# skmhrk1209/GANSynth

Hardware: AMD Instinct MI355X
Metric: G+D step images/sec at 128x1024x2 mel+IF (higher is better)
Workload: dtype bf16; 1 GPU; BASELINE.json configs[1]: fully grown PGGAN 128x1024x2 G+D iteration (D update + G update, R1 + mode-seeking), per-GPU batch 8, random-init weights; global_batch=8, parallelism=dp1, launch=hipGraph replay, forked branches, forked_branches=True

## Files before the change

### gansynth_amd/_lib.py

```python
import ctypes
import os
from ctypes import c_char_p, c_double, c_float, c_int, c_int64, c_size_t, c_void_p, POINTER

_HERE = os.path.dirname(os.path.abspath(__file__))
LIB_PATH = os.path.join(_HERE, "libgansynth_hip.so")

GS_F32, GS_BF16 = 0, 1
ACT_NONE, ACT_LRELU, ACT_TANH = 0, 1, 2
ACT_LRELU_BITS, ACT_WRITE_BITS = 5, 16
PREP_CONV_FWD, PREP_CONV_BWD_DATA, PREP_CONVT_FWD, PREP_CONVT_BWD_DATA = 0, 1, 2, 3
CONV_FWD, CONV_BWD_DATA, CONV_BWD_WEIGHT = 0, 1, 2

P, I, F, L, Z = c_void_p, c_int, c_float, c_int64, c_size_t


class GsConv(ctypes.Structure):
    _fields_ = [("n", ctypes.c_int32), ("h", ctypes.c_int32), ("w", ctypes.c_int32), ("ci", ctypes.c_int32), ("co", ctypes.c_int32),
                ("ksize", ctypes.c_int32), ("stride", ctypes.c_int32), ("transposed", ctypes.c_int32), ("dtype", ctypes.c_int32),
                ("w_prepared", ctypes.c_int32), ("alpha", c_float), ("ws", c_void_p), ("ws_bytes", c_size_t)]


C = POINTER(GsConv)

SIGNATURES = {
    "gs_last_error": (c_char_p, []),
    "gs_version": (I, []),
    "gs_init": (I, []),
    "gs_streams_create": (I, [I, POINTER(P)]),
    "gs_streams_destroy": (I, [I, POINTER(P)]),
    "gs_prof_enable": (I, [I]),
    "gs_prof_collect": (I, [POINTER(c_int), POINTER(c_double), POINTER(c_double)]),
    "gs_prof_roofline": (I, [ctypes.c_double, ctypes.c_double, P, P, P]),
    "gs_prof_records": (I, [I, P, P, P, P, P]),
    "gs_comm_available": (I, []),
    "gs_comm_unique_id": (I, [P]),
    "gs_comm_init": (I, [POINTER(P), I, I, P]),
    "gs_comm_destroy": (I, [P]),
    "gs_comm_count": (I, [P, POINTER(I)]),
    "gs_allreduce_sum_f32": (I, [P, P, ctypes.c_int64, P]),
    "gs_comm_set_marker_us": (I, [P, ctypes.c_double]),
    "gs_broadcast_f32": (I, [P, P, ctypes.c_int64, I, P]),
    "gs_conv_workspace_bytes": (Z, [C, I]),
    "gs_conv_fwd": (I, [C, P, P, P, I, P, P, F, P]),
    "gs_conv_fwd_mask": (I, [C, P, P, P, I, P, P]),
    "gs_conv_bwd_data": (I, [C, P, P, P, I, P, P]),
    "gs_conv_bwd_data_pnbwd": (I, [C, P, P, P, P, I, F, P, P]),
    "gs_conv_bwd_data_pnbwd_is_fused": (I, [C]),
    "gs_conv_fwd_pnbwdbwd": (I, [C, P, P, P, P, I, F, P, P, P]),
    "gs_conv_fwd_pnbwdbwd_is_fused": (I, [C]),
    "gs_conv_bwd_weight": (I, [C, P, P, P, P, I, P]),
    "gs_conv_wgrad_jobs_workspace_bytes": (Z, [P, I]),
    "gs_conv_wgrad_jobs": (I, [P, I, P, Z, P]),
    "gs_wgrad_cu_cap": (I, [I]),
    "gs_conv_igemm_config": (I, [I, I, I, I, I, I, I, I, POINTER(c_int)]),
    "gs_conv_igemm_table": (I, [I, POINTER(c_int)]),
    "gs_units_bias_act_to_nhwc": (I, [P, P, P, P, I, I, I, I, I, P]),
    "gs_nhwc_act_bwd_to_units": (I, [P, P, P, I, I, I, I, I, P]),
    "gs_dense_fwd_workspace_bytes": (Z, [I, I, I]),
    "gs_dense_fwd": (I, [P, P, P, I, I, I, F, I, P, Z, P]),
    "gs_dense_fwd_bias_act": (I, [P, P, P, P, I, I, I, F, I, I, P, Z, P]),
    "gs_dense_fwd_bias_act_nhwc": (I, [P, P, P, P, I, I, I, I, F, I, I, P, Z, P]),
    "gs_dense_bwd_data": (I, [P, P, P, I, I, I, F, I, P]),
    "gs_dense_bwd_weight": (I, [P, P, P, I, I, I, F, I, I, P]),
    "gs_dense_fwd_nhwc": (I, [P, P, P, I, I, I, I, F, I, P, Z, P]),
    "gs_dense_bwd_data_nhwc": (I, [P, P, P, I, I, I, I, F, I, P]),
    "gs_dense_bwd_weight_nhwc": (I, [P, P, P, I, I, I, I, F, I, I, P]),
    "gs_embedding_fwd": (I, [P, P, P, I, I, I, F, I, P]),
    "gs_embedding_onehot_fwd": (I, [P, P, P, P, I, I, I, F, I, P]),
    "gs_embedding_bwd": (I, [P, P, P, I, I, I, F, I, P]),
    "gs_bias_act_fwd": (I, [P, P, P, L, I, I, I, P]),
    "gs_act_bwd": (I, [P, P, P, L, I, I, P]),
    "gs_act_bwd_bias": (I, [P, P, P, P, L, I, I, I, I, P, Z, P]),
    "gs_tanh_bwd_bwd": (I, [P, P, P, P, L, I, P]),
    "gs_channel_sum_workspace_bytes": (Z, [L, I]),
    "gs_channel_sum": (I, [P, P, L, I, I, I, P, Z, P]),
    "gs_bias_partial_rows": (I, [I, L, I, I]),
    "gs_channel_fold_batch_workspace_bytes": (Z, [P, I]),
    "gs_channel_fold_batch": (I, [P, I, P, Z, P]),
    "gs_pixel_norm_fwd": (I, [P, P, L, I, F, I, P]),
    "gs_pixel_norm_bwd_fused": (I, [P, P, P, P, L, I, F, I, I, I, P]),
    "gs_pixel_norm_bwd_bias_workspace_bytes": (Z, [L, I, I]),
    "gs_pixel_norm_bwd_fused_bias": (I, [P, P, P, P, P, L, I, F, I, I, I, I, P, Z, P]),
    "gs_pixel_norm_bwd_bwd_fused": (I, [P, P, P, P, P, L, I, F, I, I, P]),
    "gs_upscale2d": (I, [P, P, I, I, I, I, I, I, F, I, P]),
    "gs_blocksum2d": (I, [P, P, I, I, I, I, I, I, F, I, P]),
    "gs_batch_stddev_fwd": (I, [P, P, I, I, I, F, I, P]),
    "gs_batch_stddev_bwd": (I, [P, P, P, P, I, I, I, F, I, P]),
    "gs_batch_stddev_bwd_bwd": (I, [P, P, P, P, P, I, I, I, F, I, P]),
    "gs_axpby": (I, [P, P, P, L, F, F, I, P]),
    "gs_axpby_dev": (I, [P, P, P, L, P, I, I, I, P]),
    "gs_sumsq_rows_workspace_bytes": (Z, [I]),
    "gs_sumsq_rows": (I, [P, P, I, L, I, P, Z, P]),
    "gs_row_scale": (I, [P, P, F, P, I, L, I, P]),
    "gs_weight_prep_batch": (I, [P, I, P]),
    "gs_gan_d_loss": (I, [P, P, P, P, F, I, I, P, P, P, P, I, P]),
    "gs_gan_g_loss": (I, [P, P, P, F, F, I, I, P, P, P, I, P]),
    "gs_adam_tf_step": (I, [P, P, P, P, L, F, F, F, F, F, P]),
    "gs_adam_tf_step_zero_grad": (I, [P, P, P, P, L, F, F, F, F, F, P]),
    "gs_adam_tf_step_dev": (I, [P, P, P, P, L, P, F, F, F, F, I, P]),
    "gs_pack_act_bits": (I, [P, L, I, I, P]),
    "gs_spectral_plan_create": (I, [POINTER(c_void_p), I, I, I, P, P]),
    "gs_spectral_plan_destroy": (I, [P]),
    "gs_stft_fwd": (I, [P, P, I, I, I, P, P, P]),
    "gs_mel_project": (I, [P, P, P, L, P]),
    "gs_if_unwrap": (I, [P, P, P, I, P]),
    "gs_stft_mel_if_fwd": (I, [P, P, I, I, I, P, I, P, Z, P]),
    "gs_stft_mel_if_workspace_bytes": (Z, [P, I]),
    "gs_mel_if_to_waveform": (I, [P, P, I, I, I, P, I, P, Z, P]),
    "gs_mel_if_to_waveform_workspace_bytes": (Z, [P, I]),
    "gs_weight_standardize": (I, [P, P, I, I, F, P]),
    "gs_resnet_stem_pool": (I, [P, P, P, P, P, I, I, I, I, I, P]),
    "gs_max_pool2d": (I, [P, P, I, I, I, I, I, P]),
    "gs_conv1x1_fwd": (I, [P, P, P, I, I, I, I, I, I, I, P]),
    "gs_group_norm_workspace_bytes": (Z, [I, I, I, I]),
    "gs_group_norm_stats": (I, [P, P, P, P, I, I, I, I, F, I, P, Z, P]),
    "gs_group_norm_apply": (I, [P, P, P, P, P, I, I, I, I, I, I, P]),
# ... 83 lines not shown
```

### gansynth_amd/config.py

```python
import os

KNOBS = {
    "GS_TORCH_COLLECTIVES": ("operational", "gradient all-reduce through torch.distributed's communicator instead of the library's own (gs_comm_*)"),
    "GS_NO_GRAPH_ALLREDUCE": ("operational", "no RCCL collective inside captured graphs: eager all-reduce behind each replay (bench.DP_LADDER's tamer modes)"),
    "GS_FORK_PROBE": ("operational", "auto | always | never: probe a forked hipGraph replay in a child process before the first forked capture "
                                     "(auto: only on HIP builds the workaround was not debugged on, fork_probe._forked_replay_ok)"),
    "GS_FORK_PROBED": ("operational", "(set by the probe for child processes: ok | died)"),
    "GS_FORK_PROBE_TIMEOUT_S": ("operational", "budget of that probe, seconds (600)"),
    "GS_LEVEL_STREAMS": ("operational", "throw-away streams alive while a graph is instantiated (128; capture.Capture._leveled_queues)"),
    "GS_COMM_MARKER_US": ("operational", "tests / profiles at world size 1: the one-rank all-reduce becomes a kernel that holds its stream this long "
                                         "(read once per communicator, comm.RcclComm; gs_comm_set_marker_us)"),
    "GS_CAPTURE_MODE": ("operational", "debugging: force torch.cuda.graph's capture_error_mode"),
    "GS_DEBUG_POISON_WS": ("operational", "debugging: kernel workspaces start as NaN bit patterns"),
    "GS_CHECK_FUSION": ("operational", "debugging: every fused cross-node form also runs its unfused definition and the two are compared"),
    "GS_FORK_EAGER": ("operational", "tests: the forked branches with eager launches on two streams"),
    "GS_NO_FORK_MARKS": ("operational", "debugging: branches start where they are opened, not at their marks"),
    "GS_NO_FORK": ("schedule", "no parallel branches in the runs' graphs (5.9 against 5.2 ms; also taken when GPU_MAX_HW_QUEUES != 4 or the probe fails)"),
    "GS_NO_MERGED_RUNS": ("schedule", "part A of the generator run NOT inside the discriminator run's graph (5.13 against 4.99 ms)"),
    "GS_NO_FUSED_ITERATION": ("schedule", "two graphs per iteration with eager optimizer steps between them (neutral on one GPU; data parallel both "
                                          "all-reduces are then the last node of a graph)"),
    "GS_OVERLAP_REDUCE": ("schedule", "data parallel: round 4's four-graph iteration, each all-reduce on a forked branch beside part A of the other run "
                                      "(hides both collectives; +0.7 ms at world size 1)"),
    "GS_NO_OVERLAP_REDUCE": ("schedule", "(overrides GS_OVERLAP_REDUCE)"),
    "GS_DEBUG_DP_BUCKET": ("operational", "print the range the first message of a two-step discriminator all-reduce covers"),
    "GS_DP_BUCKET_D": ("schedule", "data parallel: the discriminator's gradient all-reduced in two steps, ~98 % of it beside the end of its backward (300-us stand-ins: -0.09 ... -0.14 ms fully grown, +0.15 in a fade-in)"),
    "GS_EARLY_FLUSH_DIV": ("schedule", "a layer is 'large' from 1/DIV of the full resolution's pixels (16)"),
    "GS_EARLY_FLUSH_CUS": ("schedule", "CUs the early weight-gradient contraction is sized for (192; 160 / 224 / 256 within noise, round 6)"),
    "GS_D_TAIL_LEVELS": ("schedule", "levels of the discriminator's tail run over [real; fake] as one batch when the runs do not fork (3)"),
    "GS_NO_EARLY_FLUSH": ("ablation", "weight gradients of the full-chip levels contracted at the end of the run only"),
    "GS_NO_DEFERRED_REDUCE": ("ablation", "every weight gradient contracted where autograd produces it"),
    "GS_NO_DEFERRED_FOLDS": ("ablation", "bias-gradient partial rows folded by their producers"),
    "GS_NO_WGRAD_GROUPS": ("ablation", "no grouped weight-gradient launches"),
    "GS_NO_SPLIT_G_LOSS": ("ablation", "the generator's loss as one launch over both halves: the mode-seeking second-order pass waits for the discriminator's forward"),
    "GS_NO_SPLIT_FINAL_FLUSH": ("ablation", "the final weight-gradient contraction of a run on one stream (HBM-bound and MFMA-bound jobs one after the other)"),
    "GS_NO_FUSED_LOSSES": ("ablation", "per-sample loss algebra in torch instead of the one-launch loss heads"),
    "GS_NO_D_TAIL_BATCH": ("ablation", "real and fake pass through the discriminator's tail separately (no-fork schedule)"),
    "GS_NO_FUSED_NORM": ("ablation", "pixel norm as its own node behind every generator conv"),
    "GS_NO_NORM_EPILOGUE": ("ablation", "no pixel norm in conv epilogues"),
    "GS_NO_NORM_BWD_EPILOGUE": ("ablation", "no previous-block norm backward in data-gradient epilogues"),
    "GS_NO_NORM_BWD2_EPILOGUE": ("ablation", "no second-order norm kernel in the forward-on-cotangent conv"),
    "GS_NO_NORM_BWD_BIAS": ("ablation", "bias sums outside the norm's backward"),
    "GS_NO_MASK_BITS": ("ablation", "leaky-relu masks read as the bf16 activations themselves, not as the sign bits stored behind them"),
    "GS_NO_PREMASK": ("ablation", "activation derivative never folded into the consuming data-gradient kernel"),
    "GS_NO_PREMASK_GRAPH": ("ablation", "... not across autograd nodes"),
    "GS_NO_PREMASK_GRAPH2": ("ablation", "... not in second-order graphs"),
    "GS_NO_PARAMS_ONLY": ("ablation", "leaf activations receive gradients like tf.gradients would not ask for"),
    "GS_NO_DERIVED_SLICES": ("ablation", "the 257-channel conv's weight slices copied on every use"),
    "GS_NO_UNITS_NHWC": ("ablation", "dense -> reshape -> activation as three steps"),
    "GS_NO_DENSE_NHWC": ("ablation", "flatten copy + plain dense kernels"),
}


def _check(name):
    if name not in KNOBS:
        raise KeyError("gansynth_amd.config: %s is not a registered environment switch (add it to KNOBS with its description)" % name)


def flag(name):
    _check(name)
    return bool(os.environ.get(name))


def value(name, default=None):
    _check(name)
    return os.environ.get(name, default)
```

### gansynth_amd/csrc/conv_api.hip

```cpp
#include "conv_shared.h"
#include <utility>
#include <vector>

namespace gs {


bool igemm_supported(int ic, int oc, int dtype);
bool igemm_norm_fused(int mode, int N, int Hb, int Wb, int IC, int OC, int dtype, int want);
int igemm_config(int mode, int N, int Hb, int Wb, int IC, int OC, int dtype, int want, int* out);
int igemm_table(int index, int* out);
extern "C" int gs_pixel_norm_bwd_bwd_fused(const void* gg, const void* g, const void* x, void* out, void* out_g, int64_t p, int c, float eps, int pre_act,
                                           int dtype, void* stream);
bool wgrad_mfma_supported(int ic, int oc, int dtype);
size_t igemm_prep_bytes(int ic, int oc, int dtype);
int run_igemm(int mode, int variant, const void* x, const float* w_hwio, void* y, int N, int Hi, int Wi, int ICk,
              int OCk, int w_ci, int w_co, int Hb, int Wb, float alpha, const float* bias, int act, int dtype, int w_prepared,
              void* ws, size_t ws_bytes, hipStream_t st, const void* mask = nullptr, int mask_act = 0, void* y2 = nullptr, float pn_eps = 0.f,
              const void* addend = nullptr, int normbwd = 0);
extern "C" int gs_pixel_norm_bwd_fused(const void* g, const void* x, const void* addend, void* gx, int64_t p, int c, float eps, int pre_act, int post_act, int dtype,
                                       void* stream);
size_t wgrad_mfma_bytes(int mode, int dtype, int N, int Hb, int Wb, int IC, int OC);
bool wgrad_mfma_has_bias(int dtype);
int run_wgrad_mfma(int mode, const WgradSrcs& srcs, int nsrc, float* gw, float* gb, int N, int Hi, int Wi, int IC, int OC, int Hb,
                   int Wb, float alpha, int transpose, int accumulate, int dtype, void* ws, size_t ws_bytes, hipStream_t st,
                   GsWgradReduce* defer = nullptr);
bool wgrad_sk_supported(int mode, int dtype, int IC, int OC);
void wgrad_sk_job_geometry(int mode, int N, SkJob& q);
void wgrad_sk_plan(int mode, SkGroup& g);
size_t wgrad_sk_bytes(const SkGroup& g);
int run_wgrad_sk(int mode, const SkGroup& g, void* ws, size_t ws_bytes, hipStream_t st);

template <typename T, int OCV, int VEC>
__global__ void conv_direct_kernel(const T* __restrict__ x, const float* __restrict__ wp, T* __restrict__ y, int mode,
                                   int ks, int N, int Hi, int Wi, int IC, int OC, int Ho, int Wo, float alpha) {
    const int ngrp = OC / OCV;
    const long idx = (long)blockIdx.x * blockDim.x + threadIdx.x;
    const long total = (long)N * Ho * Wo * ngrp;
    if (idx >= total) return;
    const int g = idx % ngrp;
    long pix = idx / ngrp;
    const int ox = pix % Wo;
    pix /= Wo;
    const int oy = pix % Ho;
    const int n = pix / Ho;
    const int oc = g * OCV;
    float acc[OCV];
#pragma unroll
    for (int v = 0; v < OCV; ++v) acc[v] = 0.f;
    for (int ky = 0; ky < ks; ++ky) {
        int iy;
        if (mode == MODE_S1) iy = oy + ky - (ks >> 1);
// ... 140 lines not shown
                word |= (unsigned)__builtin_amdgcn_update_dpp(0, (int)word, 0x4E, 0xf, 0xf, false);
                if (piece == 0) bits[(px * OC + oc0) >> 5] = word;
                return;
            }
        }
        st_wide<T>(y + px * OC + oc0, o);
    };
    auto ldpix = [&](long px, float* xv) __attribute__((always_inline)) {
        if constexpr (IC == 2 && sizeof(T) == 2) {
            const unsigned u = *reinterpret_cast<const unsigned*>(x + px * 2);
            xv[0] = __uint_as_float(u << 16);
            xv[1] = __uint_as_float(u & 0xffff0000u);
        } else {
#pragma unroll
            for (int i = 0; i < IC; ++i) xv[i] = DT<T>::ld(x + px * IC + i);
        }
    };
    for (; pix + 3 * stride < P; pix += 4 * stride) {
        float xv[4][IC];
#pragma unroll
        for (int k = 0; k < 4; ++k) ldpix(pix + k * stride, xv[k]);
#pragma unroll
        for (int k = 0; k < 4; ++k) one(pix + k * stride, xv[k]);
    }
    for (; pix < P; pix += stride) {
        float xv[IC];
        ldpix(pix, xv);
        one(pix, xv);
    }
}

template <typename T, int IC>
__global__ __launch_bounds__(256) void thin_expand_pnbwd_kernel(const T* __restrict__ x, const float* __restrict__ wp, const T* __restrict__ z,
                                                                const T* __restrict__ addend, T* __restrict__ y, long P, int OC, float alpha, float eps, int act) {
    constexpr int WN = Wide<T>::N;
    const int groups = OC / WN;
    const int oc0 = (threadIdx.x % groups) * WN;
    float wr[WN][IC];
#pragma unroll
    for (int v = 0; v < WN; ++v)
#pragma unroll
        for (int i = 0; i < IC; ++i) wr[v][i] = wp[(long)(oc0 + v) * IC + i] * alpha;
    const long ppb = 256 / groups;
    const long stride = (long)gridDim.x * ppb;
    const long npass = (P + stride - 1) / stride;
    const float inv_c = 1.f / (float)OC;
    for (long k = 0; k < npass; ++k) {
        const long pix = (long)blockIdx.x * ppb + threadIdx.x / groups + k * stride;
        const long px = pix < P ? pix : P - 1;
        float xv[IC], zv[WN], av[WN], g[WN];
        if constexpr (IC == 2 && sizeof(T) == 2) {
            const unsigned u = *reinterpret_cast<const unsigned*>(x + px * 2);
            xv[0] = __uint_as_float(u << 16);
            xv[1] = __uint_as_float(u & 0xffff0000u);
        } else {
#pragma unroll
            for (int i = 0; i < IC; ++i) xv[i] = DT<T>::ld(x + px * IC + i);
        }
        ld_wide<T>(z + px * OC + oc0, zv);
        if (addend) ld_wide<T>(addend + px * OC + oc0, av);
        float ssq = 0.f, szg = 0.f;
#pragma unroll
        for (int v = 0; v < WN; ++v) {
            float a = 0.f;
#pragma unroll
            for (int i = 0; i < IC; ++i) a += xv[i] * wr[v][i];
            g[v] = a;
            ssq += zv[v] * zv[v];
            szg += zv[v] * a;
        }
        ssq = group_sum(ssq, groups);
        szg = group_sum(szg, groups);
        const float r = rsqrtf(ssq * inv_c + eps);
        const float m = szg * inv_c * r * r;
        float out[WN];
#pragma unroll
        for (int v = 0; v < WN; ++v) {
            float t = r * (g[v] - zv[v] * m);
            if (addend) t += av[v];
            out[v] = act == GS_ACT_LRELU ? (zv[v] > 0.f ? t : 0.2f * t) : t;
        }
        if (pix < P) st_wide<T>(y + pix * OC + oc0, out);
    }
}
static bool thin_expand_pnbwd_ok(int ks, int ICk, int OCk, int dtype) {
    const int wn = dtype == GS_F32 ? 4 : 8;
    if (ks != 1 || ICk < 1 || ICk > 4 || OCk % wn != 0) return false;
    const int groups = OCk / wn;
    return groups >= 1 && groups <= 64 && (groups & (groups - 1)) == 0;
}
static int run_thin_expand_pnbwd(const void* x, const float* wp, const void* z, const void* addend, void* y, long P, int ICk, int OCk, float alpha, float eps, int act,
                                 int dtype, hipStream_t st) {
    const int wn = dtype == GS_F32 ? 4 : 8;
    long nb = cdiv(P * (OCk / wn), 256);
    if (nb > 4096) nb = 4096;
    const unsigned grid = (unsigned)nb;
#define GS_TEP(TT, ICV) hipLaunchKernelGGL((thin_expand_pnbwd_kernel<TT, ICV>), dim3(grid), dim3(256), 0, st, (const TT*)x, wp, (const TT*)z, (const TT*)addend, (TT*)y, P, OCk, alpha, eps, act)
#define GS_TEP_ALL(TT) do { if (ICk == 1) GS_TEP(TT, 1); else if (ICk == 2) GS_TEP(TT, 2); else if (ICk == 3) GS_TEP(TT, 3); else GS_TEP(TT, 4); } while (0)
    GS_DISPATCH_DTYPE(dtype, GS_TEP_ALL(T));
#undef GS_TEP_ALL
#undef GS_TEP
    GS_CHECK_LAUNCH();
    return 0;
}

template <typename T, int OC, int ACT, int LC>
__global__ __launch_bounds__(256) void thin_reduce_kernel(const T* __restrict__ x, const float* __restrict__ wp, const float* __restrict__ bias,
                                                          T* __restrict__ y, long P, int IC, float alpha) {
    constexpr int WN = Wide<T>::N;
    const int L = LC ? LC : IC / WN;
    const int l = threadIdx.x % L;
    float wr[OC][WN];
#pragma unroll
    for (int v = 0; v < OC; ++v)
#pragma unroll
        for (int i = 0; i < WN; ++i) wr[v][i] = wp[v * IC + l * WN + i] * alpha;
    const long ppb = 256 / L;
    const long npass = (P + (long)gridDim.x * ppb - 1) / ((long)gridDim.x * ppb);
    float bv[OC];
#pragma unroll
    for (int v = 0; v < OC; ++v) bv[v] = bias ? bias[v] : 0.f;
    auto fold = [&](float* a) __attribute__((always_inline)) {
#pragma unroll
        for (int v = 0; v < OC; ++v) a[v] = group_sum(a[v], LC != 0 ? LC : L);
    };
    auto finish = [&](long pix, float* a) __attribute__((always_inline)) {
        fold(a);
        if (pix < P && l == 0) {
            if constexpr (OC == 2 && sizeof(T) == 2) {
                *reinterpret_cast<unsigned*>(y + pix * 2) = pack_bf16x2(thin_act<ACT>(a[0] + bv[0]), thin_act<ACT>(a[1] + bv[1]));
// ... 798 lines not shown
    JobPlan plan;
    if (plan_jobs(jobs, njobs, plan)) return 0;
    return plan.total_bytes;
}

extern "C" int gs_conv_wgrad_jobs(const GsWgradJob* jobs, int njobs, void* ws, size_t ws_bytes, void* stream) {
    GS_CHECK_ARG(njobs >= 0 && (njobs == 0 || jobs), "conv_wgrad_jobs: bad args");
    if (njobs == 0) return 0;
    JobPlan plan;
    if (int e = plan_jobs(jobs, njobs, plan)) return e;
    if (ws_bytes < plan.total_bytes) return fail(GS_ERR_WORKSPACE, "conv_wgrad_jobs: workspace %zu < %zu", ws_bytes, plan.total_bytes);
    hipStream_t st = as_stream(stream);
    for (auto& kg : plan.groups)
        if (int e = run_wgrad_sk(kg.first, kg.second, ws, plan.group_bytes, st)) return e;
    std::vector<GsWgradReduce> pend;
    for (size_t k = 0; k < plan.single.size(); ++k) {
        const GsWgradJob& jb = plan.single[k];
        GsConv c = job_conv(jb, jb.n[0]);
        c.ws = reinterpret_cast<unsigned char*>(ws) + plan.single_off[k];
        c.ws_bytes = (k + 1 < plan.single.size() ? plan.single_off[k + 1] : plan.total_bytes) - plan.single_off[k];
        GsWgradReduce d;
        memset(&d, 0, sizeof(d));
        if (int rc = wgrad_layer(c, jb.x, jb.gy, jb.n, jb.nsrc, jb.bias_mask, jb.gw, jb.gb, jb.accumulate, &d, stream)) return rc;
        if (jb.gw_ci_stride > jb.ci) {
            if (d.nslices <= 0 || d.transpose) return fail(GS_ERR_UNSUPPORTED, "conv_wgrad_jobs: a %d -> %d layer cannot add into a channel slice", jb.ci, jb.co);
            d.ic_ld = jb.gw_ci_stride;
        }
        if (d.nslices > 0) pend.push_back(d);
    }
    if (!pend.empty()) return wgrad_reduce_batch(pend.data(), (int)pend.size(), stream);
    return 0;
}

extern "C" int gs_conv_fwd_pnbwdbwd(const GsConv* c, const void* x, const float* w_hwio, const void* g, const void* z, int act, float eps, void* out_g, void* out_z,
                                    void* stream) {
    if (int e = check_conv(c)) return e;
    GS_CHECK_ARG(g && z && out_g && out_z && (act == GS_ACT_NONE || act == GS_ACT_LRELU), "conv_fwd_pnbwdbwd: g, z and both outputs are required, activation none or leaky relu (got %d)", act);
    const ConvRole r = conv_role(*c, GS_CONV_FWD);
    if (c->ksize == 3 && igemm_supported(r.ICk, r.OCk, c->dtype))
        return run_igemm(r.mode, r.variant, x, w_hwio, out_g, c->n, r.Hi, r.Wi, r.ICk, r.OCk, c->ci, c->co, r.Hb, r.Wb, c->alpha, nullptr, GS_ACT_NONE, c->dtype, c->w_prepared, c->ws,
                         c->ws_bytes, as_stream(stream), z, act, out_z, eps, g, 2);
    if (int e = gs_conv_fwd(c, x, w_hwio, nullptr, GS_ACT_NONE, out_g, nullptr, 0.f, stream)) return e;
    return gs_pixel_norm_bwd_bwd_fused(out_g, g, z, out_z, out_g, (int64_t)c->n * r.Ho * r.Wo, c->co, eps, act, c->dtype, stream);
}
extern "C" int gs_conv_fwd_pnbwdbwd_is_fused(const GsConv* c) {
    if (check_conv(c) || c->ksize != 3 || !(c->transposed || c->stride == 1)) return 0;
    const ConvRole r = conv_role(*c, GS_CONV_FWD);
    return igemm_norm_fused(r.mode, c->n, r.Hb, r.Wb, r.ICk, r.OCk, c->dtype, IGEMM_NORM_BWD2) ? 1 : 0;
}

extern "C" int gs_conv_bwd_data_pnbwd(const GsConv* c, const void* gy, const float* w_hwio, const void* z, const void* addend, int act, float eps, void* gx, void* stream) {
    if (int e = check_conv(c)) return e;
    GS_CHECK_ARG(z && gx && (act == GS_ACT_NONE || act == GS_ACT_LRELU), "conv_bwd_data_pnbwd: z is required, activation none or leaky relu (got %d)", act);
    hipStream_t st = as_stream(stream);
    const ConvRole r = conv_role(*c, GS_CONV_BWD_DATA);
    const bool epilogue_map = c->transposed || c->stride == 1;
    if (epilogue_map && c->ksize == 3 && igemm_supported(r.ICk, r.OCk, c->dtype))
        return run_igemm(r.mode, r.variant, gy, w_hwio, gx, c->n, r.Hi, r.Wi, r.ICk, r.OCk, c->ci, c->co, r.Hb, r.Wb, c->alpha, nullptr, GS_ACT_NONE, c->dtype, c->w_prepared, c->ws,
                         c->ws_bytes, st, z, act, nullptr, eps, addend, 1);
    if (c->stride == 1 && thin_expand_pnbwd_ok(c->ksize, r.ICk, r.OCk, c->dtype)) {
        const long total = (long)c->ci * c->co;
        if (c->ws_bytes < (size_t)total * 4) return fail(GS_ERR_WORKSPACE, "conv_bwd_data_pnbwd: workspace %zu < %zu", c->ws_bytes, (size_t)total * 4);
        float* wp = reinterpret_cast<float*>(c->ws);
        if (!c->w_prepared) {
            hipLaunchKernelGGL((weight_prep_kernel<float>), dim3(cdiv(total, 256)), dim3(256), 0, st, w_hwio, wp, 1, c->ci, c->co, 1);
            GS_CHECK_LAUNCH();
        }
        return run_thin_expand_pnbwd(gy, wp, z, addend, gx, (long)c->n * r.Ho * r.Wo, r.ICk, r.OCk, c->alpha, eps, act, c->dtype, st);
    }
    if (int e = gs_conv_bwd_data(c, gy, w_hwio, nullptr, 0, gx, stream)) return e;
    return gs_pixel_norm_bwd_fused(gx, z, addend, gx, (int64_t)c->n * r.Ho * r.Wo, c->ci, eps, GS_ACT_NONE, act, c->dtype, stream);
}
extern "C" int gs_conv_bwd_data_pnbwd_is_fused(const GsConv* c) {
    if (check_conv(c) || !(c->transposed || c->stride == 1)) return 0;
    const ConvRole r = conv_role(*c, GS_CONV_BWD_DATA);
    if (c->ksize == 1) return thin_expand_pnbwd_ok(1, r.ICk, r.OCk, c->dtype) ? 1 : 0;
    return igemm_norm_fused(r.mode, c->n, r.Hb, r.Wb, r.ICk, r.OCk, c->dtype, IGEMM_NORM_BWD) ? 1 : 0;
}
extern "C" int gs_conv_igemm_config(int mode, int n, int hb, int wb, int ic, int oc, int dtype, int want, int* out_cfg) {
    return igemm_config(mode, n, hb, wb, ic, oc, dtype, want, out_cfg);
}
extern "C" int gs_conv_igemm_table(int index, int* out11) { return igemm_table(index, out11); }
```

### gansynth_amd/csrc/conv_igemm.hip

```cpp
#include "conv_device.h"
#include "gs_prof.h"

extern "C" int gs_pixel_norm_fwd(const void* x, void* y, int64_t p, int c, float eps, int dtype, void* stream);
extern "C" int gs_pack_act_bits(void* z, int64_t p, int c, int dtype, void* stream);
extern "C" int gs_pixel_norm_bwd_fused(const void* g, const void* x, const void* addend, void* gx, int64_t p, int c, float eps, int pre_act, int post_act, int dtype,
                                       void* stream);
extern "C" int gs_pixel_norm_bwd_bwd_fused(const void* gg, const void* g, const void* x, void* out, void* out_g, int64_t p, int c, float eps, int pre_act,
                                           int dtype, void* stream);

namespace gs {

struct ConvP {
    const void* x;
    const void* wp;
    void* y;
    const float* bias;
    int act;
    const void* mask;
    int mask_act;
    const unsigned char* mask_bits;
    unsigned char* bits_out;
    void* y2;
    float pn_eps;
    const void* addend;
    int normbwd;
    int* norm_pending;
    int N, Hi, Wi, IC, OC, Hb, Wb, tiles_x, tiles_y, nsp, noct, nch;
    unsigned m_noct, m_tx, m_ty;
    float alpha;
#ifdef GS_IGEMM_TRACE
    unsigned long long* trace;
#endif
};
#ifdef GS_IGEMM_TRACE
#define GS_TR(slot)                                                                                              \
    do {                                                                                                         \
        if (p.trace && threadIdx.x == 0 && (slot) < 64) {                                                        \
            p.trace[blockIdx.x * 64 + (slot)] = __builtin_amdgcn_s_memtime();                                    \
            if ((slot) == 0 || (slot) == 63) p.trace[4096 * 64 + blockIdx.x * 2 + ((slot) == 63)] = __builtin_amdgcn_s_memrealtime(); \
        }                                                                                                        \
    } while (0)
#else
#define GS_TR(slot) do { } while (0)
#endif

__device__ __forceinline__ void lds_dma16_s(unsigned lds_addr, unsigned voff, i32x4 rs, unsigned soff) {
    asm volatile("s_mov_b32 m0, %0\n\ts_nop 0\n\tbuffer_load_dwordx4 %1, %2, %3 offen lds"
                 :
                 : "s"(lds_addr), "v"(voff), "s"(rs), "s"(__builtin_amdgcn_readfirstlane(soff))
                 : "memory", "m0");
}

#ifndef GS_NORM_EPI_PIPELINE
#define GS_NORM_EPI_PIPELINE 1
#endif
template <typename T, int MODE, int A, int B, int TW, int TG, bool RESIDENT, int D, int NORM, int RB = 64, bool SPEC = false, bool BITS = false>
__global__ __launch_bounds__(SPEC ? 512 : 256) void conv_igemm_kernel(const ConvP p) {
// ... 202 lines not shown
    zero_acc();
    if (computer) {
#pragma unroll
        for (int b = 0; b < B; ++b)
#pragma unroll
            for (int ox = 0; ox < 3; ++ox)
#pragma unroll
                for (int ks = 0; ks < KS; ++ks) asm volatile("" : "+v"(b_off[b][ox][ks]));
#pragma unroll
        for (int ks = 0; ks < KS; ++ks) asm volatile("" : "+v"(a_off[ks]));
#pragma unroll
        for (int ph = 0; ph < NPH; ++ph)
#pragma unroll
            for (int a = 0; a < A; ++a)
#pragma unroll
                for (int b = 0; b < B; ++b) asm volatile("" : "+v"(acc[ph][a][b]));
    }
    wait_vmcnt(0);
    block_barrier();
    GS_TR(3);
#ifdef GS_IGEMM_TRACE
    int tr_stage = 0;
#endif

    int item = first, done = 0, c_pb = 0, c_wb = 0;
    while (true) {
        int n, by, bx, oc0;
        item_coords(item, n, by, bx, oc0);
        unsigned mbw[BITS ? B * (MODE == MODE_T2 ? 4 : 1) : 1][A];
        constexpr bool NPIPE = (NORM == 2 || NORM == 3) && A * B <= 2 && GS_NORM_EPI_PIPELINE;
        typedef typename std::conditional<SZ == 4, float4, uint4>::type nvec_t;
        constexpr int NNV = SZ == 4 ? 4 : 2;
        nvec_t nz[NPIPE ? 2 : 1][A][NNV], nx[NPIPE ? 2 : 1][A][NNV];
        auto norm_fetch = [&](int i, nvec_t (&zq)[A][NNV], nvec_t (&xq)[A][NNV]) __attribute__((always_inline)) {
            constexpr int NPHB = MODE == MODE_T2 ? 4 : 1;
            const int b = i / NPHB, ph = i % NPHB;
            const int Ho = MODE == MODE_T2 ? 2 * Hb : Hb, Wo = MODE == MODE_T2 ? 2 * Wb : Wb;
            const int q = (wv * B + b) * 32 + l31;
            const int gy = by + q / TW, gx = bx + q % TW;
            const int oy = MODE == MODE_T2 ? 2 * gy + (ph >> 1) : gy;
            const int ox = MODE == MODE_T2 ? 2 * gx + (ph & 1) : gx;
            const long base = (gy < Hb && gx < Wb) ? (((long)n * Ho + oy) * Wo + ox) * OC + oc0 : 0;
#ifdef GS_ABL_NOMASKLOAD
            const long zbase = base & 1023;
#else
            const long zbase = base;
#endif
#pragma unroll
            for (int a = 0; a < A; ++a)
#pragma unroll
                for (int v = 0; v < NNV; ++v) {
                    zq[a][v] = *reinterpret_cast<const nvec_t*>(reinterpret_cast<const T*>(p.mask) + zbase + a * 32 + v * (32 / NNV) + hi * (16 / NNV));
                    if (NORM == 3 || p.addend)
                        xq[a][v] = *reinterpret_cast<const nvec_t*>(reinterpret_cast<const T*>(p.addend) + base + a * 32 + v * (32 / NNV) + hi * (16 / NNV));
                }
        };
        for (int ch = 0; ch < NCH; ++ch) {
#pragma unroll
            for (int tg = 0; tg < NTG; ++tg) {
                const int itg = (tg + D) % NTG;
                const int npiece = stage_pieces(itg);
                if (issuer) issue_setup(itg);
                if constexpr (NPIPE) {
                    if (tg == NTG - 1 && ch == NCH - 1 && computer) norm_fetch(0, nz[0], nx[0]);
                }
                if constexpr (BITS) {
                    if (tg == NTG - 1 && ch == NCH - 1 && computer && p.mask_bits) {
                        constexpr int NPHB = MODE == MODE_T2 ? 4 : 1;
                        const int Ho = MODE == MODE_T2 ? 2 * Hb : Hb, Wo = MODE == MODE_T2 ? 2 * Wb : Wb;
#pragma unroll
                        for (int b = 0; b < B; ++b) {
                            const int q = (wv * B + b) * 32 + l31;
                            const int gy = by + q / TW, gx = bx + q % TW;
#pragma unroll
                            for (int ph = 0; ph < NPHB; ++ph) {
                                const int oy = MODE == MODE_T2 ? 2 * gy + (ph >> 1) : gy;
                                const int ox = MODE == MODE_T2 ? 2 * gx + (ph & 1) : gx;
                                const long off = (gy < Hb && gx < Wb) ? (((long)n * Ho + oy) * Wo + ox) * OC + oc0 : 0;
#pragma unroll
                                for (int a = 0; a < A; ++a) mbw[b * NPHB + ph][a] = *reinterpret_cast<const unsigned*>(p.mask_bits + ((off + a * 32) >> 3));
                            }
                        }
                    }
                }
                if (SPEC && loader) {
#pragma unroll
                    for (int q = 0; q < npiece; ++q) issue_piece(q, itg);
                }
                const unsigned char* lp = lpatch + c_pb * PBUF;
                const unsigned char* lw = RESIDENT ? lwgt + ch * WBUF : lwgt + c_wb * WBUF;
                if (computer) {
                    constexpr int PF = NSTEP >= 6 ? 2 : 1;
                    frag_t af[PF + 1][A], bf[PF + 1][B];
                    auto load_frag = [&](int step, int r) __attribute__((always_inline)) {
                        const int tt = step / KS, ks = step % KS, buf = step % (PF + 1);
                        const int i = tg * TG + tt;
                        const int oyv = tap_off<MODE>(tap_ky<MODE>(i)), oxv = tap_off<MODE>(tap_kx<MODE>(i));
// ... 152 lines not shown
                    } else if constexpr (MASK_ALL) {
                        if (p.mask) {
#pragma unroll
                            for (int b = 0; b < B; ++b) {
                                const int q = (wv * B + b) * 32 + l31;
                                const int gy = by + q / TW, gx = bx + q % TW;
#pragma unroll
                                for (int ph = 0; ph < NPH; ++ph) {
                                    const int oy = MODE == MODE_T2 ? 2 * gy + (ph >> 1) : gy;
                                    const int ox = MODE == MODE_T2 ? 2 * gx + (ph & 1) : gx;
                                    mask_fetch((((long)n * Ho + oy) * Wo + ox) * OC + oc0, gy < Hb && gx < Wb, mz_all[b * NPH + ph]);
                                }
                            }
                        }
                    }
#pragma unroll
                    for (int b = 0; b < B; ++b) {
                        const int q = (wv * B + b) * 32 + l31;
                        const int gy = by + q / TW, gx = bx + q % TW;
#ifdef GS_ABL_NOSTORE
                        const bool inside = gy < -1000;
#else
                        const bool inside = gy < Hb && gx < Wb;
#endif
#pragma unroll
                        for (int ph = 0; ph < NPH; ++ph) {
                            const int oy = MODE == MODE_T2 ? 2 * gy + (ph >> 1) : gy;
                            const int ox = MODE == MODE_T2 ? 2 * gx + (ph & 1) : gx;
                            const long off = (((long)n * Ho + oy) * Wo + ox) * OC + oc0;
                            if constexpr (NORM == 2) {
                                constexpr int EV = 16 / NV;
                                const int cur = NPIPE ? ((b * NPH + ph) & 1) : 0;
                                if constexpr (NPIPE) {
                                    if (b * NPH + ph + 1 < B * NPH) norm_fetch(b * NPH + ph + 1, nz[(b * NPH + ph + 1) & 1], nx[(b * NPH + ph + 1) & 1]);
                                } else {
                                    mask_fetch(off, inside, nz[0]);
                                    if (p.addend) {
                                        const long base = inside ? off : 0;
#pragma unroll
                                        for (int a = 0; a < A; ++a)
#pragma unroll
                                            for (int v = 0; v < NV; ++v)
                                                nx[0][a][v] = *reinterpret_cast<const mvec_t*>(reinterpret_cast<const T*>(p.addend) + base + a * 32 + v * (32 / NV) + hi * (16 / NV));
                                    }
                                }
                                mvec_t (&zq)[A][NV] = nz[cur];
                                mvec_t (&aq)[A][NV] = nx[cur];
                                float gv[A][NV][EV], zv[A][NV][EV];
                                float ssq = 0.f, szg = 0.f;
#pragma unroll
                                for (int a = 0; a < A; ++a) {
                                    float o[4][4];
                                    finish(ph, a, b, o);
                                    if constexpr (SZ == 4) {
#pragma unroll
                                        for (int qd = 0; qd < 4; ++qd) {
                                            const float4 z4 = zq[a][qd];
                                            const float zz[4] = {z4.x, z4.y, z4.z, z4.w};
#pragma unroll
                                            for (int e = 0; e < 4; ++e) { gv[a][qd][e] = o[qd][e]; zv[a][qd][e] = zz[e]; }
                                        }
                                    } else {
#pragma unroll
                                        for (int qp = 0; qp < 2; ++qp) {
#pragma unroll
                                            for (int e = 0; e < 4; ++e) {
                                                const auto r = __builtin_amdgcn_permlane32_swap(__float_as_uint(o[2 * qp][e]), __float_as_uint(o[2 * qp + 1][e]), false, false);
                                                gv[a][qp][e] = __uint_as_float(r[0]);
                                                gv[a][qp][4 + e] = __uint_as_float(r[1]);
                                            }
                                            const uint4 z4 = zq[a][qp];
                                            const unsigned zw[4] = {z4.x, z4.y, z4.z, z4.w};
#pragma unroll
                                            for (int e = 0; e < 4; ++e) { zv[a][qp][2 * e] = __uint_as_float(zw[e] << 16); zv[a][qp][2 * e + 1] = __uint_as_float(zw[e] & 0xffff0000u); }
                                        }
                                    }
#pragma unroll
                                    for (int v = 0; v < NV; ++v)
#pragma unroll
                                        for (int e = 0; e < EV; ++e) { ssq += zv[a][v][e] * zv[a][v][e]; szg += zv[a][v][e] * gv[a][v][e]; }
                                }
                                ssq = swap32_sum(ssq);
                                szg = swap32_sum(szg);
                                const float inv_c = 1.f / (float)(32 * A);
                                const float r = rsqrtf(ssq * inv_c + p.pn_eps);
                                const float m = szg * inv_c * r * r;
#pragma unroll
                                for (int a = 0; a < A; ++a)
#pragma unroll
                                    for (int v = 0; v < NV; ++v) {
                                        float out[EV], ad[EV];
#pragma unroll
                                        for (int e = 0; e < EV; ++e) ad[e] = 0.f;
                                        if (p.addend) {
                                            if constexpr (SZ == 4) {
                                                const float4 a4 = aq[a][v];
                                                ad[0] = a4.x; ad[1] = a4.y; ad[2] = a4.z; ad[3] = a4.w;
                                            } else {
                                                const uint4 a4 = aq[a][v];
                                                const unsigned aw[4] = {a4.x, a4.y, a4.z, a4.w};
#pragma unroll
                                                for (int e = 0; e < 4; ++e) { ad[2 * e] = __uint_as_float(aw[e] << 16); ad[2 * e + 1] = __uint_as_float(aw[e] & 0xffff0000u); }
                                            }
                                        }
#pragma unroll
                                        for (int e = 0; e < EV; ++e) out[e] = (r * (gv[a][v][e] - zv[a][v][e] * m) + ad[e]) * mask_factor(zv[a][v][e]);
                                        if (inside) {
                                            if constexpr (SZ == 4) {
                                                st4(reinterpret_cast<float*>(y) + off + a * 32 + v * 8 + hi * 4, out);
                                            } else {
                                                uint4 w4;
                                                w4.x = pack_bf16x2(out[0], out[1]); w4.y = pack_bf16x2(out[2], out[3]);
                                                w4.z = pack_bf16x2(out[4], out[5]); w4.w = pack_bf16x2(out[6], out[7]);
                                                *reinterpret_cast<uint4*>(reinterpret_cast<bf16_t*>(y) + off + a * 32 + v * 16 + hi * 8) = w4;
                                            }
                                        }
                                    }
                            } else if constexpr (NORM == 3) {
                                constexpr int EV = 16 / NV;
                                const int cur = NPIPE ? ((b * NPH + ph) & 1) : 0;
                                if constexpr (NPIPE) {
                                    if (b * NPH + ph + 1 < B * NPH) norm_fetch(b * NPH + ph + 1, nz[(b * NPH + ph + 1) & 1], nx[(b * NPH + ph + 1) & 1]);
                                } else {
                                    mask_fetch(off, inside, nz[0]);
                                    const long base = inside ? off : 0;
#pragma unroll
                                    for (int a = 0; a < A; ++a)
#pragma unroll
                                        for (int v = 0; v < NV; ++v)
                                            nx[0][a][v] = *reinterpret_cast<const mvec_t*>(reinterpret_cast<const T*>(p.addend) + base + a * 32 + v * (32 / NV) + hi * (16 / NV));
                                }
                                mvec_t (&zq)[A][NV] = nz[cur];
                                mvec_t (&gq)[A][NV] = nx[cur];
                                float hv[A][NV][EV], zv[A][NV][EV], gv[A][NV][EV];
                                float ssq = 0.f, shg = 0.f, shz = 0.f, szg = 0.f;
#pragma unroll
                                for (int a = 0; a < A; ++a) {
                                    float o[4][4];
                                    finish(ph, a, b, o);
                                    if constexpr (SZ == 4) {
#pragma unroll
                                        for (int qd = 0; qd < 4; ++qd) {
                                            const float4 z4 = zq[a][qd], g4 = gq[a][qd];
                                            const float zz[4] = {z4.x, z4.y, z4.z, z4.w}, g_[4] = {g4.x, g4.y, g4.z, g4.w};
#pragma unroll
                                            for (int e = 0; e < 4; ++e) { hv[a][qd][e] = o[qd][e]; zv[a][qd][e] = zz[e]; gv[a][qd][e] = g_[e]; }
                                        }
                                    } else {
#pragma unroll
                                        for (int qp = 0; qp < 2; ++qp) {
#pragma unroll
                                            for (int e = 0; e < 4; ++e) {
                                                const auto r = __builtin_amdgcn_permlane32_swap(__float_as_uint(o[2 * qp][e]), __float_as_uint(o[2 * qp + 1][e]), false, false);
                                                hv[a][qp][e] = __uint_as_float(r[0]);
                                                hv[a][qp][4 + e] = __uint_as_float(r[1]);
                                            }
                                            const uint4 z4 = zq[a][qp], g4 = gq[a][qp];
                                            const unsigned zw[4] = {z4.x, z4.y, z4.z, z4.w}, gw_[4] = {g4.x, g4.y, g4.z, g4.w};
#pragma unroll
                                            for (int e = 0; e < 4; ++e) {
                                                zv[a][qp][2 * e] = __uint_as_float(zw[e] << 16); zv[a][qp][2 * e + 1] = __uint_as_float(zw[e] & 0xffff0000u);
                                                gv[a][qp][2 * e] = __uint_as_float(gw_[e] << 16); gv[a][qp][2 * e + 1] = __uint_as_float(gw_[e] & 0xffff0000u);
                                            }
                                        }
                                    }
#pragma unroll
                                    for (int v = 0; v < NV; ++v)
#pragma unroll
                                        for (int e = 0; e < EV; ++e) {
                                            const float zc = zv[a][v][e], gc = gv[a][v][e];
                                            const float hc = hv[a][v][e] * mask_factor(zc);
                                            hv[a][v][e] = hc;
                                            ssq += zc * zc; shg += hc * gc; shz += hc * zc; szg += zc * gc;
                                        }
                                }
                                ssq = swap32_sum(ssq); shg = swap32_sum(shg);
                                shz = swap32_sum(shz); szg = swap32_sum(szg);
                                const float inv_c = 1.f / (float)(32 * A);
                                const float r = rsqrtf(ssq * inv_c + p.pn_eps);
                                const float r2 = r * r, r3 = r2 * r;
                                const float ma = shg * inv_c, mb = shz * inv_c, mm = szg * inv_c;
                                const float kz = 3.f * r3 * r2 * mb * mm - r3 * ma;
#pragma unroll
                                for (int a = 0; a < A; ++a)
#pragma unroll
                                    for (int v = 0; v < NV; ++v) {
                                        float o1[EV], o2[EV];
#pragma unroll
                                        for (int e = 0; e < EV; ++e) {
                                            const float zc = zv[a][v][e], gc = gv[a][v][e], hc = hv[a][v][e];
                                            o1[e] = r * (hc - zc * r2 * mb);
                                            o2[e] = kz * zc - r3 * (mm * hc + mb * gc);
                                        }
                                        if (inside) {
                                            if constexpr (SZ == 4) {
                                                st4(reinterpret_cast<float*>(y) + off + a * 32 + v * 8 + hi * 4, o1);
                                                st4(reinterpret_cast<float*>(p.y2) + off + a * 32 + v * 8 + hi * 4, o2);
                                            } else {
                                                uint4 w4;
                                                w4.x = pack_bf16x2(o1[0], o1[1]); w4.y = pack_bf16x2(o1[2], o1[3]); w4.z = pack_bf16x2(o1[4], o1[5]); w4.w = pack_bf16x2(o1[6], o1[7]);
                                                *reinterpret_cast<uint4*>(reinterpret_cast<bf16_t*>(y) + off + a * 32 + v * 16 + hi * 8) = w4;
                                                w4.x = pack_bf16x2(o2[0], o2[1]); w4.y = pack_bf16x2(o2[2], o2[3]); w4.z = pack_bf16x2(o2[4], o2[5]); w4.w = pack_bf16x2(o2[6], o2[7]);
                                                *reinterpret_cast<uint4*>(reinterpret_cast<bf16_t*>(p.y2) + off + a * 32 + v * 16 + hi * 8) = w4;
                                            }
                                        }
                                    }
                            } else if constexpr (NORM == 1) {
                                float o[A][4][4], ssq = 0.f;
#pragma unroll
                                for (int a = 0; a < A; ++a) {
                                    finish(ph, a, b, o[a]);
#pragma unroll
                                    for (int k = 0; k < 16; ++k) ssq += o[a][k >> 2][k & 3] * o[a][k >> 2][k & 3];
                                }
// ... 63 lines not shown
    constexpr int OCT = 32 * A;
    constexpr int BK = RB / (int)sizeof(T);
    constexpr int NTG = 9 / TG;
    constexpr int PBUF = ((PH * PW * (RB / 16) + 255) / 256) * 4096;
    constexpr int WBUF = ((TG * OCT * RB + 4095) / 4096) * 4096;
    constexpr int NPB = 1 + (D + NTG - 1) / NTG, NWB = D + 1;
    p.tiles_x = cdiv(p.Wb, TW);
    p.tiles_y = cdiv(p.Hb, TH);
    p.nsp = p.N * p.tiles_x * p.tiles_y;
    p.noct = cdiv(p.OC, OCT);
    p.nch = p.IC / BK;
    {
        auto magic = [](int d) { return d <= 1 ? 0u : (unsigned)(((1ull << 32) + (unsigned)d - 1) / (unsigned)d); };
        if (p.noct >= 2048 || p.tiles_x >= 2048 || p.tiles_y >= 2048)
            return fail(GS_ERR_UNSUPPORTED, "conv igemm: %d channel tiles / %d x %d spatial tiles exceed the item decoder's range", p.noct, p.tiles_x, p.tiles_y);
        static const long max_items = getenv("GS_IGEMM_MAX_ITEMS") ? atol(getenv("GS_IGEMM_MAX_ITEMS")) : (1L << 21);
        if ((long)p.nsp * p.noct >= max_items) {
            const long per_image = (long)p.tiles_x * p.tiles_y * p.noct;
            const int chunk = (int)((max_items - 1) / per_image);
            if (chunk < 1) return fail(GS_ERR_UNSUPPORTED, "conv igemm: %ld work items per image exceed the item decoder's range", per_image);
            const size_t in_img = (size_t)p.Hi * p.Wi * p.IC * sizeof(T);
            const size_t out_img = (size_t)p.Hb * p.Wb * (MODE == MODE_T2 ? 4 : 1) * p.OC * sizeof(T);
            auto adv = [](const void* q, size_t b) -> const void* { return q ? (const char*)q + b : nullptr; };
            for (int n0 = 0; n0 < p.N; n0 += chunk) {
                ConvP q = p;
                q.N = p.N - n0 < chunk ? p.N - n0 : chunk;
                q.x = adv(p.x, n0 * in_img);
                q.y = const_cast<void*>(adv(p.y, n0 * out_img));
                q.y2 = const_cast<void*>(adv(p.y2, n0 * out_img));
                q.mask = adv(p.mask, n0 * out_img);
                q.mask_bits = reinterpret_cast<const unsigned char*>(adv(p.mask_bits, n0 * out_img / (8 * sizeof(T))));
                q.bits_out = reinterpret_cast<unsigned char*>(const_cast<void*>(adv(p.bits_out, n0 * out_img / (8 * sizeof(T)))));
                q.addend = adv(p.addend, n0 * out_img);
                int pending = 0;
                if (p.norm_pending) q.norm_pending = &pending;
                if (int e = launch_igemm<T, MODE, A, B, TW, TG, RESIDENT, D, NORM, RB, SPEC, BITS>(q, st)) return e;
                if (p.norm_pending && pending) *p.norm_pending = pending;
            }
            return 0;
        }
        p.m_noct = magic(p.noct); p.m_tx = magic(p.tiles_x); p.m_ty = magic(p.tiles_y);
    }
    const int wbufs = RESIDENT ? p.nch : NWB;
    const size_t lds = (size_t)NPB * PBUF + (size_t)wbufs * WBUF + (size_t)((p.OC + 3) / 4) * 16 + 0;
    if (p.OC % OCT != 0) return fail(GS_ERR_UNSUPPORTED, "conv igemm: %d output channels with %d-wide tiles", p.OC, OCT);
    if ((size_t)p.Hi * p.Wi * p.IC * sizeof(T) >= (1ull << 31)) return fail(GS_ERR_UNSUPPORTED, "conv igemm: one image exceeds 2 GiB");
    if (lds > 160 * 1024) return fail(GS_ERR_UNSUPPORTED, "conv igemm: %zu bytes of LDS needed", lds);
    if (NORM && p.OC != OCT) return fail(GS_ERR_UNSUPPORTED, "conv igemm: fused pixel norm needs the whole channel range in one tile");
    if ((NORM == 2 || NORM == 3) && p.OC != OCT) return fail(GS_ERR_UNSUPPORTED, "conv igemm: fused pixel-norm backward needs the whole channel range in one tile");
    if (!((NORM == 2 && p.normbwd == 1) || (NORM == 3 && p.normbwd == 2)) && p.normbwd) {
        if (p.norm_pending) *p.norm_pending = 1 + p.normbwd;
        p.normbwd = 0;
        p.mask = nullptr;
        p.addend = nullptr;
        p.y2 = nullptr;
    }
    if (NORM != 1 && NORM != 3 && p.y2) {
        if (!p.y) p.y = p.y2;
        p.y2 = nullptr;
        if (p.norm_pending) *p.norm_pending = 1;
    }
    if (p.IC % BK != 0) return fail(GS_ERR_UNSUPPORTED, "conv igemm: %d input channels with %d-channel chunks", p.IC, BK);
    auto kern = conv_igemm_kernel<T, MODE, A, B, TW, TG, RESIDENT, D, NORM, RB, SPEC, BITS>;
    static size_t max_set = 0;
    if (lds > max_set) {
        if (hipFuncSetAttribute(reinterpret_cast<const void*>(kern), hipFuncAttributeMaxDynamicSharedMemorySize, (int)lds) != hipSuccess)
            return fail(GS_ERR_HIP, "conv igemm: cannot reserve %zu bytes of dynamic LDS", lds);
        max_set = lds;
    }
    int per_cu = (int)((160 * 1024) / lds);
    if (per_cu > GS_MAX_BLOCKS_PER_CU) per_cu = GS_MAX_BLOCKS_PER_CU;
    if (per_cu < 1 || SPEC) per_cu = 1;
    const long total = (long)p.nsp * p.noct;
    long grid = (long)per_cu * num_cus();
    if (grid > total) grid = total;
    if (grid >= 8) grid &= ~7L;
    const double flops = 2.0 * 9.0 * (double)p.N * p.Hb * p.Wb * p.IC * p.OC;
    const double out_px = (double)p.N * p.Hb * p.Wb * (MODE == MODE_T2 ? 4 : 1);
    const double bytes = ((double)p.N * p.Hi * p.Wi * p.IC + out_px * p.OC * (1.0 + (p.mask ? (p.mask_bits ? 1.0 / 16.0 : 1.0) : 0.0) + (p.bits_out ? 1.0 / 16.0 : 0.0) + ((NORM == 1 && p.y) ? 1.0 : 0.0) + ((NORM == 2 && p.addend) ? 1.0 : 0.0) + (NORM == 3 ? 2.0 : 0.0)) + 9.0 * p.IC * p.OC) * sizeof(T);
    const int reps = prof_reps();
    ProfScope ps(st, flops, bytes, MODE, p.N, p.Hb, p.Wb, p.IC, p.OC, p.mask ? 1 : 0, NORM ? 1 : 0, reps);
    for (int r = 0; r < reps; ++r) hipLaunchKernelGGL(kern, dim3((unsigned)grid), dim3(SPEC ? 512 : 256), lds, st, p);
    return 0;
}

struct IgemmCfg {
    int A, B, TW, TG;
    bool RESIDENT = false;
    int D = 2, NORM = IGEMM_PLAIN, RB = 64;
    bool SPEC = false;
    bool operator==(const IgemmCfg& o) const {
        return A == o.A && B == o.B && TW == o.TW && TG == o.TG && RESIDENT == o.RESIDENT && D == o.D && NORM == o.NORM && RB == o.RB && SPEC == o.SPEC;
    }
};
struct IgemmKnobs { bool no_small_tiles, no_rb128, spec; };
static IgemmKnobs igemm_knobs() {
    static const IgemmKnobs k = {getenv("GS_NO_SMALL_TILES") != nullptr, getenv("GS_NO_RB128") != nullptr,
                                 getenv("GS_SPEC") ? (atoi(getenv("GS_SPEC")) & 1) != 0 : true};
    return k;
}

static IgemmCfg choose_igemm(int mode, int dtype, int N, int Hb, int Wb, int IC, int OC, int want, long cus, IgemmKnobs knobs) {
    constexpr int FWD = 1 << IGEMM_NORM_FWD, BWD = 1 << IGEMM_NORM_BWD, BWD2 = 1 << IGEMM_NORM_BWD2;
    auto epi = [&](int forms) { return (forms >> want) & 1 ? want : IGEMM_PLAIN; };
    const int nch = IC / (dtype == GS_F32 ? 16 : 32);
    const bool a2 = OC % 64 == 0;
    const int tw = Wb >= 32 ? 32 : 16;
    auto items64 = [&](int B_) { return (long)N * cdiv(Hb, 4 * B_) * cdiv(Wb, 32) * (OC / 64); };
    const bool small = !knobs.no_small_tiles && items64(1) <= cus;
    const bool rb128 = dtype == GS_BF16 && !knobs.no_rb128 && IC % 64 == 0;
    if (mode == MODE_S2) {
        if (small) return {1, 1, tw, 9, false, 1};
// ... 105 lines not shown
int igemm_config(int mode, int N, int Hb, int Wb, int IC, int OC, int dtype, int want, int* out) {
    if (mode < MODE_S1 || mode > MODE_T2 || (dtype != GS_F32 && dtype != GS_BF16) || want < IGEMM_PLAIN || want > IGEMM_NORM_BWD2 || N < 1 || Hb < 1 || Wb < 1 || !out)
        return fail(GS_ERR_ARG, "conv igemm config: bad mode %d / dtype %d / epilogue %d / shape %d x %d x %d", mode, dtype, want, N, Hb, Wb);
    if (!igemm_supported(IC, OC, dtype)) return fail(GS_ERR_UNSUPPORTED, "conv igemm config: %d -> %d channels do not run on the implicit GEMM", IC, OC);
    const IgemmCfg c = choose_igemm(mode, dtype, N, Hb, Wb, IC, OC, want, num_cus(), igemm_knobs());
    const int v[10] = {c.A, c.B, c.TW, c.TG, c.RESIDENT, c.D, c.NORM, c.RB, c.SPEC, igemm_instantiated(mode, dtype, c)};
    memcpy(out, v, sizeof(v));
    return 0;
}
int igemm_table(int index, int* out) {
    static const int rows[][11] = {
#define GS_ROW(M, BF16_ONLY, A, B, TW, TG, RESIDENT, D, NORM, RB, SPEC) {M, BF16_ONLY, A, B, TW, TG, RESIDENT, D, NORM, RB, SPEC},
        GS_IGEMM_CONFIGS(GS_ROW)
#undef GS_ROW
    };
#ifdef GS_FORCE_CFG
    constexpr int n = (int)(sizeof(rows) / sizeof(rows[0])) - 1;
#else
    constexpr int n = (int)(sizeof(rows) / sizeof(rows[0]));
#endif
    if (index < 0 || index >= n || !out) return fail(GS_ERR_ARG, "conv igemm table: row %d of %d", index, n);
    memcpy(out, rows[index], sizeof(rows[0]));
    return 0;
}

size_t igemm_prep_bytes(int ic, int oc, int dtype) {
    return align256((size_t)9 * ic * oc * (dtype == GS_F32 ? 4 : 2));
}

template <typename T>
static int run_igemm_t(int mode, int variant, const void* x, const float* w_hwio, void* y, int N, int Hi, int Wi,
                       int ICk, int OCk, int w_ci, int w_co, int Hb, int Wb, float alpha, const float* bias, int act,
                       int w_prepared, void* ws, size_t ws_bytes, hipStream_t st, const void* mask, int mask_act, void* y2, float pn_eps,
                       const void* addend, int normbwd) {
    const size_t need = (size_t)9 * w_ci * w_co * sizeof(T);
    if (ws_bytes < need) return fail(GS_ERR_WORKSPACE, "conv igemm: workspace %zu < %zu", ws_bytes, need);
    T* wp = reinterpret_cast<T*>(ws);
    const long total = 9L * w_ci * w_co;
    if (!w_prepared)
        hipLaunchKernelGGL((weight_prep_kernel<T>), dim3(cdiv(total, 256)), dim3(256), 0, st, w_hwio, wp, 9, w_ci, w_co, variant);
    ConvP p;
    memset(&p, 0, sizeof(p));
    const size_t out_numel = (size_t)N * Hb * Wb * (mode == MODE_T2 ? 4 : 1) * OCk;
    const bool plain = y2 == nullptr && !normbwd;
    const bool write_bits = (act & GS_ACT_WRITE_BITS) != 0;
    act &= ~GS_ACT_WRITE_BITS;
    if (mask_act == GS_ACT_LRELU_BITS) {
        mask_act = GS_ACT_LRELU;
        if (sizeof(T) == 2 && plain && mask && OCk % 32 == 0) p.mask_bits = reinterpret_cast<const unsigned char*>(mask) + out_numel * sizeof(T);
    }
    bool bits_pending = write_bits;
    if (write_bits && sizeof(T) == 2 && plain && y && act == GS_ACT_LRELU && OCk % 32 == 0 && (!mask || p.mask_bits)) {
        p.bits_out = reinterpret_cast<unsigned char*>(y) + out_numel * sizeof(T);
        bits_pending = false;
    }
    p.x = x; p.wp = wp; p.y = y; p.bias = bias; p.act = act; p.mask = mask; p.mask_act = mask_act;
    p.N = N; p.Hi = Hi; p.Wi = Wi; p.IC = ICk; p.OC = OCk; p.Hb = Hb; p.Wb = Wb; p.alpha = alpha;
    int pending = 0;
    p.y2 = y2; p.pn_eps = pn_eps; p.norm_pending = &pending;
    p.addend = normbwd ? addend : nullptr; p.normbwd = normbwd;
    int rc;
    if (mode == MODE_S1) rc = dispatch_igemm<T, MODE_S1>(p, st);
    else if (mode == MODE_S2) rc = dispatch_igemm<T, MODE_S2>(p, st);
    else rc = dispatch_igemm<T, MODE_T2>(p, st);
    if (rc) return rc;
    GS_CHECK_LAUNCH();
    if (pending == 3) {
        const long px = (long)N * Hb * Wb * (mode == MODE_T2 ? 4 : 1);
        return gs_pixel_norm_bwd_bwd_fused(y, addend, mask, y2, y, px, OCk, pn_eps, mask_act, sizeof(T) == 4 ? GS_F32 : GS_BF16, st);
    }
    if (pending == 2) {
        const long px = (long)N * Hb * Wb * (mode == MODE_T2 ? 4 : 1);
        return gs_pixel_norm_bwd_fused(y, mask, addend, y, px, OCk, pn_eps, GS_ACT_NONE, mask_act, sizeof(T) == 4 ? GS_F32 : GS_BF16, st);
    }
    if (pending) {
        const long px = (long)N * Hb * Wb * (mode == MODE_T2 ? 4 : 1);
        if (int e = gs_pixel_norm_fwd(y ? y : y2, y2, px, OCk, pn_eps, sizeof(T) == 4 ? GS_F32 : GS_BF16, st)) return e;
    }
    if (bits_pending && y)
        return gs_pack_act_bits(y, (int64_t)(out_numel / OCk), OCk, sizeof(T) == 4 ? GS_F32 : GS_BF16, st);
    return 0;
}

int run_igemm(int mode, int variant, const void* x, const float* w_hwio, void* y, int N, int Hi, int Wi, int ICk,
              int OCk, int w_ci, int w_co, int Hb, int Wb, float alpha, const float* bias, int act, int dtype, int w_prepared,
              void* ws, size_t ws_bytes, hipStream_t st, const void* mask, int mask_act, void* y2, float pn_eps, const void* addend, int normbwd) {
    GS_DISPATCH_DTYPE(dtype, return (run_igemm_t<T>(mode, variant, x, w_hwio, y, N, Hi, Wi, ICk, OCk, w_ci, w_co, Hb,
                                                    Wb, alpha, bias, act, w_prepared, ws, ws_bytes, st, mask, mask_act, y2, pn_eps, addend, normbwd)));
}

}

extern "C" int gs_prof_enable(int on) {
    gs::g_prof.on = on != 0;
    gs::g_prof.burst = on > 1 ? on : 1;
    gs::g_prof.used = 0;
    gs::g_prof.flops = 0.0;
    return 0;
}

extern "C" int gs_prof_roofline(double peak_tflops, double peak_gbps, double* total_bytes, double* roof_ms, double* roof_ms_hbm_bound) {
    double bytes = 0.0, roof = 0.0, roof_hbm = 0.0;
    for (int i = 0; i < gs::g_prof.used; ++i) {
        if (gs::g_prof.ldesc[i][0] >= 10) continue;
        const double tf = gs::g_prof.lflops[i] / (peak_tflops * 1e12) * 1e3, tb = gs::g_prof.lbytes[i] / (peak_gbps * 1e9) * 1e3;
        bytes += gs::g_prof.lbytes[i];
        roof += tf > tb ? tf : tb;
        if (tb >= tf) roof_hbm += tb;
    }
    if (total_bytes) *total_bytes = bytes;
    if (roof_ms) *roof_ms = roof;
    if (roof_ms_hbm_bound) *roof_ms_hbm_bound = roof_hbm;
    return 0;
}

extern "C" int gs_prof_records(int max_records, int* n, double* ms, double* flops, double* bytes, int* desc) {
    int k = 0;
    for (int i = 0; i < gs::g_prof.used && k < max_records; ++i, ++k) {
        (void)hipEventSynchronize(gs::g_prof.ev[i][1]);
        float t = 0.f;
        if (hipEventElapsedTime(&t, gs::g_prof.ev[i][0], gs::g_prof.ev[i][1]) != hipSuccess) t = 0.f;
// ... 26 lines not shown
```

### gansynth_amd/csrc/elementwise.hip

```cpp
#include "gs_common.h"

namespace gs {

static inline int ew_grid(long nvec) {
    long g = (nvec + 255) / 256;
    static const long cap = getenv("GS_EW_GRID_CAP") ? atol(getenv("GS_EW_GRID_CAP")) : 8192;
    if (g > cap) g = cap;
    if (g < 1) g = 1;
    return (int)g;
}

template <typename T, int ACT, bool BIAS>
__global__ void bias_act_kernel(const T* __restrict__ x, const float* __restrict__ bias, T* __restrict__ y, long nvec, int cvec) {
    for (long i = (long)blockIdx.x * blockDim.x + threadIdx.x; i < nvec; i += (long)gridDim.x * blockDim.x) {
        float v[4];
        ld4(x + i * 4, v);
        if (BIAS) {
            const float4 b = *reinterpret_cast<const float4*>(bias + (i % cvec) * 4);
            v[0] += b.x; v[1] += b.y; v[2] += b.z; v[3] += b.w;
        }
#pragma unroll
        for (int e = 0; e < 4; ++e) {
            if (ACT == GS_ACT_LRELU) v[e] = v[e] > 0.f ? v[e] : 0.2f * v[e];
            if (ACT == GS_ACT_TANH) v[e] = tanhf(v[e]);
// ... 322 lines not shown
    return fold_launch(second, st);
}
extern "C" int gs_bias_partial_rows(int producer, int64_t p, int c, int dtype);

template <typename T>
__global__ __launch_bounds__(256) void channel_sum_rows_kernel(const T* __restrict__ g, float* __restrict__ out, int p, int c, int accumulate) {
    const int ch = blockIdx.x * 256 + threadIdx.x;
    if (ch >= c) return;
    float s = 0.f;
    for (int r = 0; r < p; ++r) s += DT<T>::ld(g + (long)r * c + ch);
    out[ch] = accumulate ? out[ch] + s : s;
}

static int channel_sum_parts(long p, int c) {
    long rows_per_block = 256 / (c >= 4 ? ((c & 3) == 0 ? c / 4 : (c < 256 ? c : 256)) : c);
    if (rows_per_block < 1) rows_per_block = 1;
    long nb = (p + rows_per_block * 8 - 1) / (rows_per_block * 8);
    if (nb > 2048) nb = 2048;
    if (nb < 1) nb = 1;
    return (int)nb;
}

template <typename T, int E> __device__ inline void pn_ld(const T* p, float* o) {
    if constexpr (E == Wide<T>::N) ld_wide<T>(p, o);
    else ld4(p, *reinterpret_cast<float(*)[4]>(o));
}
template <typename T, int E> __device__ inline void pn_st(T* p, const float* o) {
    if constexpr (E == Wide<T>::N) st_wide<T>(p, o);
    else st4(p, *reinterpret_cast<const float(*)[4]>(o));
}
template <typename T, int MODE, int E, int P, int U, bool BS = false>
__global__ __launch_bounds__(256) void pixel_norm_kernel(const T* __restrict__ a0, const T* __restrict__ a1, const T* __restrict__ a2,
                                                         T* __restrict__ out, long p, int c, float eps, int act, int pre,
                                                         const T* __restrict__ addend, T* __restrict__ out2, float* __restrict__ bsum = nullptr) {
    const int vecs = c / E;
    const int L = vecs < 64 ? vecs : 64;
    const int rows_per_wave = 64 / L;
    const int lane = threadIdx.x & 63;
    const int sub = lane % L;
    const long wave = ((long)blockIdx.x * blockDim.x + threadIdx.x) >> 6;
    const long nwaves = ((long)gridDim.x * blockDim.x) >> 6;
    const float invc = 1.f / (float)c;
    const T* const xbase = MODE == 0 ? a0 : (MODE == 1 ? a1 : a2);
    float bs[BS ? P : 1][BS ? E : 1];
    if (BS) {
#pragma unroll
        for (int k = 0; k < P; ++k)
#pragma unroll
            for (int e = 0; e < E; ++e) bs[k][e] = 0.f;
    }
    auto dact = [&](int kind, float xv) __attribute__((always_inline)) {
        return kind == GS_ACT_LRELU ? (xv > 0.f ? 1.f : 0.2f) : (kind == GS_ACT_TANH ? 1.f - xv * xv : 1.f);
    };
    for (long row0 = wave * rows_per_wave; row0 < p; row0 += nwaves * rows_per_wave * U) {
        long off[U];
        bool ok[U];
        float xv[U][P][E], av[U][P][E], bv[U][P][E];
#pragma unroll
        for (int u = 0; u < U; ++u) {
            const long row = row0 + u * nwaves * rows_per_wave + lane / L;
            ok[u] = row < p;
            off[u] = (ok[u] ? row : 0) * c + sub * E;
#pragma unroll
            for (int k = 0; k < P; ++k) {
                pn_ld<T, E>(xbase + off[u] + k * L * E, xv[u][k]);
                if (MODE >= 1) pn_ld<T, E>(a0 + off[u] + k * L * E, av[u][k]);
                if (MODE == 2) pn_ld<T, E>(a1 + off[u] + k * L * E, bv[u][k]);
            }
        }
#pragma unroll
        for (int u = 0; u < U; ++u) {
            float s = 0.f;
#pragma unroll
            for (int k = 0; k < P; ++k)
#pragma unroll
                for (int e = 0; e < E; ++e) s += xv[u][k][e] * xv[u][k][e];
            s = group_sum(s, L);
            const float r = rsqrtf(s * invc + eps);
            if (MODE == 0) {
#pragma unroll
                for (int k = 0; k < P; ++k) {
                    float o[E];
#pragma unroll
                    for (int e = 0; e < E; ++e) o[e] = xv[u][k][e] * r;
                    if (ok[u]) pn_st<T, E>(out + off[u] + k * L * E, o);
                }
            } else if (MODE == 1) {
                float q = 0.f;
#pragma unroll
                for (int k = 0; k < P; ++k)
#pragma unroll
                    for (int e = 0; e < E; ++e) {
                        av[u][k][e] *= dact(pre, xv[u][k][e]);
                        q += xv[u][k][e] * r * av[u][k][e];
                    }
                q = group_sum(q, L);
                q *= invc;
#pragma unroll
                for (int k = 0; k < P; ++k) {
                    float o[E], ad[E];
#pragma unroll
                    for (int e = 0; e < E; ++e) ad[e] = 0.f;
                    if (addend) pn_ld<T, E>(addend + off[u] + k * L * E, ad);
#pragma unroll
                    for (int e = 0; e < E; ++e) o[e] = (r * (av[u][k][e] - xv[u][k][e] * r * q) + ad[e]) * dact(act, xv[u][k][e]);
                    if (ok[u]) pn_st<T, E>(out + off[u] + k * L * E, o);
                    if (BS && ok[u]) {
#pragma unroll
                        for (int e = 0; e < E; ++e) bs[k][e] += o[e];
                    }
                }
            } else {
                float sa = 0.f, sp = 0.f, sq = 0.f;
#pragma unroll
                for (int k = 0; k < P; ++k)
#pragma unroll
                    for (int e = 0; e < E; ++e) {
                        av[u][k][e] *= dact(pre, xv[u][k][e]);
                        const float yv = xv[u][k][e] * r;
                        sa += av[u][k][e] * bv[u][k][e];
                        sp += yv * av[u][k][e];
                        sq += yv * bv[u][k][e];
                    }
                sa = group_sum(sa, L);
                sp = group_sum(sp, L);
                sq = group_sum(sq, L);
                const float k0 = r * r * invc;
#pragma unroll
                for (int k = 0; k < P; ++k) {
                    float o[E];
#pragma unroll
                    for (int e = 0; e < E; ++e) {
                        const float yv = xv[u][k][e] * r;
                        o[e] = k0 * (-sa * yv - sq * av[u][k][e] - sp * bv[u][k][e] + 3.f * sp * sq * yv * invc);
                    }
                    if (ok[u]) pn_st<T, E>(out + off[u] + k * L * E, o);
                    if (out2) {
                        float o2[E];
#pragma unroll
                        for (int e = 0; e < E; ++e) o2[e] = r * (av[u][k][e] - xv[u][k][e] * r * (sp * invc));
                        if (ok[u]) pn_st<T, E>(out2 + off[u] + k * L * E, o2);
                    }
                }
            }
        }
    }
    if constexpr (BS) {
        __shared__ float bred[4][P * 64 * E];
#pragma unroll
        for (int k = 0; k < P; ++k)
#pragma unroll
            for (int e = 0; e < E; ++e) {
                bs[k][e] = residue_sum(bs[k][e], L);
            }
        const int wv = threadIdx.x >> 6;
        if (lane < L) {
#pragma unroll
            for (int k = 0; k < P; ++k)
#pragma unroll
// ... 289 lines not shown
    if ((c & 3) != 0 || c > 1024 || 256 % (c >> 2) != 0) {
        if (int e = gs_act_bwd(g, y, gx, p * c, act, dtype, stream)) return e;
        return gs_channel_sum(gx, gb, p, c, accumulate, dtype, ws, ws_bytes, stream);
    }
    const bool partials_only = (accumulate & GS_SUM_PARTIALS) != 0;
    accumulate &= 1;
    const int nparts = channel_sum_parts(p, c);
    if (ws_bytes < (partials_only ? (size_t)nparts * c * sizeof(float) : gs_channel_sum_workspace_bytes(p, c))) return fail(GS_ERR_WORKSPACE, "act_bwd_bias: workspace too small");
    hipStream_t st = as_stream(stream);
    float* part = (float*)ws;
    GS_DISPATCH_DTYPE(dtype, {
        if (act == 1) hipLaunchKernelGGL((act_bwd_sum_kernel<T, 1>), dim3(nparts), dim3(256), 0, st, (const T*)g, (const T*)y, (T*)gx, part, (long)p, c);
        else hipLaunchKernelGGL((act_bwd_sum_kernel<T, 2>), dim3(nparts), dim3(256), 0, st, (const T*)g, (const T*)y, (T*)gx, part, (long)p, c);
    });
    GS_CHECK_LAUNCH();
    if (partials_only) return 0;
    return channel_sum_finalize(part, gb, nparts, c, accumulate, st);
}

static int pixel_norm_grid(long p, int c, int wn, bool bias_sums = false) {
    const int E = c % wn == 0 ? wn : 4;
    const int vecs = c / E, L = vecs < 64 ? vecs : 64, P = vecs / L;
    const int U = P == 1 ? 2 : 1;
    const long rows_per_block = 4L * (64 / L) * U;
    int g = ew_grid((p + rows_per_block - 1) / rows_per_block * 256);
    if (bias_sums) {
        static const int cap = getenv("GS_PN_BIAS_GRID_CAP") ? atoi(getenv("GS_PN_BIAS_GRID_CAP")) : 1024;
        if (g > cap) g = cap;
    }
    return g;
}
template <typename T, int MODE, bool BS = false>
static void pixel_norm_launch_t(const void* a0, const void* a1, const void* a2, void* out, long p, int c, float eps, int act, int pre, const void* addend,
                                void* out2, hipStream_t st, float* bsum = nullptr) {
    constexpr int WN = Wide<T>::N;
    const int E = c % WN == 0 ? WN : 4;
    const int vecs = c / E, L = vecs < 64 ? vecs : 64, P = vecs / L;
    dim3 grid(pixel_norm_grid(p, c, WN, BS));
#define GS_PN(EE, PP, UU)                                                                                                          \
    hipLaunchKernelGGL((pixel_norm_kernel<T, MODE, EE, PP, UU, BS>), grid, dim3(256), 0, st, (const T*)a0, (const T*)a1, (const T*)a2, (T*)out, p, c, eps, \
                       act, pre, (const T*)addend, (T*)out2, bsum)
    if (E == WN) {
        if (P == 1) GS_PN(WN, 1, 2); else if (P == 2) GS_PN(WN, 2, 1); else GS_PN(WN, 4, 1);
    } else {
        if (P == 1) GS_PN(4, 1, 2); else if (P == 2) GS_PN(4, 2, 1); else GS_PN(4, 4, 1);
    }
#undef GS_PN
}
static int pixel_norm_launch(int mode, const void* a0, const void* a1, const void* a2, void* out, int64_t p, int c, float eps, int dtype, void* stream, int act = 0,
                             int pre = 0, const void* addend = nullptr, void* out2 = nullptr) {
    GS_CHECK_ARG(p > 0 && c >= 4 && c <= 1024 && (c & (c - 1)) == 0, "pixel_norm: c=%d must be a power of two in [4,1024]", c);
    hipStream_t st = as_stream(stream);
    GS_DISPATCH_DTYPE(dtype, {
        if (mode == 0) pixel_norm_launch_t<T, 0>(a0, a1, a2, out, (long)p, c, eps, act, pre, addend, out2, st);
        else if (mode == 1) pixel_norm_launch_t<T, 1>(a0, a1, a2, out, (long)p, c, eps, act, pre, addend, out2, st);
        else pixel_norm_launch_t<T, 2>(a0, a1, a2, out, (long)p, c, eps, act, pre, addend, out2, st);
    });
    GS_CHECK_LAUNCH();
    return 0;
}
extern "C" int gs_pixel_norm_fwd(const void* x, void* y, int64_t p, int c, float eps, int dtype, void* stream) {
    return pixel_norm_launch(0, x, nullptr, nullptr, y, p, c, eps, dtype, stream);
}
static bool pn_act_ok(int a) { return a == GS_ACT_NONE || a == GS_ACT_LRELU || a == GS_ACT_TANH; }
extern "C" int gs_pixel_norm_bwd_fused(const void* g, const void* x, const void* addend, void* gx, int64_t p, int c, float eps, int pre_act, int post_act,
                                       int dtype, void* stream) {
    GS_CHECK_ARG(pn_act_ok(pre_act) && pn_act_ok(post_act), "pixel_norm_bwd_fused: bad activation %d / %d", pre_act, post_act);
    return pixel_norm_launch(1, g, x, nullptr, gx, p, c, eps, dtype, stream, post_act, pre_act, addend);
}
extern "C" size_t gs_pixel_norm_bwd_bias_workspace_bytes(int64_t p, int c, int dtype) {
    const int nb = pixel_norm_grid((long)p, c, dtype == GS_F32 ? 4 : 8, true);
    return (size_t)(nb + cdiv(nb, CS_SLAB)) * c * sizeof(float);
}
extern "C" int gs_pixel_norm_bwd_fused_bias(const void* g, const void* x, const void* addend, void* gx, float* gb, int64_t p, int c, float eps, int pre_act,
                                            int post_act, int accumulate, int dtype, void* ws, size_t ws_bytes, void* stream) {
    GS_CHECK_ARG(pn_act_ok(pre_act) && pn_act_ok(post_act), "pixel_norm_bwd_fused_bias: bad activation %d / %d", pre_act, post_act);
    GS_CHECK_ARG(p > 0 && c >= 4 && c <= 1024 && (c & (c - 1)) == 0 && gb && g && x && gx, "pixel_norm_bwd_fused_bias: bad args (c=%d)", c);
    const bool partials_only = (accumulate & GS_SUM_PARTIALS) != 0;
    accumulate &= 1;
    const int nb = pixel_norm_grid((long)p, c, dtype == GS_F32 ? 4 : 8, true);
    if (ws_bytes < (partials_only ? (size_t)nb * c * sizeof(float) : gs_pixel_norm_bwd_bias_workspace_bytes(p, c, dtype)))
        return fail(GS_ERR_WORKSPACE, "pixel_norm_bwd_fused_bias: workspace too small");
    hipStream_t st = as_stream(stream);
    float* part = (float*)ws;
    GS_DISPATCH_DTYPE(dtype, (pixel_norm_launch_t<T, 1, true>(g, x, nullptr, gx, (long)p, c, eps, post_act, pre_act, addend, nullptr, st, part)));
    GS_CHECK_LAUNCH();
    if (partials_only) return 0;
    return channel_sum_finalize(part, gb, nb, c, accumulate, st);
}
extern "C" int gs_bias_partial_rows(int producer, int64_t p, int c, int dtype) {
    if (p <= 0 || c <= 0) return 0;
    const bool act_fast = !((c & 3) != 0 || c > 1024 || 256 % (c >> 2) != 0);
    switch (producer) {
        case GS_BIAS_FROM_CHANNEL_SUM: return (p <= 64 && c >= 256) ? 0 : channel_sum_parts(p, c);
        case GS_BIAS_FROM_ACT_BWD: return (!act_fast && p <= 64 && c >= 256) ? 0 : channel_sum_parts(p, c);
        case GS_BIAS_FROM_PIXEL_NORM_BWD: return (c >= 4 && c <= 1024 && (c & (c - 1)) == 0) ? pixel_norm_grid((long)p, c, dtype == GS_F32 ? 4 : 8, true) : 0;
        default: return 0;
    }
}
extern "C" int gs_pixel_norm_bwd_bwd_fused(const void* gg, const void* g, const void* x, void* out, void* out_g, int64_t p, int c, float eps, int pre_act,
                                           int dtype, void* stream) {
    GS_CHECK_ARG(pn_act_ok(pre_act), "pixel_norm_bwd_bwd_fused: bad activation %d", pre_act);
    return pixel_norm_launch(2, gg, g, x, out, p, c, eps, dtype, stream, 0, pre_act, nullptr, out_g);
}

extern "C" int gs_upscale2d(const void* x, void* y, int n, int h, int w, int c, int fy, int fx, float scale, int dtype, void* stream) {
    GS_CHECK_ARG(n > 0 && h > 0 && w > 0 && c > 0 && fy > 0 && fx > 0, "upscale2d: bad args");
    const long total = (long)n * h * fy * w * fx * c;
    GS_DISPATCH_DTYPE(dtype, hipLaunchKernelGGL((upscale_kernel<T>), dim3(ew_grid(total)), dim3(256), 0, as_stream(stream),
                                                (const T*)x, (T*)y, n, h, w, c, fy, fx, scale));
    GS_CHECK_LAUNCH();
    return 0;
}

extern "C" int gs_blocksum2d(const void* x, void* y, int n, int h, int w, int c, int fy, int fx, float scale, int dtype, void* stream) {
    GS_CHECK_ARG(n > 0 && c > 0 && fy > 0 && fx > 0 && h % fy == 0 && w % fx == 0, "blocksum2d: bad args");
    const long total = (long)n * (h / fy) * (w / fx) * c;
    hipStream_t st = as_stream(stream);
    if (fy * fx >= 32) {
        GS_DISPATCH_DTYPE(dtype, hipLaunchKernelGGL((blocksum_kernel<T>), dim3(ew_grid(total * 64)), dim3(256), 0, st, (const T*)x, (T*)y, n, h, w, c, fy, fx, scale));
    } else {
        GS_DISPATCH_DTYPE(dtype, hipLaunchKernelGGL((blocksum_small_kernel<T>), dim3(ew_grid(total)), dim3(256), 0, st, (const T*)x, (T*)y, n, h, w, c, fy, fx, scale));
    }
    GS_CHECK_LAUNCH();
    return 0;
}

extern "C" size_t gs_sumsq_rows_workspace_bytes(int rows) { return (size_t)(rows > 0 ? rows : 0) * SSQ_CHUNKS * sizeof(float); }

extern "C" int gs_sumsq_rows(const void* x, float* out, int rows, int64_t cols, int dtype, void* ws, size_t ws_bytes, void* stream) {
    GS_CHECK_ARG(rows > 0 && cols > 0, "sumsq_rows: bad args");
    if (ws_bytes < gs_sumsq_rows_workspace_bytes(rows)) return fail(GS_ERR_WORKSPACE, "sumsq_rows: workspace too small");
    float* part = (float*)ws;
    GS_DISPATCH_DTYPE(dtype, hipLaunchKernelGGL((sumsq_rows_kernel<T>), dim3(SSQ_CHUNKS, rows), dim3(256), 0, as_stream(stream), (const T*)x, part, (long)cols));
    GS_CHECK_LAUNCH();
    hipLaunchKernelGGL(sumsq_rows_final_kernel, dim3(rows), dim3(64), 0, as_stream(stream), part, out);
    GS_CHECK_LAUNCH();
// ... 67 lines not shown
```

### gansynth_amd/functional.py

```python
import contextlib
import itertools

import torch
from torch.autograd.function import once_differentiable

_NODE_SEQ = itertools.count(1 << 40)


def _number_node(out):
    t = out[0] if isinstance(out, (tuple, list)) and out else out
    fn = getattr(t, "grad_fn", None) if isinstance(t, torch.Tensor) else None
    if fn is not None and hasattr(fn, "_set_sequence_nr"):
        fn._set_sequence_nr(next(_NODE_SEQ))


class Function(torch.autograd.Function):

    @classmethod
    def apply(cls, *args, **kwargs):
        out = super().apply(*args, **kwargs)
        _number_node(out)
        return out


# ... 64 lines not shown
class _ConvKind(object):

    def __init__(self, ksize, stride):
        self.ksize, self.stride = ksize, stride

    def fwd(self, x, w, alpha):
        return _K().conv2d_fwd(x, w, self.ksize, self.stride, alpha)

    def fwd_bias_act(self, x, w, bias, alpha, act):
        return _K().conv2d_fwd_bias_act(x, w, bias, self.ksize, self.stride, alpha, act)

    def fwd_mask(self, x, w, alpha, mask, mask_act):
        K = _K()
        if hasattr(K, "conv2d_fwd_mask"):
            return K.conv2d_fwd_mask(x, w, self.ksize, self.stride, alpha, mask, mask_act)
        return K.act_bwd(self.fwd(x, w, alpha), mask, mask_act)

    def fwd_bias_act_norm(self, x, w, bias, alpha, act, eps, want_z):
        K = _K()
        if hasattr(K, "conv2d_fwd_bias_act_norm"):
            return K.conv2d_fwd_bias_act_norm(x, w, bias, self.ksize, self.stride, alpha, act, eps, want_z=want_z)
        z = self.fwd_bias_act(x, w, bias, alpha, act)
        return z, K.pixel_norm_fwd(z, eps)

    def bwd_data(self, gy, w, x_shape, alpha):
        return _K().conv2d_bwd_data(gy, w, x_shape, self.ksize, self.stride, alpha)

    def bwd_data_mask(self, gy, w, x_shape, alpha, mask, mask_act):
        return _K().conv2d_bwd_data(gy, w, x_shape, self.ksize, self.stride, alpha, mask=mask, mask_act=mask_act)

    def bwd_data_pnbwd(self, gy, w, x_shape, alpha, z, eps, act, addend):
        return _K().conv2d_bwd_data_pnbwd(gy, w, x_shape, self.ksize, self.stride, alpha, z, eps, act, addend=addend)

    def bwd_data_pnbwd_is_fused(self, x_shape, co, dtype):
        K = _K()
        return hasattr(K, "bwd_data_pnbwd_is_fused") and K.bwd_data_pnbwd_is_fused(x_shape, co, self.ksize, self.stride, False, dtype)

    def fwd_pnbwdbwd(self, x, w, alpha, g, z, eps, act):
        return _K().conv2d_fwd_pnbwdbwd(x, w, self.ksize, self.stride, alpha, g, z, eps, act)

    def fwd_pnbwdbwd_is_fused(self, x_shape, co, dtype):
        K = _K()
        return hasattr(K, "fwd_pnbwdbwd_is_fused") and K.fwd_pnbwdbwd_is_fused(x_shape, co, self.ksize, self.stride, False, dtype)

    bias_in_wgrad = True

    def bwd_weight(self, x, gy, alpha, out=None, bias_out=None):
        return _K().conv2d_bwd_weight(x, gy, self.ksize, self.stride, alpha, out=out, bias_out=bias_out)


class _ConvTransposeKind(object):

    def fwd(self, x, w, alpha):
        return _K().conv2d_transpose_fwd(x, w, alpha)

    def fwd_bias_act(self, x, w, bias, alpha, act):
        return _K().conv2d_transpose_fwd_bias_act(x, w, bias, alpha, act)

    def fwd_bias_act_norm(self, x, w, bias, alpha, act, eps, want_z):
        K = _K()
        if hasattr(K, "conv2d_transpose_fwd_bias_act_norm"):
            return K.conv2d_transpose_fwd_bias_act_norm(x, w, bias, alpha, act, eps, want_z=want_z)
        z = self.fwd_bias_act(x, w, bias, alpha, act)
        return z, K.pixel_norm_fwd(z, eps)

    def bwd_data(self, gy, w, x_shape, alpha):
        return _K().conv2d_transpose_bwd_data(gy, w, alpha)

    def bwd_data_pnbwd(self, gy, w, x_shape, alpha, z, eps, act, addend):
        return _K().conv2d_transpose_bwd_data_pnbwd(gy, w, alpha, z, eps, act, addend=addend)

    def bwd_data_pnbwd_is_fused(self, x_shape, co, dtype):
        K = _K()
        return hasattr(K, "bwd_data_pnbwd_is_fused") and K.bwd_data_pnbwd_is_fused(x_shape, co, 3, 2, True, dtype)

    def fwd_pnbwdbwd(self, x, w, alpha, g, z, eps, act):
        return _K().conv2d_transpose_fwd_pnbwdbwd(x, w, alpha, g, z, eps, act)

    def fwd_pnbwdbwd_is_fused(self, x_shape, co, dtype):
        K = _K()
        return hasattr(K, "fwd_pnbwdbwd_is_fused") and K.fwd_pnbwdbwd_is_fused(x_shape, co, 3, 2, True, dtype)

    def bwd_weight(self, x, gy, alpha, out=None):
        return _K().conv2d_transpose_bwd_weight(x, gy, alpha, out=out)


class _DenseKind(object):

    def fwd(self, x, w, alpha):
        return _K().dense_fwd(x, w, alpha)

    def fwd_bias_act(self, x, w, bias, alpha, act):
        if hasattr(_K(), "dense_fwd_bias_act"):
            return _K().dense_fwd_bias_act(x, w, bias, alpha, act)
        return _K().bias_act_fwd(_K().dense_fwd(x, w, alpha), bias, act)

    def bwd_data(self, gy, w, x_shape, alpha):
        return _K().dense_bwd_data(gy, w, alpha)

    def bwd_weight(self, x, gy, alpha, out=None):
        return _K().dense_bwd_weight(x, gy, alpha, out=out)


class _DenseFlatKind(object):

    def fwd(self, x, w, alpha):
        return _K().dense_fwd_nhwc(x, w, alpha)

    def fwd_bias_act(self, x, w, bias, alpha, act):
# ... 141 lines not shown
        ctx.save_for_backward(x, w)
        return kind.fwd(x, w, alpha)

    @staticmethod
    def backward(ctx, gy):
        x, w = ctx.saved_tensors
        gx = _BilinearBwdData.apply(gy, w, x.shape, ctx.kind, ctx.alpha) if ctx.needs_input_grad[0] else None
        gw = None
        if ctx.needs_input_grad[1] and _want_params():
            tgt = _accum_target(ctx.wref)
            if tgt is None:
                tgt = _slice_target(ctx.wref, x, gy, ctx.kind)
            if tgt is not None:
                ctx.kind.bwd_weight(x, gy, ctx.alpha, out=tgt)
            else:
                gw = _BilinearBwdWeight.apply(x, gy, ctx.kind, ctx.alpha).to(w.dtype)
        return gx, gw, None, None


class _BilinearBwdData(Function):

    @staticmethod
    def forward(ctx, gy, w, x_shape, kind, alpha, sole_consumer=False):
        ctx.kind, ctx.alpha, ctx.wref = kind, alpha, w
        ctx.sole_consumer = bool(sole_consumer)
        ctx.save_for_backward(gy, w)
        up = gy.grad_fn
        ctx._gs_up = up if (isinstance(up, _BwdDataMasked._backward_cls) and not _want_params() and hasattr(kind, "fwd_mask") and not _NO_PREMASK_GRAPH2) else None
        return kind.bwd_data(gy, w, x_shape, alpha)

    @staticmethod
    def backward(ctx, ggx):
        gy, w = ctx.saved_tensors
        g_gy = None
        if ctx.needs_input_grad[0]:
            pn = gy.grad_fn if (_FUSE_NORM_BWD2 and ctx.sole_consumer and not torch.is_grad_enabled() and hasattr(ctx.kind, "fwd_pnbwdbwd")) else None
            if (pn is not None and isinstance(pn, _PnActBwd._backward_cls) and pn.needs_input_grad[0] and pn.needs_input_grad[1]
                    and ctx.kind.fwd_pnbwdbwd_is_fused(tuple(ggx.shape), gy.shape[1], gy.dtype)):
                g, z = pn.saved_tensors
                g_z, g_gy = ctx.kind.fwd_pnbwdbwd(ggx, w, ctx.alpha, g, z, pn.eps, pn.act)
                if _CHECK_FUSION:
                    _check_fused("fwd_pnbwdbwd", (g_z, g_gy), _K().pixel_norm_bwd_bwd(ctx.kind.fwd(ggx, w, ctx.alpha), g, z, pn.eps, pre_act=pn.act, with_g=True))
                pn._gs_done = (g_gy.data_ptr(), g_z)
            elif ctx._gs_up is not None and not torch.is_grad_enabled():
                up = ctx._gs_up
                g_gy = ctx.kind.fwd_mask(ggx, w, ctx.alpha, up.saved_tensors[2], up.act)
                if _CHECK_FUSION:
                    _check_fused("fwd_mask", g_gy, _K().act_bwd(ctx.kind.fwd(ggx, w, ctx.alpha), up.saved_tensors[2], up.act))
                up._gs_gg_premasked = g_gy.data_ptr()
            else:
                g_gy = _Bilinear.apply(ggx, w, ctx.kind, ctx.alpha)
        g_w = None
        if ctx.needs_input_grad[1]:
            tgt = _accum_target(ctx.wref)
            if tgt is None:
                tgt = _slice_target(ctx.wref, ggx, gy, ctx.kind)
            if tgt is not None:
                ctx.kind.bwd_weight(ggx, gy, ctx.alpha, out=tgt)
            else:
                g_w = _BilinearBwdWeight.apply(ggx, gy, ctx.kind, ctx.alpha).to(w.dtype)
        return g_gy, g_w, None, None, None, None


class _BwdDataMasked(Function):

    @staticmethod
    def forward(ctx, gy, w, x, kind, alpha, act):
        if act != ACT_LRELU:
            raise NotImplementedError("_BwdDataMasked: piecewise-linear activations only")
        ctx.kind, ctx.alpha, ctx.act, ctx.wref = kind, alpha, act, w
        ctx.save_for_backward(gy, w, x)
        up = gy.grad_fn
        ctx._gs_up = up if (isinstance(up, _BwdDataMasked._backward_cls) and not _want_params() and hasattr(kind, "fwd_mask") and not _NO_PREMASK_GRAPH2) else None
        ctx._gs_gg_premasked = None
        return kind.bwd_data_mask(gy, w, x.shape, alpha, x, act)

    @staticmethod
    def backward(ctx, gg):
        gy, w, x = ctx.saved_tensors
        pre, ctx._gs_gg_premasked = ctx._gs_gg_premasked, None
        if pre is not None and pre != gg.data_ptr():
            _handoff_broken("activation mask of the R1 chain in the producing conv")
        if pre is not None and not torch.is_grad_enabled():
            t = gg
        else:
            t = _ActBwd.apply(gg, x, ctx.act)
        up = ctx._gs_up
        if up is not None and ctx.needs_input_grad[0] and not torch.is_grad_enabled():
            g_gy = ctx.kind.fwd_mask(t, w, ctx.alpha, up.saved_tensors[2], up.act)
            if _CHECK_FUSION:
                _check_fused("fwd_mask", g_gy, _K().act_bwd(ctx.kind.fwd(t, w, ctx.alpha), up.saved_tensors[2], up.act))
            up._gs_gg_premasked = g_gy.data_ptr()
        else:
            g_gy = _Bilinear.apply(t, w, ctx.kind, ctx.alpha) if ctx.needs_input_grad[0] else None
# ... 48 lines not shown
        ctx.wref, ctx.bref = w, bias
        ctx.in_act = in_act
        ctx.input_normed = bool(input_normed)
        ctx._gs_act_out = act
        ctx._gs_premasked = None
        z = kind.fwd_bias_act(x, w, bias, alpha, act)
        _tap(z, act)
        ctx.save_for_backward(x, w, z)
        return z

    @staticmethod
    def backward(ctx, gz):
        x, w, z = ctx.saved_tensors
        want_w = ctx.needs_input_grad[1] and _want_params()
        want_b = ctx.has_bias and ctx.needs_input_grad[2] and _want_params()
        act = ACT_NONE if _take_premasked(ctx, gz) else ctx.act

        def data_grad(gy):
            if not ctx.needs_input_grad[0]:
                return None
            if _PARAMS_ONLY and x.grad_fn is None and not torch.is_grad_enabled():
                return None
            if _FUSE_NORM_BWD and ctx.input_normed and not torch.is_grad_enabled() and hasattr(ctx.kind, "bwd_data_pnbwd"):
                pn = x.grad_fn
                if (isinstance(pn, _ConvBiasActNorm._backward_cls) and pn.act in (ACT_NONE, ACT_LRELU)
                        and ctx.kind.bwd_data_pnbwd_is_fused(tuple(x.shape), gy.shape[1], gy.dtype)):
                    z_prev = pn.saved_tensors[2]
                    gz_prev = _GZ.pop(z_prev.data_ptr(), None)
                    gx_ = ctx.kind.bwd_data_pnbwd(gy, w, tuple(x.shape), ctx.alpha, z_prev, pn.eps, pn.act, gz_prev)
                    if _CHECK_FUSION:
                        _check_fused("bwd_data_pnbwd", gx_, _K().pixel_norm_bwd(ctx.kind.bwd_data(gy, w, tuple(x.shape), ctx.alpha), z_prev, pn.eps, act=pn.act, addend=gz_prev))
                    pn._gs_fused = (gx_.data_ptr(), gz_prev is not None)
                    return gx_
            prod = _premask_producer(x, ctx.in_act, differentiable=True) if hasattr(ctx.kind, "bwd_data_mask") else None
            if prod is None:
                return _BilinearBwdData.apply(gy, w, x.shape, ctx.kind, ctx.alpha)
            if torch.is_grad_enabled():
                gx_ = _BwdDataMasked.apply(gy, w, x, ctx.kind, ctx.alpha, ctx.in_act)
            else:
                gx_ = ctx.kind.bwd_data_mask(gy, w, x.shape, ctx.alpha, x, ctx.in_act)
            prod._gs_premasked = gx_.data_ptr()
            return gx_

        if want_b and want_w and getattr(ctx.kind, "bias_in_wgrad", False):
            tw, tb = _accum_target(ctx.wref), _accum_target(ctx.bref)
            if tw is not None and tb is not None:
                gy = _ActBwd.apply(gz, z, act) if act != ACT_NONE else gz
                gx = data_grad(gy)
                ctx.kind.bwd_weight(x, gy, ctx.alpha, out=tw, bias_out=tb)
                return gx, None, None, None, None, None, None, None
        gy, gb = _bias_act_backward(gz, z if act != ACT_NONE else None, act, ctx.bref if want_b else None, want_b)
        gx = data_grad(gy)
        gw = None
        if want_w:
            tgt = _accum_target(ctx.wref)
            if tgt is not None:
                ctx.kind.bwd_weight(x, gy, ctx.alpha, out=tgt)
            else:
                gw = _BilinearBwdWeight.apply(x, gy, ctx.kind, ctx.alpha).to(w.dtype)
        return gx, gw, gb, None, None, None, None, None


class _PnActBwd(Function):

    @staticmethod
    def forward(ctx, g, z, eps, act):
        if act != ACT_LRELU:
            raise NotImplementedError("_PnActBwd: piecewise-linear activations only (the tanh head has no pixel norm)")
        ctx.eps, ctx.act = eps, act
        ctx._gs_done = None
        ctx.save_for_backward(g, z)
        return _K().pixel_norm_bwd(g, z, eps, act=act)

    @staticmethod
    @once_differentiable
    def backward(ctx, gg):
        g, z = ctx.saved_tensors
        done, ctx._gs_done = ctx._gs_done, None
        if ctx.needs_input_grad[0] and ctx.needs_input_grad[1]:
            if done is not None and gg.data_ptr() != done[0]:
                _handoff_broken("second-order norm gradients in the forward-on-cotangent conv")
            if done is not None:
                g_g, g_z = gg, done[1]
            else:
                g_z, g_g = _K().pixel_norm_bwd_bwd(gg, g, z, ctx.eps, pre_act=ctx.act, with_g=True)
            if _FUSE_NORM_BWD:
                _GZ[z.data_ptr()] = g_z
            return g_g, g_z, None, None
        if done is not None:
            _handoff_broken("second-order norm gradients in the forward-on-cotangent conv")
        g_g = _K().pixel_norm_bwd(gg, z, ctx.eps, pre_act=ctx.act) if ctx.needs_input_grad[0] else None
        g_z = _K().pixel_norm_bwd_bwd(gg, g, z, ctx.eps, pre_act=ctx.act) if ctx.needs_input_grad[1] else None
        return g_g, g_z, None, None


_FUSE_NORM_EPILOGUE = not config.flag("GS_NO_NORM_EPILOGUE")
_FUSE_NORM_BWD = not config.flag("GS_NO_NORM_BWD_EPILOGUE")
_FUSE_NORM_BWD2 = not config.flag("GS_NO_NORM_BWD2_EPILOGUE")

_GZ = {}


def reset_fusion_state():
    _GZ.clear()


def _handoff_broken(what):
    raise RuntimeError("gansynth_amd.functional: fused hand-off '%s' was prepared but the node received another tensor -- the single-consumer "
                       "promise of the wiring (networks.py: input_normed / input_activation, functional: sole_consumer) does not hold" % what)


_CHECK_FUSION = config.flag("GS_CHECK_FUSION")


def _check_fused(what, got, ref):
    if torch.cuda.is_available() and torch.cuda.is_current_stream_capturing():
        return
    for g, r in zip(got if isinstance(got, (tuple, list)) else (got,), ref if isinstance(ref, (tuple, list)) else (ref,)):
        scale = float(r.float().abs().max()) + 1e-30
        err = float((g.float() - r.float()).abs().max()) / scale
        tol = 1e-4 if g.dtype == torch.float32 else 4e-2
        if not err <= tol:
            raise RuntimeError("GS_CHECK_FUSION: %s differs from its unfused definition by %.3e of the tensor's scale" % (what, err))

_NORM_BWD_BIAS = not config.flag("GS_NO_NORM_BWD_BIAS")


class _ConvBiasActNorm(Function):

    @staticmethod
    def forward(ctx, x, w, bias, kind, alpha, act, eps, input_normed=False):
        ctx.kind, ctx.alpha, ctx.act, ctx.eps, ctx.has_bias = kind, alpha, act, eps, bias is not None
        ctx.wref, ctx.bref = w, bias
        ctx.input_normed = bool(input_normed)
        ctx._gs_fused = None
        ctx.set_materialize_grads(False)
        keep = any(ctx.needs_input_grad)
        want_z = keep or activation_tap.active is not None
        if _FUSE_NORM_EPILOGUE:
            z, y = kind.fwd_bias_act_norm(x, w, bias, alpha, act, eps, want_z)
        else:
            z = kind.fwd_bias_act(x, w, bias, alpha, act)
            y = _K().pixel_norm_fwd(z, eps)
        if want_z:
            _tap(z, act)
        if keep:
            ctx.save_for_backward(x, w, z)
        return y, z

    @staticmethod
    def backward(ctx, g_y, g_z):
        x, w, z = ctx.saved_tensors
        want_w = ctx.needs_input_grad[1] and _want_params()
        want_b = ctx.has_bias and ctx.needs_input_grad[2] and _want_params()
        if torch.is_grad_enabled():
            gy = _PnActBwd.apply(g_y, z, ctx.eps, ctx.act) if g_y is not None else None
            if g_z is not None:
                extra = _ActBwd.apply(g_z, z, ctx.act)
                gy = extra if gy is None else gy + extra
            sole = g_y is not None and g_z is None and not want_w and not want_b
            gx = _BilinearBwdData.apply(gy, w, x.shape, ctx.kind, ctx.alpha, sole) if ctx.needs_input_grad[0] else None
            gw = _BilinearBwdWeight.apply(x, gy, ctx.kind, ctx.alpha).to(w.dtype) if want_w else None
            gb = _ChannelSum.apply(gy) if want_b else None
            return gx, gw, gb, None, None, None, None, None
        tw = _accum_target(ctx.wref) if want_w else None
        tb = _accum_target(ctx.bref) if want_b else None
        bias_done = False
        fused, ctx._gs_fused = ctx._gs_fused, None
        if fused is not None and (g_y is None or g_y.data_ptr() != fused[0]):
            _handoff_broken("previous block's norm backward in the data-gradient conv")
        if fused is not None:
            gy = g_y
            if g_z is not None and not fused[1]:
                gy = _K().axpby(gy, _K().act_bwd(g_z, z, ctx.act), 1.0, 1.0)
        elif g_y is None:
            gy = _K().act_bwd(g_z, z, ctx.act)
        elif (tb is not None and not getattr(ctx.kind, "bias_in_wgrad", False) and _NORM_BWD_BIAS and getattr(_K(), "norm_bwd_sums_bias", False)
              and _K().norm_bwd_bias_ok(z.shape[1], z.dtype)):
            gy = _K().pixel_norm_bwd(g_y, z, ctx.eps, act=ctx.act, addend=g_z, bias_out=tb)
            bias_done = True
        else:
            gy = _K().pixel_norm_bwd(g_y, z, ctx.eps, act=ctx.act, addend=g_z)
        gx = None
        if ctx.needs_input_grad[0]:
            prod = x.grad_fn if (_FUSE_NORM_BWD and ctx.input_normed and hasattr(ctx.kind, "bwd_data_pnbwd")) else None
            if (prod is not None and isinstance(prod, _ConvBiasActNorm._backward_cls) and prod.act in (ACT_NONE, ACT_LRELU)
                    and ctx.kind.bwd_data_pnbwd_is_fused(tuple(x.shape), gy.shape[1], gy.dtype)):
                z_prev = prod.saved_tensors[2]
                gz_prev = _GZ.pop(z_prev.data_ptr(), None)
                gx = ctx.kind.bwd_data_pnbwd(gy, w, tuple(x.shape), ctx.alpha, z_prev, prod.eps, prod.act, gz_prev)
                if _CHECK_FUSION:
                    _check_fused("bwd_data_pnbwd", gx, _K().pixel_norm_bwd(ctx.kind.bwd_data(gy, w, tuple(x.shape), ctx.alpha), z_prev, prod.eps, act=prod.act, addend=gz_prev))
                prod._gs_fused = (gx.data_ptr(), gz_prev is not None)
            else:
# ... 651 lines not shown
```

### gansynth_amd/kernels.py

```python
import contextlib
import ctypes
import os

import numpy as np
import torch

from . import config
from . import _lib
from ._lib import GS_BF16, GS_F32

CL = torch.channels_last


def _dt(t):
    if t.dtype == torch.float32:
        return GS_F32
    if t.dtype == torch.bfloat16:
        return GS_BF16
    raise TypeError(f"unsupported activation dtype {t.dtype}")


def _act(x):
    if x.dim() == 4:
        return x if x.is_contiguous(memory_format=CL) else x.contiguous(memory_format=CL)
# ... 22 lines not shown


def _bits_wanted(ref, co, act):
    return _MASK_BITS and act == _lib.ACT_LRELU and ref.dtype == torch.bfloat16 and co % 32 == 0


def _has_bits(t):
    return (_MASK_BITS and t.dtype == torch.bfloat16 and t.dim() == 4 and t.shape[1] % 32 == 0 and t.storage_offset() == 0
            and t.untyped_storage().nbytes() == t.numel() * 2 + t.numel() // 8)


def _mask_act(mask, mask_act):
    return _lib.ACT_LRELU_BITS if (mask_act == _lib.ACT_LRELU and _has_bits(mask)) else int(mask_act)


def _stream():
    return ctypes.c_void_p(torch.cuda.current_stream().cuda_stream)


_POISON = config.flag("GS_DEBUG_POISON_WS")


def _ws(nbytes, device):
    if _POISON:
        return torch.full((max(int(nbytes), 256),), 0xFF, dtype=torch.uint8, device=device)
    return torch.empty(max(int(nbytes), 256), dtype=torch.uint8, device=device)


def _rows_cols(x):
    if x.dim() == 4:
        n, c, h, w = x.shape
        return n * h * w, c
    return x.shape[0], x.shape[1]


def note_mix_table(table, rows, length, total):
    if len(table) == 0:
        raise ValueError("note_mix: the table is empty")
    if int(total) <= 0:
        raise ValueError(f"note_mix: total must be positive (got {total})")
    checked = []
    for i, entry in enumerate(table):
        if len(entry) != 5:
            raise ValueError(f"note_mix: note {i} has {len(entry)} fields, not (onset, hold, release, row, gain)")
        onset, hold, release, row, gain = entry
        for name, v in (("onset", onset), ("hold", hold), ("release", release), ("row", row)):
            if not isinstance(v, (int, np.integer)) or isinstance(v, bool):
                raise ValueError(f"note_mix: note {i} field '{name}' must be an integer (got {v!r})")
        if not 0 <= onset < total:
            raise ValueError(f"note_mix: note {i} field 'onset' = {onset} is outside the clip [0, {total})")
        if not 1 <= hold <= length:
            raise ValueError(f"note_mix: note {i} field 'hold' = {hold} is outside [1, {length}]")
        if not 0 <= release <= length - hold:
            raise ValueError(f"note_mix: note {i} field 'release' = {release} is outside [0, {length} - hold = {length - hold}]")
        if not 0 <= row < rows:
            raise ValueError(f"note_mix: note {i} field 'row' = {row} is outside [0, {rows})")
        if isinstance(gain, bool) or not isinstance(gain, (int, float, np.floating, np.integer)) or not np.isfinite(gain):
            raise ValueError(f"note_mix: note {i} field 'gain' must be a finite number (got {gain!r})")
        checked.append((int(onset), int(hold), int(release), int(row), float(gain)))
    order = sorted(range(len(checked)), key=lambda i: (checked[i][0], i))
    return (_lib.GsMixNote * len(checked))(*[_lib.GsMixNote(*checked[i]) for i in order])


class HipKernels(object):
    def __init__(self):
        self.lib = _lib.load()
# ... 336 lines not shown
        y = _empty_like_act(shape, x)
        z = _empty_like_act(shape, x) if want_z else None
        self._conv_fwd(x, w, bias, act, ksize, stride, transposed, alpha, z, y, eps)
        return z, y

    def conv2d_transpose_fwd_bias_act_norm(self, x, w, bias, alpha, act, eps, want_z=True):
        return self._fwd_bias_act_norm(x, w, bias, 3, 2, True, alpha, act, eps, want_z)

    def conv2d_bwd_data(self, gy, w, x_shape, ksize, stride, alpha, mask=None, mask_act=0):
        return self._bwd_data(gy, w, x_shape, ksize, stride, False, alpha, mask, mask_act)

    def _bwd_data(self, gy, w, x_shape, ksize, stride, transposed, alpha, mask=None, mask_act=0):
        gy, w = _act(gy), _f32c(w)
        n, ci, h, wd = x_shape
        gx = _empty_like_act((n, ci, h, wd), gy)
        c, ws = self._conv(_lib.CONV_BWD_DATA, w, alpha, _dt(gy), n, ci, h, wd, w.shape[3], ksize, stride, transposed)
        mp = None
        if mask is not None:
            mask = _act(mask)
            assert mask.shape == gx.shape and mask.dtype == gx.dtype
            mp = mask.data_ptr()
        _lib.check(self.lib.gs_conv_bwd_data(c, gy.data_ptr(), w.data_ptr(), mp, _mask_act(mask, mask_act) if mask is not None else 0, gx.data_ptr(), _stream()),
                   "gs_conv_bwd_data")
        return gx

    def _is_fused(self, query, x_shape, co, ksize, stride, transposed, dtype):
        n, ci, h, wd = (int(v) for v in x_shape)
        dt = GS_F32 if dtype == torch.float32 else GS_BF16
        return bool(query(_lib.GsConv(n, h, wd, ci, int(co), int(ksize), int(stride), 1 if transposed else 0, dt)))

    def fwd_pnbwdbwd_is_fused(self, x_shape, co, ksize, stride, transposed, dtype):
        return self._is_fused(self.lib.gs_conv_fwd_pnbwdbwd_is_fused, x_shape, co, ksize, stride, transposed, dtype)

    def conv2d_fwd_pnbwdbwd(self, x, w, ksize, stride, alpha, g, z, eps, act):
        return self._fwd_pnbwdbwd(x, w, ksize, stride, False, alpha, g, z, eps, act)

    def _fwd_pnbwdbwd(self, x, w, ksize, stride, transposed, alpha, g, z, eps, act):
        x, w, g, z = _act(x), _f32c(w), _act(g), _act(z)
        n, ci, h, wd = x.shape
        out_g = _empty_like_act(self._out_shape(x, w.shape[3], stride, transposed), x)
        assert g.shape == out_g.shape == z.shape and g.dtype == x.dtype == z.dtype
        out_z = torch.empty_like(out_g)
        c, ws = self._conv(_lib.CONV_FWD, w, alpha, _dt(x), n, ci, h, wd, w.shape[3], ksize, stride, transposed)
        _lib.check(self.lib.gs_conv_fwd_pnbwdbwd(c, x.data_ptr(), w.data_ptr(), g.data_ptr(), z.data_ptr(), int(act), float(eps), out_g.data_ptr(), out_z.data_ptr(),
                                                 _stream()), "gs_conv_fwd_pnbwdbwd")
        return out_z, out_g

    def conv2d_transpose_fwd_pnbwdbwd(self, x, w, alpha, g, z, eps, act):
        return self._fwd_pnbwdbwd(x, w, 3, 2, True, alpha, g, z, eps, act)

    def bwd_data_pnbwd_is_fused(self, x_shape, co, ksize, stride, transposed, dtype):
        return self._is_fused(self.lib.gs_conv_bwd_data_pnbwd_is_fused, x_shape, co, ksize, stride, transposed, dtype)

    def conv2d_bwd_data_pnbwd(self, gy, w, x_shape, ksize, stride, alpha, z, eps, act, addend=None):
        return self._bwd_data_pnbwd(gy, w, x_shape, ksize, stride, False, alpha, z, eps, act, addend)

    def _bwd_data_pnbwd(self, gy, w, x_shape, ksize, stride, transposed, alpha, z, eps, act, addend):
        gy, w, z = _act(gy), _f32c(w), _act(z)
        n, ci, h, wd = x_shape
        assert tuple(z.shape) == (n, ci, h, wd) and z.dtype == gy.dtype
        gx = _empty_like_act((n, ci, h, wd), gy)
        c, ws = self._conv(_lib.CONV_BWD_DATA, w, alpha, _dt(gy), n, ci, h, wd, w.shape[3], ksize, stride, transposed)
        ap = None
        if addend is not None:
            addend = _match(addend, z)
            ap = addend.data_ptr()
        _lib.check(self.lib.gs_conv_bwd_data_pnbwd(c, gy.data_ptr(), w.data_ptr(), z.data_ptr(), ap, int(act), float(eps), gx.data_ptr(), _stream()),
                   "gs_conv_bwd_data_pnbwd")
        return gx

    def conv2d_transpose_bwd_data_pnbwd(self, gy, w, alpha, z, eps, act, addend=None):
        n, _, h2, w2 = gy.shape
        return self._bwd_data_pnbwd(gy, w, (n, w.shape[2], h2 // 2, w2 // 2), 3, 2, True, alpha, z, eps, act, addend)

    def conv2d_bwd_weight(self, x, gy, ksize, stride, alpha, out=None, bias_out=None):
        return self._bwd_weight(x, gy, ksize, stride, False, alpha, out, bias_out)

    def _bwd_weight(self, x, gy, ksize, stride, transposed, alpha, out, bias_out):
        x, gy = _act(x), _act(gy)
        n, ci, h, wd = x.shape
        co = gy.shape[1]
        gw = torch.empty((ksize, ksize, ci, co), dtype=torch.float32, device=x.device) if out is None else out
        if bias_out is not None:
            assert out is not None and bias_out.dtype == torch.float32 and bias_out.is_contiguous()
        if out is not None and self._pending is not None:
            self._defer_wgrad(("convT" if transposed else "conv", out.data_ptr(), ksize, stride, float(alpha), tuple(x.shape[1:]), tuple(gy.shape[1:]), x.dtype),
                              x, gy, out, bias_out)
            return gw
        assert out is None or transposed or out.is_contiguous(), "a channel-slice target needs deferred gradients (wgrad_slice_target_ok)"
        c, ws = self._conv(_lib.CONV_BWD_WEIGHT, None, alpha, _dt(x), n, ci, h, wd, co, ksize, stride, transposed, device=x.device)
        with self._adds_into(out, bias_out):
            _lib.check(self.lib.gs_conv_bwd_weight(c, x.data_ptr(), gy.data_ptr(), gw.data_ptr(), None if bias_out is None else bias_out.data_ptr(),
                                                   0 if out is None else 1, _stream()), "gs_conv_bwd_weight")
        return gw

# ... 208 lines not shown
        x = _act(x)
        p, c = _rows_cols(x)
        y = torch.empty_like(x)
        _lib.check(self.lib.gs_pixel_norm_fwd(x.data_ptr(), y.data_ptr(), p, c, float(eps), _dt(x), _stream()), "gs_pixel_norm_fwd")
        return y

    norm_bwd_sums_bias = True

    def norm_bwd_bias_ok(self, c, dtype=torch.float32):
        return self.lib.gs_bias_partial_rows(_lib.BIAS_FROM_PIXEL_NORM_BWD, 1, int(c), GS_F32 if dtype == torch.float32 else GS_BF16) > 0

    def pixel_norm_bwd(self, g, x, eps, act=0, pre_act=0, addend=None, bias_out=None):
        x = _act(x)
        g = _match(g, x)
        p, c = _rows_cols(x)
        gx = torch.empty_like(x)
        ap = None
        if addend is not None:
            addend = _match(addend, x)
            ap = addend.data_ptr()
        if bias_out is not None:
            assert bias_out.dtype == torch.float32 and bias_out.is_contiguous() and bias_out.numel() == c
            part = self._partial_rows(_lib.BIAS_FROM_PIXEL_NORM_BWD, p, c, _dt(x), bias_out)
            ws = part if part is not None else _ws(self.lib.gs_pixel_norm_bwd_bias_workspace_bytes(p, c, _dt(x)), x.device)
            with self._adds_into(bias_out if part is None else None):
                _lib.check(self.lib.gs_pixel_norm_bwd_fused_bias(g.data_ptr(), x.data_ptr(), ap, gx.data_ptr(), bias_out.data_ptr(), p, c, float(eps), int(pre_act),
                                                                 int(act), 1 | (_lib.SUM_PARTIALS if part is not None else 0), _dt(x), ws.data_ptr(),
                                                                 ws.numel() * ws.element_size(), _stream()), "gs_pixel_norm_bwd_fused_bias")
            return gx
        _lib.check(self.lib.gs_pixel_norm_bwd_fused(g.data_ptr(), x.data_ptr(), ap, gx.data_ptr(), p, c, float(eps), int(pre_act), int(act), _dt(x),
                                                    _stream()), "gs_pixel_norm_bwd_fused")
        return gx

    def pixel_norm_bwd_bwd(self, gg, g, x, eps, pre_act=0, with_g=False):
        x = _act(x)
        gg, g = _match(gg, x), _match(g, x)
        p, c = _rows_cols(x)
        out = torch.empty_like(x)
        out_g = torch.empty_like(x) if with_g else None
        _lib.check(self.lib.gs_pixel_norm_bwd_bwd_fused(gg.data_ptr(), g.data_ptr(), x.data_ptr(), out.data_ptr(), None if out_g is None else out_g.data_ptr(),
                                                        p, c, float(eps), int(pre_act), _dt(x), _stream()), "gs_pixel_norm_bwd_bwd_fused")
        return (out, out_g) if with_g else out

    def upscale2d(self, x, fy, fx, scale):
        x = _act(x)
        n, c, h, w = x.shape
        y = _empty_like_act((n, c, h * fy, w * fx), x)
        _lib.check(self.lib.gs_upscale2d(x.data_ptr(), y.data_ptr(), n, h, w, c, fy, fx, float(scale), _dt(x), _stream()), "gs_upscale2d")
        return y

    def blocksum2d(self, x, fy, fx, scale):
        x = _act(x)
        n, c, h, w = x.shape
        y = _empty_like_act((n, c, h // fy, w // fx), x)
        _lib.check(self.lib.gs_blocksum2d(x.data_ptr(), y.data_ptr(), n, h, w, c, fy, fx, float(scale), _dt(x), _stream()), "gs_blocksum2d")
        return y

    def batch_stddev_fwd(self, x, eps, sub=1):
        x = _act(x)
        n, c, h, w = x.shape
        y = _empty_like_act((n, 1, h, w), x)
        m, es = n // sub, x.element_size()
        for s in range(sub):
            _lib.check(self.lib.gs_batch_stddev_fwd(x.data_ptr() + s * m * c * h * w * es, y.data_ptr() + s * m * h * w * es, m, h * w, c, float(eps), _dt(x),
                                                    _stream()), "gs_batch_stddev_fwd")
        return y

    def batch_stddev_bwd(self, gy, x, eps, addend=None, sub=1):
        x = _act(x)
        n, c, h, w = x.shape
        gy = _act(gy.to(x.dtype))
        gx = torch.empty_like(x)
# ... 534 lines not shown
```

### include/gansynth_hip.h

```cpp
#ifndef GANSYNTH_HIP_H
#define GANSYNTH_HIP_H

#include <stddef.h>
#include <stdint.h>

#ifdef __cplusplus
extern "C" {
#endif

enum { GS_F32 = 0, GS_BF16 = 1 };
enum { GS_OK = 0, GS_ERR_ARG = -1, GS_ERR_HIP = -2, GS_ERR_UNSUPPORTED = -3, GS_ERR_WORKSPACE = -4 };
enum { GS_ACT_NONE = 0, GS_ACT_LRELU = 1, GS_ACT_TANH = 2 };
enum { GS_ACT_LRELU_BITS = 5, GS_ACT_WRITE_BITS = 16 };
enum { GS_CONV_FWD = 0, GS_CONV_BWD_DATA = 1, GS_CONV_BWD_WEIGHT = 2 };

const char* gs_last_error(void);
int gs_version(void);
int gs_init(void);
int gs_streams_create(int n, void** streams);
int gs_streams_destroy(int n, void** streams);

int gs_prof_enable(int on);
int gs_prof_collect(int* launches, double* total_ms, double* total_flops);
int gs_prof_roofline(double peak_tflops, double peak_gbps, double* total_bytes, double* roof_ms, double* roof_ms_hbm_bound);
int gs_prof_records(int max_records, int* n, double* ms, double* flops, double* bytes, int* desc);

#define GS_COMM_ID_BYTES 128
typedef struct gs_comm gs_comm;
int gs_comm_available(void);
int gs_comm_unique_id(void* id128);
int gs_comm_init(gs_comm** out, int rank, int world, const void* id128);
int gs_comm_destroy(gs_comm* comm);
int gs_comm_count(gs_comm* comm, int* ranks);
int gs_allreduce_sum_f32(gs_comm* comm, float* data, int64_t count, void* stream);
int gs_comm_set_marker_us(gs_comm* comm, double us);
int gs_broadcast_f32(gs_comm* comm, float* data, int64_t count, int root, void* stream);

typedef struct GsConv {
    int32_t n, h, w;
    int32_t ci, co, ksize, stride;
    int32_t transposed;
    int32_t dtype, w_prepared;
    float alpha;
    void* ws;
    size_t ws_bytes;
} GsConv;
size_t gs_conv_workspace_bytes(const GsConv* c, int which);
int gs_conv_fwd(const GsConv* c, const void* x, const float* w_hwio, const float* bias, int act, void* y, void* y_norm, float eps, void* stream);
int gs_pack_act_bits(void* z, int64_t p, int c, int dtype, void* stream);
int gs_conv_fwd_mask(const GsConv* c, const void* x, const float* w_hwio, const void* mask, int mask_act, void* y, void* stream);
int gs_conv_bwd_data(const GsConv* c, const void* gy, const float* w_hwio, const void* mask, int mask_act, void* gx, void* stream);
int gs_conv_bwd_data_pnbwd(const GsConv* c, const void* gy, const float* w_hwio, const void* z, const void* addend, int act, float eps, void* gx, void* stream);
int gs_conv_bwd_data_pnbwd_is_fused(const GsConv* c);
int gs_conv_fwd_pnbwdbwd(const GsConv* c, const void* x, const float* w_hwio, const void* g, const void* z, int act, float eps, void* out_g, void* out_z, void* stream);
int gs_conv_fwd_pnbwdbwd_is_fused(const GsConv* c);
int gs_conv_bwd_weight(const GsConv* c, const void* x, const void* gy, float* gw_hwio, float* gb, int accumulate, void* stream);
int gs_conv_igemm_config(int mode, int n, int hb, int wb, int ic, int oc, int dtype, int want, int* out_cfg);
int gs_conv_igemm_table(int index, int* out11);

#define GS_WGRAD_MAX_SOURCES 4
typedef struct GsWgradJob {
    const void* x[GS_WGRAD_MAX_SOURCES];
    const void* gy[GS_WGRAD_MAX_SOURCES];
    int32_t n[GS_WGRAD_MAX_SOURCES];
    int32_t nsrc;
    uint32_t bias_mask;
    float* gw;
    float* gb;
    int32_t h, w, ci, co, ksize, stride, transposed;
    float alpha;
    int32_t accumulate, dtype;
    int32_t gw_ci_stride;
} GsWgradJob;
size_t gs_conv_wgrad_jobs_workspace_bytes(const GsWgradJob* jobs, int njobs);
int gs_conv_wgrad_jobs(const GsWgradJob* jobs, int njobs, void* ws, size_t ws_bytes, void* stream);
int gs_wgrad_cu_cap(int cap);

enum { GS_PREP_CONV_FWD = 0, GS_PREP_CONV_BWD_DATA = 1, GS_PREP_CONVT_FWD = 2, GS_PREP_CONVT_BWD_DATA = 3 };
typedef struct GsPrepDesc {
    const float* w_hwio;
    void* ws;
    int32_t map, ci, co, ksize, stride, dtype;
} GsPrepDesc;
int gs_weight_prep_batch(const GsPrepDesc* descs, int n, void* stream);

size_t gs_dense_fwd_workspace_bytes(int b, int in, int out);
int gs_dense_fwd(const void* x, const float* w, void* y, int b, int in, int out, float alpha, int dtype,
                 void* ws, size_t ws_bytes, void* stream);
// ... 15 lines not shown
int gs_embedding_bwd(const int64_t* idx, const void* gy, float* gw, int b, int rows, int units, float alpha, int dtype, void* stream);

int gs_bias_act_fwd(const void* x, const float* bias, void* y, int64_t p, int c, int act, int dtype, void* stream);
int gs_act_bwd(const void* g, const void* y, void* gx, int64_t numel, int act, int dtype, void* stream);
int gs_units_bias_act_to_nhwc(const void* y, const float* bias, const void* mask, void* z, int n, int c, int hw, int act, int dtype, void* stream);
int gs_nhwc_act_bwd_to_units(const void* g, const void* z, void* gu, int n, int c, int hw, int act, int dtype, void* stream);

int gs_act_bwd_bias(const void* g, const void* y, void* gx, float* gb, int64_t p, int c, int act, int accumulate, int dtype,
                    void* ws, size_t ws_bytes, void* stream);
int gs_tanh_bwd_bwd(const void* gg, const void* g, const void* y, void* out, int64_t numel, int dtype, void* stream);
size_t gs_channel_sum_workspace_bytes(int64_t p, int c);
int gs_channel_sum(const void* g, float* out, int64_t p, int c, int accumulate, int dtype, void* ws, size_t ws_bytes, void* stream);
#define GS_SUM_PARTIALS 2
enum { GS_BIAS_FROM_CHANNEL_SUM = 0, GS_BIAS_FROM_ACT_BWD = 1, GS_BIAS_FROM_PIXEL_NORM_BWD = 2 };
typedef struct GsFoldJob {
    const float* part;
    float* out;
    int32_t nparts, c;
    int32_t accumulate;
    int32_t reserved;
} GsFoldJob;
int gs_bias_partial_rows(int producer, int64_t p, int c, int dtype);
size_t gs_channel_fold_batch_workspace_bytes(const GsFoldJob* jobs, int njobs);
int gs_channel_fold_batch(const GsFoldJob* jobs, int njobs, void* ws, size_t ws_bytes, void* stream);

int gs_pixel_norm_fwd(const void* x, void* y, int64_t p, int c, float eps, int dtype, void* stream);
int gs_pixel_norm_bwd_fused(const void* g, const void* x, const void* addend, void* gx, int64_t p, int c, float eps, int pre_act, int post_act,
                            int dtype, void* stream);
size_t gs_pixel_norm_bwd_bias_workspace_bytes(int64_t p, int c, int dtype);
int gs_pixel_norm_bwd_fused_bias(const void* g, const void* x, const void* addend, void* gx, float* gb, int64_t p, int c, float eps, int pre_act,
                                 int post_act, int accumulate, int dtype, void* ws, size_t ws_bytes, void* stream);
int gs_pixel_norm_bwd_bwd_fused(const void* gg, const void* g, const void* x, void* out, void* out_g, int64_t p, int c, float eps, int pre_act,
                                int dtype, void* stream);

int gs_upscale2d(const void* x, void* y, int n, int h, int w, int c, int fy, int fx, float scale, int dtype, void* stream);
int gs_blocksum2d(const void* x, void* y, int n, int h, int w, int c, int fy, int fx, float scale, int dtype, void* stream);

int gs_batch_stddev_fwd(const void* x, void* y, int b, int hw, int c, float eps, int dtype, void* stream);
int gs_batch_stddev_bwd(const void* gy, const void* x, const void* addend, void* gx, int b, int hw, int c, float eps, int dtype, void* stream);
int gs_batch_stddev_bwd_bwd(const void* ggx, const void* gy, const void* x, void* ggy, void* gx2,
                            int b, int hw, int c, float eps, int dtype, void* stream);

int gs_axpby(const void* a, const void* b, void* out, int64_t numel, float ca, float cb, int dtype, void* stream);
int gs_axpby_dev(const void* a, const void* b, void* out, int64_t numel, const float* coef, int ia, int ib, int dtype, void* stream);

size_t gs_sumsq_rows_workspace_bytes(int rows);
int gs_sumsq_rows(const void* x, float* out, int rows, int64_t cols, int dtype, void* ws, size_t ws_bytes, void* stream);
int gs_row_scale(const void* x, const float* s, float alpha, void* out, int rows, int64_t cols, int dtype, void* stream);

int gs_gan_d_loss(const void* real_logits, const void* fake_logits, const void* labels, const float* penalty, float penalty_weight, int n, int c,
                  float* loss, void* g_real, void* g_fake, float* g_penalty, int dtype, void* stream);
int gs_gan_g_loss(const void* fake_logits, const void* labels, const float* sumsq, float weight, float eps, int n, int c, float* loss,
                  void* g_fake, float* g_sumsq, int dtype, void* stream);

int gs_adam_tf_step(float* p, const float* g, float* m, float* v, int64_t numel, float lr_t, float beta1,
                    float beta2, float eps, float grad_scale, void* stream);
int gs_adam_tf_step_zero_grad(float* p, float* g, float* m, float* v, int64_t numel, float lr_t, float beta1,
                              float beta2, float eps, float grad_scale, void* stream);
int gs_adam_tf_step_dev(float* p, float* g, float* m, float* v, int64_t numel, const float* lr_t_dev, float beta1,
                        float beta2, float eps, float grad_scale, int zero_grad, void* stream);

typedef struct gs_spectral_plan gs_spectral_plan;
int gs_spectral_plan_create(gs_spectral_plan** plan, int frame_length, int frame_step, int time_steps,
                            const float* mel_dense , const float* mel_pinv );
int gs_spectral_plan_destroy(gs_spectral_plan* plan);
int gs_stft_fwd(const gs_spectral_plan* plan, const float* wave, int batch, int wave_len, int front_pad,
// ... 74 lines not shown
```

Baseline: 1673 images/sec.

## Fuse previous-block norm backward into mode-seeking first-order data-gradient convs

Adds a stats form of the data-gradient conv with pixel-norm-backward epilogue, used in the mode-seeking term's first-order (graph-building) pass. It also writes the per-pixel mean of z·g. A matching 'u' variant of the second-order forward conv and norm kernel consumes that saved mean instead of recomputing it from g. The aim is to remove the separate norm-backward kernel launches and their extra activation passes in the double-backward path. The cost is a small float32 per-pixel buffer, more epilogue register pressure, and extra autograd plumbing.

```diff
diff --git a/gansynth_amd/_lib.py b/gansynth_amd/_lib.py
--- a/gansynth_amd/_lib.py
+++ b/gansynth_amd/_lib.py
@@ -46,8 +46,10 @@
     "gs_conv_bwd_data": (I, [C, P, P, P, I, P, P]),
     "gs_conv_bwd_data_pnbwd": (I, [C, P, P, P, P, I, F, P, P]),
     "gs_conv_bwd_data_pnbwd_is_fused": (I, [C]),
+    "gs_conv_bwd_data_pnbwd_stats": (I, [C, P, P, P, I, F, P, P, P]),
     "gs_conv_fwd_pnbwdbwd": (I, [C, P, P, P, P, I, F, P, P, P]),
     "gs_conv_fwd_pnbwdbwd_is_fused": (I, [C]),
+    "gs_conv_fwd_pnbwdbwd_u": (I, [C, P, P, P, P, P, I, F, P, P, P]),
     "gs_conv_bwd_weight": (I, [C, P, P, P, P, I, P]),
     "gs_conv_wgrad_jobs_workspace_bytes": (Z, [P, I]),
     "gs_conv_wgrad_jobs": (I, [P, I, P, Z, P]),
@@ -82,6 +84,7 @@
     "gs_pixel_norm_bwd_bias_workspace_bytes": (Z, [L, I, I]),
     "gs_pixel_norm_bwd_fused_bias": (I, [P, P, P, P, P, L, I, F, I, I, I, I, P, Z, P]),
     "gs_pixel_norm_bwd_bwd_fused": (I, [P, P, P, P, P, L, I, F, I, I, P]),
+    "gs_pixel_norm_bwd_bwd_fused_u": (I, [P, P, P, P, P, P, L, I, F, I, I, P]),
     "gs_upscale2d": (I, [P, P, I, I, I, I, I, I, F, I, P]),
     "gs_blocksum2d": (I, [P, P, I, I, I, I, I, I, F, I, P]),
     "gs_batch_stddev_fwd": (I, [P, P, I, I, I, F, I, P]),
diff --git a/gansynth_amd/config.py b/gansynth_amd/config.py
--- a/gansynth_amd/config.py
+++ b/gansynth_amd/config.py
@@ -39,6 +39,7 @@
     "GS_NO_NORM_EPILOGUE": ("ablation", "no pixel norm in conv epilogues"),
     "GS_NO_NORM_BWD_EPILOGUE": ("ablation", "no previous-block norm backward in data-gradient epilogues"),
     "GS_NO_NORM_BWD2_EPILOGUE": ("ablation", "no second-order norm kernel in the forward-on-cotangent conv"),
+    "GS_NO_NORM_BWD_GRAPH_EPILOGUE": ("ablation", "no previous-block norm backward in the data-gradient epilogues of the mode-seeking term's first-order pass"),
     "GS_NO_NORM_BWD_BIAS": ("ablation", "bias sums outside the norm's backward"),
     "GS_NO_MASK_BITS": ("ablation", "leaky-relu masks read as the bf16 activations themselves, not as the sign bits stored behind them"),
     "GS_NO_PREMASK": ("ablation", "activation derivative never folded into the consuming data-gradient kernel"),
diff --git a/gansynth_amd/csrc/conv_api.hip b/gansynth_amd/csrc/conv_api.hip
--- a/gansynth_amd/csrc/conv_api.hip
+++ b/gansynth_amd/csrc/conv_api.hip
@@ -11,12 +11,14 @@
 int igemm_table(int index, int* out);
 extern "C" int gs_pixel_norm_bwd_bwd_fused(const void* gg, const void* g, const void* x, void* out, void* out_g, int64_t p, int c, float eps, int pre_act,
                                            int dtype, void* stream);
+extern "C" int gs_pixel_norm_bwd_bwd_fused_u(const void* gg, const void* u, const float* zg_mean, const void* x, void* out, void* out_g, int64_t p, int c, float eps,
+                                             int pre_act, int dtype, void* stream);
 bool wgrad_mfma_supported(int ic, int oc, int dtype);
 size_t igemm_prep_bytes(int ic, int oc, int dtype);
 int run_igemm(int mode, int variant, const void* x, const float* w_hwio, void* y, int N, int Hi, int Wi, int ICk,
               int OCk, int w_ci, int w_co, int Hb, int Wb, float alpha, const float* bias, int act, int dtype, int w_prepared,
               void* ws, size_t ws_bytes, hipStream_t st, const void* mask = nullptr, int mask_act = 0, void* y2 = nullptr, float pn_eps = 0.f,
-              const void* addend = nullptr, int normbwd = 0);
+              const void* addend = nullptr, int normbwd = 0, float* zg = nullptr);
 extern "C" int gs_pixel_norm_bwd_fused(const void* g, const void* x, const void* addend, void* gx, int64_t p, int c, float eps, int pre_act, int post_act, int dtype,
                                        void* stream);
 size_t wgrad_mfma_bytes(int mode, int dtype, int N, int Hb, int Wb, int IC, int OC);
@@ -223,7 +225,8 @@
 
 template <typename T, int IC>
 __global__ __launch_bounds__(256) void thin_expand_pnbwd_kernel(const T* __restrict__ x, const float* __restrict__ wp, const T* __restrict__ z,
-                                                                const T* __restrict__ addend, T* __restrict__ y, long P, int OC, float alpha, float eps, int act) {
+                                                                const T* __restrict__ addend, T* __restrict__ y, long P, int OC, float alpha, float eps, int act,
+                                                                float* __restrict__ zg_out) {
     constexpr int WN = Wide<T>::N;
     const int groups = OC / WN;
     const int oc0 = (threadIdx.x % groups) * WN;
@@ -264,6 +267,7 @@
         szg = group_sum(szg, groups);
         const float r = rsqrtf(ssq * inv_c + eps);
         const float m = szg * inv_c * r * r;
+        if (zg_out && pix < P && threadIdx.x % groups == 0) zg_out[pix] = szg * inv_c;
         float out[WN];
 #pragma unroll
         for (int v = 0; v < WN; ++v) {
@@ -281,12 +285,12 @@
     return groups >= 1 && groups <= 64 && (groups & (groups - 1)) == 0;
 }
 static int run_thin_expand_pnbwd(const void* x, const float* wp, const void* z, const void* addend, void* y, long P, int ICk, int OCk, float alpha, float eps, int act,
-                                 int dtype, hipStream_t st) {
+                                 int dtype, hipStream_t st, float* zg_out = nullptr) {
     const int wn = dtype == GS_F32 ? 4 : 8;
     long nb = cdiv(P * (OCk / wn), 256);
     if (nb > 4096) nb = 4096;
     const unsigned grid = (unsigned)nb;
-#define GS_TEP(TT, ICV) hipLaunchKernelGGL((thin_expand_pnbwd_kernel<TT, ICV>), dim3(grid), dim3(256), 0, st, (const TT*)x, wp, (const TT*)z, (const TT*)addend, (TT*)y, P, OCk, alpha, eps, act)
+#define GS_TEP(TT, ICV) hipLaunchKernelGGL((thin_expand_pnbwd_kernel<TT, ICV>), dim3(grid), dim3(256), 0, st, (const TT*)x, wp, (const TT*)z, (const TT*)addend, (TT*)y, P, OCk, alpha, eps, act, zg_out)
 #define GS_TEP_ALL(TT) do { if (ICk == 1) GS_TEP(TT, 1); else if (ICk == 2) GS_TEP(TT, 2); else if (ICk == 3) GS_TEP(TT, 3); else GS_TEP(TT, 4); } while (0)
     GS_DISPATCH_DTYPE(dtype, GS_TEP_ALL(T));
 #undef GS_TEP_ALL
@@ -1151,16 +1155,26 @@
     return 0;
 }
 
-extern "C" int gs_conv_fwd_pnbwdbwd(const GsConv* c, const void* x, const float* w_hwio, const void* g, const void* z, int act, float eps, void* out_g, void* out_z,
-                                    void* stream) {
+static int conv_fwd_pnbwdbwd(const GsConv* c, const void* x, const float* w_hwio, const void* g, const float* zg_mean, const void* z, int act, float eps, void* out_g,
+                             void* out_z, void* stream) {
     if (int e = check_conv(c)) return e;
     GS_CHECK_ARG(g && z && out_g && out_z && (act == GS_ACT_NONE || act == GS_ACT_LRELU), "conv_fwd_pnbwdbwd: g, z and both outputs are required, activation none or leaky relu (got %d)", act);
     const ConvRole r = conv_role(*c, GS_CONV_FWD);
     if (c->ksize == 3 && igemm_supported(r.ICk, r.OCk, c->dtype))
         return run_igemm(r.mode, r.variant, x, w_hwio, out_g, c->n, r.Hi, r.Wi, r.ICk, r.OCk, c->ci, c->co, r.Hb, r.Wb, c->alpha, nullptr, GS_ACT_NONE, c->dtype, c->w_prepared, c->ws,
-                         c->ws_bytes, as_stream(stream), z, act, out_z, eps, g, 2);
+                         c->ws_bytes, as_stream(stream), z, act, out_z, eps, g, 2, const_cast<float*>(zg_mean));
     if (int e = gs_conv_fwd(c, x, w_hwio, nullptr, GS_ACT_NONE, out_g, nullptr, 0.f, stream)) return e;
+    if (zg_mean) return gs_pixel_norm_bwd_bwd_fused_u(out_g, g, zg_mean, z, out_z, out_g, (int64_t)c->n * r.Ho * r.Wo, c->co, eps, act, c->dtype, stream);
     return gs_pixel_norm_bwd_bwd_fused(out_g, g, z, out_z, out_g, (int64_t)c->n * r.Ho * r.Wo, c->co, eps, act, c->dtype, stream);
+}
+extern "C" int gs_conv_fwd_pnbwdbwd(const GsConv* c, const void* x, const float* w_hwio, const void* g, const void* z, int act, float eps, void* out_g, void* out_z,
+                                    void* stream) {
+    return conv_fwd_pnbwdbwd(c, x, w_hwio, g, nullptr, z, act, eps, out_g, out_z, stream);
+}
+extern "C" int gs_conv_fwd_pnbwdbwd_u(const GsConv* c, const void* x, const float* w_hwio, const void* u, const float* zg_mean, const void* z, int act, float eps,
+                                      void* out_g, void* out_z, void* stream) {
+    GS_CHECK_ARG(zg_mean, "conv_fwd_pnbwdbwd_u: zg_mean is required");
+    return conv_fwd_pnbwdbwd(c, x, w_hwio, u, zg_mean, z, act, eps, out_g, out_z, stream);
 }
 extern "C" int gs_conv_fwd_pnbwdbwd_is_fused(const GsConv* c) {
     if (check_conv(c) || c->ksize != 3 || !(c->transposed || c->stride == 1)) return 0;
@@ -1168,7 +1182,8 @@
     return igemm_norm_fused(r.mode, c->n, r.Hb, r.Wb, r.ICk, r.OCk, c->dtype, IGEMM_NORM_BWD2) ? 1 : 0;
 }
 
-extern "C" int gs_conv_bwd_data_pnbwd(const GsConv* c, const void* gy, const float* w_hwio, const void* z, const void* addend, int act, float eps, void* gx, void* stream) {
+static int conv_bwd_data_pnbwd(const GsConv* c, const void* gy, const float* w_hwio, const void* z, const void* addend, int act, float eps, void* gx, float* zg_mean,
+                               void* stream) {
     if (int e = check_conv(c)) return e;
     GS_CHECK_ARG(z && gx && (act == GS_ACT_NONE || act == GS_ACT_LRELU), "conv_bwd_data_pnbwd: z is required, activation none or leaky relu (got %d)", act);
     hipStream_t st = as_stream(stream);
@@ -1176,7 +1191,7 @@
     const bool epilogue_map = c->transposed || c->stride == 1;
     if (epilogue_map && c->ksize == 3 && igemm_supported(r.ICk, r.OCk, c->dtype))
         return run_igemm(r.mode, r.variant, gy, w_hwio, gx, c->n, r.Hi, r.Wi, r.ICk, r.OCk, c->ci, c->co, r.Hb, r.Wb, c->alpha, nullptr, GS_ACT_NONE, c->dtype, c->w_prepared, c->ws,
-                         c->ws_bytes, st, z, act, nullptr, eps, addend, 1);
+                         c->ws_bytes, st, z, act, nullptr, eps, addend, 1, zg_mean);
     if (c->stride == 1 && thin_expand_pnbwd_ok(c->ksize, r.ICk, r.OCk, c->dtype)) {
         const long total = (long)c->ci * c->co;
         if (c->ws_bytes < (size_t)total * 4) return fail(GS_ERR_WORKSPACE, "conv_bwd_data_pnbwd: workspace %zu < %zu", c->ws_bytes, (size_t)total * 4);
@@ -1185,10 +1200,20 @@
             hipLaunchKernelGGL((weight_prep_kernel<float>), dim3(cdiv(total, 256)), dim3(256), 0, st, w_hwio, wp, 1, c->ci, c->co, 1);
             GS_CHECK_LAUNCH();
         }
-        return run_thin_expand_pnbwd(gy, wp, z, addend, gx, (long)c->n * r.Ho * r.Wo, r.ICk, r.OCk, c->alpha, eps, act, c->dtype, st);
-    }
+        return run_thin_expand_pnbwd(gy, wp, z, addend, gx, (long)c->n * r.Ho * r.Wo, r.ICk, r.OCk, c->alpha, eps, act, c->dtype, st, zg_mean);
+    }
+    if (zg_mean) return fail(GS_ERR_UNSUPPORTED, "conv_bwd_data_pnbwd_stats: no one-launch form for this layer");
     if (int e = gs_conv_bwd_data(c, gy, w_hwio, nullptr, 0, gx, stream)) return e;
     return gs_pixel_norm_bwd_fused(gx, z, addend, gx, (int64_t)c->n * r.Ho * r.Wo, c->ci, eps, GS_ACT_NONE, act, c->dtype, stream);
+}
+extern "C" int gs_conv_bwd_data_pnbwd(const GsConv* c, const void* gy, const float* w_hwio, const void* z, const void* addend, int act, float eps, void* gx, void* stream) {
+    return conv_bwd_data_pnbwd(c, gy, w_hwio, z, addend, act, eps, gx, nullptr, stream);
+}
+extern "C" int gs_conv_bwd_data_pnbwd_stats(const GsConv* c, const void* gy, const float* w_hwio, const void* z, int act, float eps, void* gx, float* zg_mean,
+                                            void* stream) {
+    GS_CHECK_ARG(zg_mean, "conv_bwd_data_pnbwd_stats: zg_mean is required");
+    if (!gs_conv_bwd_data_pnbwd_is_fused(c)) return fail(GS_ERR_UNSUPPORTED, "conv_bwd_data_pnbwd_stats: no one-launch form for this layer");
+    return conv_bwd_data_pnbwd(c, gy, w_hwio, z, nullptr, act, eps, gx, zg_mean, stream);
 }
 extern "C" int gs_conv_bwd_data_pnbwd_is_fused(const GsConv* c) {
     if (check_conv(c) || !(c->transposed || c->stride == 1)) return 0;
diff --git a/gansynth_amd/csrc/conv_igemm.hip b/gansynth_amd/csrc/conv_igemm.hip
--- a/gansynth_amd/csrc/conv_igemm.hip
+++ b/gansynth_amd/csrc/conv_igemm.hip
@@ -7,6 +7,8 @@
                                        void* stream);
 extern "C" int gs_pixel_norm_bwd_bwd_fused(const void* gg, const void* g, const void* x, void* out, void* out_g, int64_t p, int c, float eps, int pre_act,
                                            int dtype, void* stream);
+extern "C" int gs_pixel_norm_bwd_bwd_fused_u(const void* gg, const void* u, const float* zg_mean, const void* x, void* out, void* out_g, int64_t p, int c, float eps,
+                                             int pre_act, int dtype, void* stream);
 
 namespace gs {
 
@@ -23,6 +25,8 @@
     void* y2;
     float pn_eps;
     const void* addend;
+    float* zg_out;
+    const float* zg_in;
     int normbwd;
     int* norm_pending;
     int N, Hi, Wi, IC, OC, Hb, Wb, tiles_x, tiles_y, nsp, noct, nch;
@@ -291,7 +295,8 @@
         typedef typename std::conditional<SZ == 4, float4, uint4>::type nvec_t;
         constexpr int NNV = SZ == 4 ? 4 : 2;
         nvec_t nz[NPIPE ? 2 : 1][A][NNV], nx[NPIPE ? 2 : 1][A][NNV];
-        auto norm_fetch = [&](int i, nvec_t (&zq)[A][NNV], nvec_t (&xq)[A][NNV]) __attribute__((always_inline)) {
+        float nm[NPIPE ? 2 : 1];
+        auto norm_fetch = [&](int i, nvec_t (&zq)[A][NNV], nvec_t (&xq)[A][NNV], float& mq) __attribute__((always_inline)) {
             constexpr int NPHB = MODE == MODE_T2 ? 4 : 1;
             const int b = i / NPHB, ph = i % NPHB;
             const int Ho = MODE == MODE_T2 ? 2 * Hb : Hb, Wo = MODE == MODE_T2 ? 2 * Wb : Wb;
@@ -305,6 +310,9 @@
 #else
             const long zbase = base;
 #endif
+            if constexpr (NORM == 3) {
+                if (p.zg_in) mq = p.zg_in[(gy < Hb && gx < Wb) ? ((long)n * Ho + oy) * Wo + ox : 0];
+            }
 #pragma unroll
             for (int a = 0; a < A; ++a)
 #pragma unroll
@@ -321,7 +329,7 @@
                 const int npiece = stage_pieces(itg);
                 if (issuer) issue_setup(itg);
                 if constexpr (NPIPE) {
-                    if (tg == NTG - 1 && ch == NCH - 1 && computer) norm_fetch(0, nz[0], nx[0]);
+                    if (tg == NTG - 1 && ch == NCH - 1 && computer) norm_fetch(0, nz[0], nx[0], nm[0]);
                 }
                 if constexpr (BITS) {
                     if (tg == NTG - 1 && ch == NCH - 1 && computer && p.mask_bits) {
@@ -540,7 +548,7 @@
                                 constexpr int EV = 16 / NV;
                                 const int cur = NPIPE ? ((b * NPH + ph) & 1) : 0;
                                 if constexpr (NPIPE) {
-                                    if (b * NPH + ph + 1 < B * NPH) norm_fetch(b * NPH + ph + 1, nz[(b * NPH + ph + 1) & 1], nx[(b * NPH + ph + 1) & 1]);
+                                    if (b * NPH + ph + 1 < B * NPH) norm_fetch(b * NPH + ph + 1, nz[(b * NPH + ph + 1) & 1], nx[(b * NPH + ph + 1) & 1], nm[(b * NPH + ph + 1) & 1]);
                                 } else {
                                     mask_fetch(off, inside, nz[0]);
                                     if (p.addend) {
@@ -593,6 +601,7 @@
                                 const float inv_c = 1.f / (float)(32 * A);
                                 const float r = rsqrtf(ssq * inv_c + p.pn_eps);
                                 const float m = szg * inv_c * r * r;
+                                if (p.zg_out && inside && !hi) p.zg_out[((long)n * Ho + oy) * Wo + ox] = szg * inv_c;
 #pragma unroll
                                 for (int a = 0; a < A; ++a)
 #pragma unroll
@@ -628,7 +637,7 @@
                                 constexpr int EV = 16 / NV;
                                 const int cur = NPIPE ? ((b * NPH + ph) & 1) : 0;
                                 if constexpr (NPIPE) {
-                                    if (b * NPH + ph + 1 < B * NPH) norm_fetch(b * NPH + ph + 1, nz[(b * NPH + ph + 1) & 1], nx[(b * NPH + ph + 1) & 1]);
+                                    if (b * NPH + ph + 1 < B * NPH) norm_fetch(b * NPH + ph + 1, nz[(b * NPH + ph + 1) & 1], nx[(b * NPH + ph + 1) & 1], nm[(b * NPH + ph + 1) & 1]);
                                 } else {
                                     mask_fetch(off, inside, nz[0]);
                                     const long base = inside ? off : 0;
@@ -637,7 +646,9 @@
 #pragma unroll
                                         for (int v = 0; v < NV; ++v)
                                             nx[0][a][v] = *reinterpret_cast<const mvec_t*>(reinterpret_cast<const T*>(p.addend) + base + a * 32 + v * (32 / NV) + hi * (16 / NV));
-                                }
+                                    if (p.zg_in) nm[0] = p.zg_in[inside ? ((long)n * Ho + oy) * Wo + ox : 0];
+                                }
+                                const bool uform = p.zg_in != nullptr;
                                 mvec_t (&zq)[A][NV] = nz[cur];
                                 mvec_t (&gq)[A][NV] = nx[cur];
                                 float hv[A][NV][EV], zv[A][NV][EV], gv[A][NV][EV];
@@ -677,17 +688,37 @@
 #pragma unroll
                                         for (int e = 0; e < EV; ++e) {
                                             const float zc = zv[a][v][e], gc = gv[a][v][e];
-                                            const float hc = hv[a][v][e] * mask_factor(zc);
+                                            const float tc = hv[a][v][e];
+                                            const float hc = tc * mask_factor(zc);
                                             hv[a][v][e] = hc;
-                                            ssq += zc * zc; shg += hc * gc; shz += hc * zc; szg += zc * gc;
+                                            ssq += zc * zc; shg += (uform ? tc : hc) * gc; shz += hc * zc;
+                                            if (!uform) szg += zc * gc;
                                         }
                                 }
                                 ssq = swap32_sum(ssq); shg = swap32_sum(shg);
-                                shz = swap32_sum(shz); szg = swap32_sum(szg);
+                                shz = swap32_sum(shz);
+                                if (!uform) szg = swap32_sum(szg);
                                 const float inv_c = 1.f / (float)(32 * A);
                                 const float r = rsqrtf(ssq * inv_c + p.pn_eps);
                                 const float r2 = r * r, r3 = r2 * r;
-                                const float ma = shg * inv_c, mb = shz * inv_c, mm = szg * inv_c;
+                                float ma = shg * inv_c, mm = szg * inv_c;
+                                const float mb = shz * inv_c;
+                                if (uform) {
+                                    const float rinv = (ssq * inv_c + p.pn_eps) * r;
+                                    mm = nm[cur];
+                                    ma = ma * rinv + r2 * mm * mb;
+                                    const float gz = r2 * mm;
+#pragma unroll
+                                    for (int a = 0; a < A; ++a)
+#pragma unroll
+                                        for (int v = 0; v < NV; ++v)
+#pragma unroll
+                                            for (int e = 0; e < EV; ++e) {
+                                                const float zc = zv[a][v][e];
+                                                const float im = (p.mask_act == GS_ACT_LRELU && !(zc > 0.f)) ? 5.f : 1.f;
+                                                gv[a][v][e] = gv[a][v][e] * (rinv * im) + gz * zc;
+                                            }
+                                }
                                 const float kz = 3.f * r3 * r2 * mb * mm - r3 * ma;
 #pragma unroll
                                 for (int a = 0; a < A; ++a)
@@ -817,6 +848,8 @@
                 q.mask_bits = reinterpret_cast<const unsigned char*>(adv(p.mask_bits, n0 * out_img / (8 * sizeof(T))));
                 q.bits_out = reinterpret_cast<unsigned char*>(const_cast<void*>(adv(p.bits_out, n0 * out_img / (8 * sizeof(T)))));
                 q.addend = adv(p.addend, n0 * out_img);
+                q.zg_out = reinterpret_cast<float*>(const_cast<void*>(adv(p.zg_out, n0 * out_img / (p.OC * sizeof(T)) * sizeof(float))));
+                q.zg_in = reinterpret_cast<const float*>(adv(p.zg_in, n0 * out_img / (p.OC * sizeof(T)) * sizeof(float)));
                 int pending = 0;
                 if (p.norm_pending) q.norm_pending = &pending;
                 if (int e = launch_igemm<T, MODE, A, B, TW, TG, RESIDENT, D, NORM, RB, SPEC, BITS>(q, st)) return e;
@@ -839,6 +872,8 @@
         p.mask = nullptr;
         p.addend = nullptr;
         p.y2 = nullptr;
+        p.zg_out = nullptr;
+        p.zg_in = nullptr;
     }
     if (NORM != 1 && NORM != 3 && p.y2) {
         if (!p.y) p.y = p.y2;
@@ -862,7 +897,8 @@
     if (grid >= 8) grid &= ~7L;
     const double flops = 2.0 * 9.0 * (double)p.N * p.Hb * p.Wb * p.IC * p.OC;
     const double out_px = (double)p.N * p.Hb * p.Wb * (MODE == MODE_T2 ? 4 : 1);
-    const double bytes = ((double)p.N * p.Hi * p.Wi * p.IC + out_px * p.OC * (1.0 + (p.mask ? (p.mask_bits ? 1.0 / 16.0 : 1.0) : 0.0) + (p.bits_out ? 1.0 / 16.0 : 0.0) + ((NORM == 1 && p.y) ? 1.0 : 0.0) + ((NORM == 2 && p.addend) ? 1.0 : 0.0) + (NORM == 3 ? 2.0 : 0.0)) + 9.0 * p.IC * p.OC) * sizeof(T);
+    const double bytes = ((double)p.N * p.Hi * p.Wi * p.IC + out_px * p.OC * (1.0 + (p.mask ? (p.mask_bits ? 1.0 / 16.0 : 1.0) : 0.0) + (p.bits_out ? 1.0 / 16.0 : 0.0) + ((NORM == 1 && p.y) ? 1.0 : 0.0) + ((NORM == 2 && p.addend) ? 1.0 : 0.0) + (NORM == 3 ? 2.0 : 0.0)) + 9.0 * p.IC * p.OC) * sizeof(T) +
+                         ((NORM == 2 && p.zg_out) || (NORM == 3 && p.zg_in) ? out_px * sizeof(float) : 0.0);
     const int reps = prof_reps();
     ProfScope ps(st, flops, bytes, MODE, p.N, p.Hb, p.Wb, p.IC, p.OC, p.mask ? 1 : 0, NORM ? 1 : 0, reps);
     for (int r = 0; r < reps; ++r) hipLaunchKernelGGL(kern, dim3((unsigned)grid), dim3(SPEC ? 512 : 256), lds, st, p);
@@ -1034,7 +1070,7 @@
 static int run_igemm_t(int mode, int variant, const void* x, const float* w_hwio, void* y, int N, int Hi, int Wi,
                        int ICk, int OCk, int w_ci, int w_co, int Hb, int Wb, float alpha, const float* bias, int act,
                        int w_prepared, void* ws, size_t ws_bytes, hipStream_t st, const void* mask, int mask_act, void* y2, float pn_eps,
-                       const void* addend, int normbwd) {
+                       const void* addend, int normbwd, float* zg) {
     const size_t need = (size_t)9 * w_ci * w_co * sizeof(T);
     if (ws_bytes < need) return fail(GS_ERR_WORKSPACE, "conv igemm: workspace %zu < %zu", ws_bytes, need);
     T* wp = reinterpret_cast<T*>(ws);
@@ -1061,6 +1097,8 @@
     int pending = 0;
     p.y2 = y2; p.pn_eps = pn_eps; p.norm_pending = &pending;
     p.addend = normbwd ? addend : nullptr; p.normbwd = normbwd;
+    if (zg && normbwd == 1) p.zg_out = zg;
+    if (zg && normbwd == 2) p.zg_in = zg;
     int rc;
     if (mode == MODE_S1) rc = dispatch_igemm<T, MODE_S1>(p, st);
     else if (mode == MODE_S2) rc = dispatch_igemm<T, MODE_S2>(p, st);
@@ -1069,8 +1107,10 @@
     GS_CHECK_LAUNCH();
     if (pending == 3) {
         const long px = (long)N * Hb * Wb * (mode == MODE_T2 ? 4 : 1);
+        if (zg) return gs_pixel_norm_bwd_bwd_fused_u(y, addend, zg, mask, y2, y, px, OCk, pn_eps, mask_act, sizeof(T) == 4 ? GS_F32 : GS_BF16, st);
         return gs_pixel_norm_bwd_bwd_fused(y, addend, mask, y2, y, px, OCk, pn_eps, mask_act, sizeof(T) == 4 ? GS_F32 : GS_BF16, st);
     }
+    if (pending == 2 && zg) return fail(GS_ERR_UNSUPPORTED, "conv igemm: mean(z g) on the side needs the fused pixel-norm backward epilogue, which this shape does not have");
     if (pending == 2) {
         const long px = (long)N * Hb * Wb * (mode == MODE_T2 ? 4 : 1);
         return gs_pixel_norm_bwd_fused(y, mask, addend, y, px, OCk, pn_eps, GS_ACT_NONE, mask_act, sizeof(T) == 4 ? GS_F32 : GS_BF16, st);
@@ -1086,9 +1126,9 @@
 
 int run_igemm(int mode, int variant, const void* x, const float* w_hwio, void* y, int N, int Hi, int Wi, int ICk,
               int OCk, int w_ci, int w_co, int Hb, int Wb, float alpha, const float* bias, int act, int dtype, int w_prepared,
-              void* ws, size_t ws_bytes, hipStream_t st, const void* mask, int mask_act, void* y2, float pn_eps, const void* addend, int normbwd) {
+              void* ws, size_t ws_bytes, hipStream_t st, const void* mask, int mask_act, void* y2, float pn_eps, const void* addend, int normbwd, float* zg) {
     GS_DISPATCH_DTYPE(dtype, return (run_igemm_t<T>(mode, variant, x, w_hwio, y, N, Hi, Wi, ICk, OCk, w_ci, w_co, Hb,
-                                                    Wb, alpha, bias, act, w_prepared, ws, ws_bytes, st, mask, mask_act, y2, pn_eps, addend, normbwd)));
+                                                    Wb, alpha, bias, act, w_prepared, ws, ws_bytes, st, mask, mask_act, y2, pn_eps, addend, normbwd, zg)));
 }
 
 }
diff --git a/gansynth_amd/csrc/elementwise.hip b/gansynth_amd/csrc/elementwise.hip
--- a/gansynth_amd/csrc/elementwise.hip
+++ b/gansynth_amd/csrc/elementwise.hip
@@ -378,7 +378,8 @@
 template <typename T, int MODE, int E, int P, int U, bool BS = false>
 __global__ __launch_bounds__(256) void pixel_norm_kernel(const T* __restrict__ a0, const T* __restrict__ a1, const T* __restrict__ a2,
                                                          T* __restrict__ out, long p, int c, float eps, int act, int pre,
-                                                         const T* __restrict__ addend, T* __restrict__ out2, float* __restrict__ bsum = nullptr) {
+                                                         const T* __restrict__ addend, T* __restrict__ out2, float* __restrict__ bsum = nullptr,
+                                                         const float* __restrict__ zg = nullptr) {
     const int vecs = c / E;
     const int L = vecs < 64 ? vecs : 64;
     const int rows_per_wave = 64 / L;
@@ -402,11 +403,13 @@
         long off[U];
         bool ok[U];
         float xv[U][P][E], av[U][P][E], bv[U][P][E];
+        float mz[U];
 #pragma unroll
         for (int u = 0; u < U; ++u) {
             const long row = row0 + u * nwaves * rows_per_wave + lane / L;
             ok[u] = row < p;
             off[u] = (ok[u] ? row : 0) * c + sub * E;
+            if (MODE == 2 && zg) mz[u] = zg[ok[u] ? row : 0];
 #pragma unroll
             for (int k = 0; k < P; ++k) {
                 pn_ld<T, E>(xbase + off[u] + k * L * E, xv[u][k]);
@@ -462,15 +465,29 @@
                 for (int k = 0; k < P; ++k)
 #pragma unroll
                     for (int e = 0; e < E; ++e) {
+                        const float raw = av[u][k][e];
                         av[u][k][e] *= dact(pre, xv[u][k][e]);
                         const float yv = xv[u][k][e] * r;
-                        sa += av[u][k][e] * bv[u][k][e];
+                        sa += (zg ? raw : av[u][k][e]) * bv[u][k][e];
                         sp += yv * av[u][k][e];
-                        sq += yv * bv[u][k][e];
+                        if (!zg) sq += yv * bv[u][k][e];
                     }
                 sa = group_sum(sa, L);
                 sp = group_sum(sp, L);
-                sq = group_sum(sq, L);
+                if (!zg) sq = group_sum(sq, L);
+                if (zg) {
+                    const float m = mz[u];
+                    const float rinv = (s * invc + eps) * r;
+                    sq = r * m * (float)c;
+                    sa = sa * rinv + r * m * sp;
+#pragma unroll
+                    for (int k = 0; k < P; ++k)
+#pragma unroll
+                        for (int e = 0; e < E; ++e) {
+                            const float im = (pre == GS_ACT_LRELU && !(xv[u][k][e] > 0.f)) ? 5.f : 1.f;
+                            bv[u][k][e] = bv[u][k][e] * (rinv * im) + r * r * m * xv[u][k][e];
+                        }
+                }
                 const float k0 = r * r * invc;
 #pragma unroll
                 for (int k = 0; k < P; ++k) {
@@ -826,14 +843,14 @@
 }
 template <typename T, int MODE, bool BS = false>
 static void pixel_norm_launch_t(const void* a0, const void* a1, const void* a2, void* out, long p, int c, float eps, int act, int pre, const void* addend,
-                                void* out2, hipStream_t st, float* bsum = nullptr) {
+                                void* out2, hipStream_t st, float* bsum = nullptr, const float* zg = nullptr) {
     constexpr int WN = Wide<T>::N;
     const int E = c % WN == 0 ? WN : 4;
     const int vecs = c / E, L = vecs < 64 ? vecs : 64, P = vecs / L;
     dim3 grid(pixel_norm_grid(p, c, WN, BS));
 #define GS_PN(EE, PP, UU)                                                                                                          \
     hipLaunchKernelGGL((pixel_norm_kernel<T, MODE, EE, PP, UU, BS>), grid, dim3(256), 0, st, (const T*)a0, (const T*)a1, (const T*)a2, (T*)out, p, c, eps, \
-                       act, pre, (const T*)addend, (T*)out2, bsum)
+                       act, pre, (const T*)addend, (T*)out2, bsum, zg)
     if (E == WN) {
         if (P == 1) GS_PN(WN, 1, 2); else if (P == 2) GS_PN(WN, 2, 1); else GS_PN(WN, 4, 1);
     } else {
@@ -842,13 +859,13 @@
 #undef GS_PN
 }
 static int pixel_norm_launch(int mode, const void* a0, const void* a1, const void* a2, void* out, int64_t p, int c, float eps, int dtype, void* stream, int act = 0,
-                             int pre = 0, const void* addend = nullptr, void* out2 = nullptr) {
+                             int pre = 0, const void* addend = nullptr, void* out2 = nullptr, const float* zg = nullptr) {
     GS_CHECK_ARG(p > 0 && c >= 4 && c <= 1024 && (c & (c - 1)) == 0, "pixel_norm: c=%d must be a power of two in [4,1024]", c);
     hipStream_t st = as_stream(stream);
     GS_DISPATCH_DTYPE(dtype, {
         if (mode == 0) pixel_norm_launch_t<T, 0>(a0, a1, a2, out, (long)p, c, eps, act, pre, addend, out2, st);
         else if (mode == 1) pixel_norm_launch_t<T, 1>(a0, a1, a2, out, (long)p, c, eps, act, pre, addend, out2, st);
-        else pixel_norm_launch_t<T, 2>(a0, a1, a2, out, (long)p, c, eps, act, pre, addend, out2, st);
+        else pixel_norm_launch_t<T, 2>(a0, a1, a2, out, (long)p, c, eps, act, pre, addend, out2, st, nullptr, zg);
     });
     GS_CHECK_LAUNCH();
     return 0;
@@ -897,6 +914,11 @@
     GS_CHECK_ARG(pn_act_ok(pre_act), "pixel_norm_bwd_bwd_fused: bad activation %d", pre_act);
     return pixel_norm_launch(2, gg, g, x, out, p, c, eps, dtype, stream, 0, pre_act, nullptr, out_g);
 }
+extern "C" int gs_pixel_norm_bwd_bwd_fused_u(const void* gg, const void* u, const float* zg_mean, const void* x, void* out, void* out_g, int64_t p, int c, float eps,
+                                             int pre_act, int dtype, void* stream) {
+    GS_CHECK_ARG(zg_mean && (pre_act == GS_ACT_NONE || pre_act == GS_ACT_LRELU), "pixel_norm_bwd_bwd_fused_u: zg_mean is required, activation none or leaky relu (got %d)", pre_act);
+    return pixel_norm_launch(2, gg, u, x, out, p, c, eps, dtype, stream, 0, pre_act, nullptr, out_g, zg_mean);
+}
 
 extern "C" int gs_upscale2d(const void* x, void* y, int n, int h, int w, int c, int fy, int fx, float scale, int dtype, void* stream) {
     GS_CHECK_ARG(n > 0 && h > 0 && w > 0 && c > 0 && fy > 0 && fx > 0, "upscale2d: bad args");
diff --git a/gansynth_amd/functional.py b/gansynth_amd/functional.py
--- a/gansynth_amd/functional.py
+++ b/gansynth_amd/functional.py
@@ -120,11 +120,16 @@
     def bwd_data_pnbwd(self, gy, w, x_shape, alpha, z, eps, act, addend):
         return _K().conv2d_bwd_data_pnbwd(gy, w, x_shape, self.ksize, self.stride, alpha, z, eps, act, addend=addend)
 
+    def bwd_data_pnbwd_graph(self, gy, w, x_shape, alpha, z, eps, act):
+        return _K().conv2d_bwd_data_pnbwd_graph(gy, w, x_shape, self.ksize, self.stride, alpha, z, eps, act)
+
     def bwd_data_pnbwd_is_fused(self, x_shape, co, dtype):
         K = _K()
         return hasattr(K, "bwd_data_pnbwd_is_fused") and K.bwd_data_pnbwd_is_fused(x_shape, co, self.ksize, self.stride, False, dtype)
 
-    def fwd_pnbwdbwd(self, x, w, alpha, g, z, eps, act):
+    def fwd_pnbwdbwd(self, x, w, alpha, g, z, eps, act, zg=None):
+        if zg is not None:
+            return _K().conv2d_fwd_pnbwdbwd(x, w, self.ksize, self.stride, alpha, g, z, eps, act, zg=zg)
         return _K().conv2d_fwd_pnbwdbwd(x, w, self.ksize, self.stride, alpha, g, z, eps, act)
 
     def fwd_pnbwdbwd_is_fused(self, x_shape, co, dtype):
@@ -158,11 +163,16 @@
     def bwd_data_pnbwd(self, gy, w, x_shape, alpha, z, eps, act, addend):
         return _K().conv2d_transpose_bwd_data_pnbwd(gy, w, alpha, z, eps, act, addend=addend)
 
+    def bwd_data_pnbwd_graph(self, gy, w, x_shape, alpha, z, eps, act):
+        return _K().conv2d_transpose_bwd_data_pnbwd_graph(gy, w, alpha, z, eps, act)
+
     def bwd_data_pnbwd_is_fused(self, x_shape, co, dtype):
         K = _K()
         return hasattr(K, "bwd_data_pnbwd_is_fused") and K.bwd_data_pnbwd_is_fused(x_shape, co, 3, 2, True, dtype)
 
-    def fwd_pnbwdbwd(self, x, w, alpha, g, z, eps, act):
+    def fwd_pnbwdbwd(self, x, w, alpha, g, z, eps, act, zg=None):
+        if zg is not None:
+            return _K().conv2d_transpose_fwd_pnbwdbwd(x, w, alpha, g, z, eps, act, zg=zg)
         return _K().conv2d_transpose_fwd_pnbwdbwd(x, w, alpha, g, z, eps, act)
 
     def fwd_pnbwdbwd_is_fused(self, x_shape, co, dtype):
@@ -370,34 +380,47 @@
     @staticmethod
     def backward(ctx, ggx):
         gy, w = ctx.saved_tensors
-        g_gy = None
-        if ctx.needs_input_grad[0]:
-            pn = gy.grad_fn if (_FUSE_NORM_BWD2 and ctx.sole_consumer and not torch.is_grad_enabled() and hasattr(ctx.kind, "fwd_pnbwdbwd")) else None
-            if (pn is not None and isinstance(pn, _PnActBwd._backward_cls) and pn.needs_input_grad[0] and pn.needs_input_grad[1]
-                    and ctx.kind.fwd_pnbwdbwd_is_fused(tuple(ggx.shape), gy.shape[1], gy.dtype)):
-                g, z = pn.saved_tensors
-                g_z, g_gy = ctx.kind.fwd_pnbwdbwd(ggx, w, ctx.alpha, g, z, pn.eps, pn.act)
-                if _CHECK_FUSION:
-                    _check_fused("fwd_pnbwdbwd", (g_z, g_gy), _K().pixel_norm_bwd_bwd(ctx.kind.fwd(ggx, w, ctx.alpha), g, z, pn.eps, pre_act=pn.act, with_g=True))
-                pn._gs_done = (g_gy.data_ptr(), g_z)
-            elif ctx._gs_up is not None and not torch.is_grad_enabled():
-                up = ctx._gs_up
-                g_gy = ctx.kind.fwd_mask(ggx, w, ctx.alpha, up.saved_tensors[2], up.act)
-                if _CHECK_FUSION:
-                    _check_fused("fwd_mask", g_gy, _K().act_bwd(ctx.kind.fwd(ggx, w, ctx.alpha), up.saved_tensors[2], up.act))
-                up._gs_gg_premasked = g_gy.data_ptr()
-            else:
-                g_gy = _Bilinear.apply(ggx, w, ctx.kind, ctx.alpha)
-        g_w = None
-        if ctx.needs_input_grad[1]:
-            tgt = _accum_target(ctx.wref)
-            if tgt is None:
-                tgt = _slice_target(ctx.wref, ggx, gy, ctx.kind)
-            if tgt is not None:
-                ctx.kind.bwd_weight(ggx, gy, ctx.alpha, out=tgt)
-            else:
-                g_w = _BilinearBwdWeight.apply(ggx, gy, ctx.kind, ctx.alpha).to(w.dtype)
+        g_gy, g_w = _bwd_data_backward(ctx, ggx, gy, w, ctx.needs_input_grad[0], ctx.needs_input_grad[1])
         return g_gy, g_w, None, None, None, None
+
+
+def _bwd_data_backward(ctx, ggx, gy, w, need_gy, need_w):
+    g_gy = None
+    if need_gy:
+        pn = gy.grad_fn if (_FUSE_NORM_BWD2 and ctx.sole_consumer and not torch.is_grad_enabled() and hasattr(ctx.kind, "fwd_pnbwdbwd")) else None
+        if (pn is not None and isinstance(pn, _PnActBwd._backward_cls) and pn.needs_input_grad[0] and pn.needs_input_grad[1]
+                and ctx.kind.fwd_pnbwdbwd_is_fused(tuple(ggx.shape), gy.shape[1], gy.dtype)):
+            g, z = pn.saved_tensors
+            g_z, g_gy = ctx.kind.fwd_pnbwdbwd(ggx, w, ctx.alpha, g, z, pn.eps, pn.act)
+            if _CHECK_FUSION:
+                _check_fused("fwd_pnbwdbwd", (g_z, g_gy), _K().pixel_norm_bwd_bwd(ctx.kind.fwd(ggx, w, ctx.alpha), g, z, pn.eps, pre_act=pn.act, with_g=True))
+            pn._gs_done = (g_gy.data_ptr(), g_z)
+        elif (pn is not None and isinstance(pn, _BwdDataPnActBwd._backward_cls) and (pn.needs_input_grad[0] or pn.needs_input_grad[1]) and pn.needs_input_grad[2]
+                and ctx.kind.fwd_pnbwdbwd_is_fused(tuple(ggx.shape), gy.shape[1], gy.dtype)):
+            gy_n, w_n, z, u, zg = pn.saved_tensors
+            g_z, g_gy = ctx.kind.fwd_pnbwdbwd(ggx, w, ctx.alpha, u, z, pn.eps, pn.act, zg=zg)
+            if _CHECK_FUSION:
+                _check_fused("fwd_pnbwdbwd (u, zg)", (g_z, g_gy), _K().pixel_norm_bwd_bwd(ctx.kind.fwd(ggx, w, ctx.alpha), pn.kind.bwd_data(gy_n, w_n, tuple(z.shape), pn.alpha),
+                                                                                          z, pn.eps, pre_act=pn.act, with_g=True))
+            pn._gs_done = (g_gy.data_ptr(), g_z)
+        elif ctx._gs_up is not None and not torch.is_grad_enabled():
+            up = ctx._gs_up
+            g_gy = ctx.kind.fwd_mask(ggx, w, ctx.alpha, up.saved_tensors[2], up.act)
+            if _CHECK_FUSION:
+                _check_fused("fwd_mask", g_gy, _K().act_bwd(ctx.kind.fwd(ggx, w, ctx.alpha), up.saved_tensors[2], up.act))
+            up._gs_gg_premasked = g_gy.data_ptr()
+        else:
+            g_gy = _Bilinear.apply(ggx, w, ctx.kind, ctx.alpha)
+    g_w = None
+    if need_w:
+        tgt = _accum_target(ctx.wref)
+        if tgt is None:
+            tgt = _slice_target(ctx.wref, ggx, gy, ctx.kind)
+        if tgt is not None:
+            ctx.kind.bwd_weight(ggx, gy, ctx.alpha, out=tgt)
+        else:
+            g_w = _BilinearBwdWeight.apply(ggx, gy, ctx.kind, ctx.alpha).to(w.dtype)
+    return g_gy, g_w
 
 
 class _BwdDataMasked(Function):
@@ -512,6 +535,12 @@
                         _check_fused("bwd_data_pnbwd", gx_, _K().pixel_norm_bwd(ctx.kind.bwd_data(gy, w, tuple(x.shape), ctx.alpha), z_prev, pn.eps, act=pn.act, addend=gz_prev))
                     pn._gs_fused = (gx_.data_ptr(), gz_prev is not None)
                     return gx_
+            if torch.is_grad_enabled():
+                pn = _graph_norm_producer(ctx, x, gy)
+                if pn is not None:
+                    gx_ = _BwdDataPnActBwd.apply(gy, w, pn.saved_tensors[2], ctx.kind, ctx.alpha, pn.eps, pn.act, False)
+                    pn._gs_fused_graph = gx_.data_ptr()
+                    return gx_
             prod = _premask_producer(x, ctx.in_act, differentiable=True) if hasattr(ctx.kind, "bwd_data_mask") else None
             if prod is None:
                 return _BilinearBwdData.apply(gy, w, x.shape, ctx.kind, ctx.alpha)
@@ -557,26 +586,68 @@
     def backward(ctx, gg):
         g, z = ctx.saved_tensors
         done, ctx._gs_done = ctx._gs_done, None
-        if ctx.needs_input_grad[0] and ctx.needs_input_grad[1]:
-            if done is not None and gg.data_ptr() != done[0]:
-                _handoff_broken("second-order norm gradients in the forward-on-cotangent conv")
-            if done is not None:
-                g_g, g_z = gg, done[1]
-            else:
-                g_z, g_g = _K().pixel_norm_bwd_bwd(gg, g, z, ctx.eps, pre_act=ctx.act, with_g=True)
-            if _FUSE_NORM_BWD:
-                _GZ[z.data_ptr()] = g_z
-            return g_g, g_z, None, None
+        g_g, g_z = _pn_act_bwd_backward(gg, g, z, ctx.eps, ctx.act, done, ctx.needs_input_grad[0], ctx.needs_input_grad[1])
+        return g_g, g_z, None, None
+
+
+def _pn_act_bwd_backward(gg, g, z, eps, act, done, need_g, need_z, zg=None):
+    if need_g and need_z:
+        if done is not None and gg.data_ptr() != done[0]:
+            _handoff_broken("second-order norm gradients in the forward-on-cotangent conv")
         if done is not None:
-            _handoff_broken("second-order norm gradients in the forward-on-cotangent conv")
-        g_g = _K().pixel_norm_bwd(gg, z, ctx.eps, pre_act=ctx.act) if ctx.needs_input_grad[0] else None
-        g_z = _K().pixel_norm_bwd_bwd(gg, g, z, ctx.eps, pre_act=ctx.act) if ctx.needs_input_grad[1] else None
-        return g_g, g_z, None, None
+            g_g, g_z = gg, done[1]
+        else:
+            g_z, g_g = _K().pixel_norm_bwd_bwd(gg, g, z, eps, pre_act=act, with_g=True, **({} if zg is None else {"zg": zg}))
+        if _FUSE_NORM_BWD:
+            _GZ[z.data_ptr()] = g_z
+        return g_g, g_z
+    if done is not None:
+        _handoff_broken("second-order norm gradients in the forward-on-cotangent conv")
+    g_g = _K().pixel_norm_bwd(gg, z, eps, pre_act=act) if need_g else None
+    g_z = _K().pixel_norm_bwd_bwd(gg, g, z, eps, pre_act=act, **({} if zg is None else {"zg": zg})) if need_z else None
+    return g_g, g_z
+
+
+class _BwdDataPnActBwd(Function):
+
+    @staticmethod
+    def forward(ctx, gy, w, z, kind, alpha, eps, act, sole_consumer=False):
+        ctx.kind, ctx.alpha, ctx.wref, ctx.eps, ctx.act = kind, alpha, w, eps, act
+        ctx.sole_consumer = bool(sole_consumer)
+        ctx._gs_up = None
+        ctx._gs_done = None
+        u, zg = kind.bwd_data_pnbwd_graph(gy, w, tuple(z.shape), alpha, z, eps, act)
+        if _CHECK_FUSION:
+            _check_fused("bwd_data_pnbwd_graph", u, _K().pixel_norm_bwd(kind.bwd_data(gy, w, tuple(z.shape), alpha), z, eps, act=act))
+        ctx.save_for_backward(gy, w, z, u, zg)
+        return u
+
+    @staticmethod
+    @once_differentiable
+    def backward(ctx, gg):
+        gy, w, z, u, zg = ctx.saved_tensors
+        done, ctx._gs_done = ctx._gs_done, None
+        need_gy, need_w, need_z = ctx.needs_input_grad[0], ctx.needs_input_grad[1], ctx.needs_input_grad[2]
+        g_g, g_z = _pn_act_bwd_backward(gg, u, z, ctx.eps, ctx.act, done, need_gy or need_w, need_z, zg=zg)
+        g_gy, g_w = _bwd_data_backward(ctx, g_g, gy, w, need_gy, need_w) if g_g is not None else (None, None)
+        return g_gy, g_w, g_z, None, None, None, None, None
+
+
+def _graph_norm_producer(ctx, x, gy):
+    if not (_FUSE_NORM_BWD_GRAPH and ctx.input_normed and not _want_params() and hasattr(_K(), "conv2d_bwd_data_pnbwd_graph")
+            and hasattr(ctx.kind, "bwd_data_pnbwd_graph")):
+        return None
+    prod = x.grad_fn
+    if (isinstance(prod, _ConvBiasActNorm._backward_cls) and prod.act in (ACT_NONE, ACT_LRELU)
+            and ctx.kind.bwd_data_pnbwd_is_fused(tuple(x.shape), gy.shape[1], gy.dtype)):
+        return prod
+    return None
 
 
 _FUSE_NORM_EPILOGUE = not config.flag("GS_NO_NORM_EPILOGUE")
 _FUSE_NORM_BWD = not config.flag("GS_NO_NORM_BWD_EPILOGUE")
 _FUSE_NORM_BWD2 = not config.flag("GS_NO_NORM_BWD2_EPILOGUE")
+_FUSE_NORM_BWD_GRAPH = not config.flag("GS_NO_NORM_BWD_GRAPH_EPILOGUE")
 
 _GZ = {}
 
@@ -614,6 +685,7 @@
         ctx.wref, ctx.bref = w, bias
         ctx.input_normed = bool(input_normed)
         ctx._gs_fused = None
+        ctx._gs_fused_graph = None
         ctx.set_materialize_grads(False)
         keep = any(ctx.needs_input_grad)
         want_z = keep or activation_tap.active is not None
@@ -634,12 +706,25 @@
         want_w = ctx.needs_input_grad[1] and _want_params()
         want_b = ctx.has_bias and ctx.needs_input_grad[2] and _want_params()
         if torch.is_grad_enabled():
-            gy = _PnActBwd.apply(g_y, z, ctx.eps, ctx.act) if g_y is not None else None
+            fused, ctx._gs_fused_graph = ctx._gs_fused_graph, None
+            if fused is not None and (g_y is None or g_y.data_ptr() != fused):
+                _handoff_broken("previous block's norm backward in the data-gradient conv (create_graph)")
+            if fused is not None:
+                gy = g_y
+            else:
+                gy = _PnActBwd.apply(g_y, z, ctx.eps, ctx.act) if g_y is not None else None
             if g_z is not None:
                 extra = _ActBwd.apply(g_z, z, ctx.act)
                 gy = extra if gy is None else gy + extra
             sole = g_y is not None and g_z is None and not want_w and not want_b
-            gx = _BilinearBwdData.apply(gy, w, x.shape, ctx.kind, ctx.alpha, sole) if ctx.needs_input_grad[0] else None
+            gx = None
+            if ctx.needs_input_grad[0]:
+                prod = _graph_norm_producer(ctx, x, gy) if sole else None
+                if prod is not None:
+                    gx = _BwdDataPnActBwd.apply(gy, w, prod.saved_tensors[2], ctx.kind, ctx.alpha, prod.eps, prod.act, sole)
+                    prod._gs_fused_graph = gx.data_ptr()
+                else:
+                    gx = _BilinearBwdData.apply(gy, w, x.shape, ctx.kind, ctx.alpha, sole)
             gw = _BilinearBwdWeight.apply(x, gy, ctx.kind, ctx.alpha).to(w.dtype) if want_w else None
             gb = _ChannelSum.apply(gy) if want_b else None
             return gx, gw, gb, None, None, None, None, None
diff --git a/gansynth_amd/kernels.py b/gansynth_amd/kernels.py
--- a/gansynth_amd/kernels.py
+++ b/gansynth_amd/kernels.py
@@ -78,6 +78,10 @@
         n, c, h, w = x.shape
         return n * h * w, c
     return x.shape[0], x.shape[1]
+
+
+def _check_zg(zg, z):
+    assert zg.dtype == torch.float32 and zg.is_contiguous() and zg.numel() == _rows_cols(z)[0] and zg.device == z.device
 
 
 def note_mix_table(table, rows, length, total):
@@ -480,22 +484,27 @@
     def fwd_pnbwdbwd_is_fused(self, x_shape, co, ksize, stride, transposed, dtype):
         return self._is_fused(self.lib.gs_conv_fwd_pnbwdbwd_is_fused, x_shape, co, ksize, stride, transposed, dtype)
 
-    def conv2d_fwd_pnbwdbwd(self, x, w, ksize, stride, alpha, g, z, eps, act):
-        return self._fwd_pnbwdbwd(x, w, ksize, stride, False, alpha, g, z, eps, act)
-
-    def _fwd_pnbwdbwd(self, x, w, ksize, stride, transposed, alpha, g, z, eps, act):
+    def conv2d_fwd_pnbwdbwd(self, x, w, ksize, stride, alpha, g, z, eps, act, zg=None):
+        return self._fwd_pnbwdbwd(x, w, ksize, stride, False, alpha, g, z, eps, act, zg)
+
+    def _fwd_pnbwdbwd(self, x, w, ksize, stride, transposed, alpha, g, z, eps, act, zg=None):
         x, w, g, z = _act(x), _f32c(w), _act(g), _act(z)
         n, ci, h, wd = x.shape
         out_g = _empty_like_act(self._out_shape(x, w.shape[3], stride, transposed), x)
         assert g.shape == out_g.shape == z.shape and g.dtype == x.dtype == z.dtype
         out_z = torch.empty_like(out_g)
         c, ws = self._conv(_lib.CONV_FWD, w, alpha, _dt(x), n, ci, h, wd, w.shape[3], ksize, stride, transposed)
+        if zg is not None:
+            _check_zg(zg, z)
+            _lib.check(self.lib.gs_conv_fwd_pnbwdbwd_u(c, x.data_ptr(), w.data_ptr(), g.data_ptr(), zg.data_ptr(), z.data_ptr(), int(act), float(eps), out_g.data_ptr(),
+                                                       out_z.data_ptr(), _stream()), "gs_conv_fwd_pnbwdbwd_u")
+            return out_z, out_g
         _lib.check(self.lib.gs_conv_fwd_pnbwdbwd(c, x.data_ptr(), w.data_ptr(), g.data_ptr(), z.data_ptr(), int(act), float(eps), out_g.data_ptr(), out_z.data_ptr(),
                                                  _stream()), "gs_conv_fwd_pnbwdbwd")
         return out_z, out_g
 
-    def conv2d_transpose_fwd_pnbwdbwd(self, x, w, alpha, g, z, eps, act):
-        return self._fwd_pnbwdbwd(x, w, 3, 2, True, alpha, g, z, eps, act)
+    def conv2d_transpose_fwd_pnbwdbwd(self, x, w, alpha, g, z, eps, act, zg=None):
+        return self._fwd_pnbwdbwd(x, w, 3, 2, True, alpha, g, z, eps, act, zg)
 
     def bwd_data_pnbwd_is_fused(self, x_shape, co, ksize, stride, transposed, dtype):
         return self._is_fused(self.lib.gs_conv_bwd_data_pnbwd_is_fused, x_shape, co, ksize, stride, transposed, dtype)
@@ -503,12 +512,24 @@
     def conv2d_bwd_data_pnbwd(self, gy, w, x_shape, ksize, stride, alpha, z, eps, act, addend=None):
         return self._bwd_data_pnbwd(gy, w, x_shape, ksize, stride, False, alpha, z, eps, act, addend)
 
-    def _bwd_data_pnbwd(self, gy, w, x_shape, ksize, stride, transposed, alpha, z, eps, act, addend):
+    def conv2d_bwd_data_pnbwd_graph(self, gy, w, x_shape, ksize, stride, alpha, z, eps, act):
+        return self._bwd_data_pnbwd(gy, w, x_shape, ksize, stride, False, alpha, z, eps, act, None, stats=True)
+
+    def conv2d_transpose_bwd_data_pnbwd_graph(self, gy, w, alpha, z, eps, act):
+        n, _, h2, w2 = gy.shape
+        return self._bwd_data_pnbwd(gy, w, (n, w.shape[2], h2 // 2, w2 // 2), 3, 2, True, alpha, z, eps, act, None, stats=True)
+
+    def _bwd_data_pnbwd(self, gy, w, x_shape, ksize, stride, transposed, alpha, z, eps, act, addend, stats=False):
         gy, w, z = _act(gy), _f32c(w), _act(z)
         n, ci, h, wd = x_shape
         assert tuple(z.shape) == (n, ci, h, wd) and z.dtype == gy.dtype
         gx = _empty_like_act((n, ci, h, wd), gy)
         c, ws = self._conv(_lib.CONV_BWD_DATA, w, alpha, _dt(gy), n, ci, h, wd, w.shape[3], ksize, stride, transposed)
+        if stats:
+            zg = torch.empty((n, h, wd), dtype=torch.float32, device=gy.device)
+            _lib.check(self.lib.gs_conv_bwd_data_pnbwd_stats(c, gy.data_ptr(), w.data_ptr(), z.data_ptr(), int(act), float(eps), gx.data_ptr(), zg.data_ptr(), _stream()),
+                       "gs_conv_bwd_data_pnbwd_stats")
+            return gx, zg
         ap = None
         if addend is not None:
             addend = _match(addend, z)
@@ -783,12 +804,18 @@
                                                     _stream()), "gs_pixel_norm_bwd_fused")
         return gx
 
-    def pixel_norm_bwd_bwd(self, gg, g, x, eps, pre_act=0, with_g=False):
+    def pixel_norm_bwd_bwd(self, gg, g, x, eps, pre_act=0, with_g=False, zg=None):
         x = _act(x)
         gg, g = _match(gg, x), _match(g, x)
         p, c = _rows_cols(x)
         out = torch.empty_like(x)
         out_g = torch.empty_like(x) if with_g else None
+        if zg is not None:
+            _check_zg(zg, x)
+            _lib.check(self.lib.gs_pixel_norm_bwd_bwd_fused_u(gg.data_ptr(), g.data_ptr(), zg.data_ptr(), x.data_ptr(), out.data_ptr(),
+                                                              None if out_g is None else out_g.data_ptr(), p, c, float(eps), int(pre_act), _dt(x), _stream()),
+                       "gs_pixel_norm_bwd_bwd_fused_u")
+            return (out, out_g) if with_g else out
         _lib.check(self.lib.gs_pixel_norm_bwd_bwd_fused(gg.data_ptr(), g.data_ptr(), x.data_ptr(), out.data_ptr(), None if out_g is None else out_g.data_ptr(),
                                                         p, c, float(eps), int(pre_act), _dt(x), _stream()), "gs_pixel_norm_bwd_bwd_fused")
         return (out, out_g) if with_g else out
diff --git a/include/gansynth_hip.h b/include/gansynth_hip.h
--- a/include/gansynth_hip.h
+++ b/include/gansynth_hip.h
@@ -52,8 +52,11 @@
 int gs_conv_bwd_data(const GsConv* c, const void* gy, const float* w_hwio, const void* mask, int mask_act, void* gx, void* stream);
 int gs_conv_bwd_data_pnbwd(const GsConv* c, const void* gy, const float* w_hwio, const void* z, const void* addend, int act, float eps, void* gx, void* stream);
 int gs_conv_bwd_data_pnbwd_is_fused(const GsConv* c);
+int gs_conv_bwd_data_pnbwd_stats(const GsConv* c, const void* gy, const float* w_hwio, const void* z, int act, float eps, void* gx, float* zg_mean, void* stream);
 int gs_conv_fwd_pnbwdbwd(const GsConv* c, const void* x, const float* w_hwio, const void* g, const void* z, int act, float eps, void* out_g, void* out_z, void* stream);
 int gs_conv_fwd_pnbwdbwd_is_fused(const GsConv* c);
+int gs_conv_fwd_pnbwdbwd_u(const GsConv* c, const void* x, const float* w_hwio, const void* u, const float* zg_mean, const void* z, int act, float eps, void* out_g,
+                           void* out_z, void* stream);
 int gs_conv_bwd_weight(const GsConv* c, const void* x, const void* gy, float* gw_hwio, float* gb, int accumulate, void* stream);
 int gs_conv_igemm_config(int mode, int n, int hb, int wb, int ic, int oc, int dtype, int want, int* out_cfg);
 int gs_conv_igemm_table(int index, int* out11);
@@ -135,6 +138,8 @@
                                  int post_act, int accumulate, int dtype, void* ws, size_t ws_bytes, void* stream);
 int gs_pixel_norm_bwd_bwd_fused(const void* gg, const void* g, const void* x, void* out, void* out_g, int64_t p, int c, float eps, int pre_act,
                                 int dtype, void* stream);
+int gs_pixel_norm_bwd_bwd_fused_u(const void* gg, const void* u, const float* zg_mean, const void* x, void* out, void* out_g, int64_t p, int c, float eps,
+                                  int pre_act, int dtype, void* stream);
 
 int gs_upscale2d(const void* x, void* y, int n, int h, int w, int c, int fy, int fx, float scale, int dtype, void* stream);
 int gs_blocksum2d(const void* x, void* y, int n, int h, int w, int c, int fy, int fx, float scale, int dtype, void* stream);
```

New measurement: 1690 images/sec (median of 6 runs). Within noise of the previous version (+1.0%).
